# anilshanbhag/gpu-sort

Hardware: AMD Instinct MI355X
Metric: Gkeys/s sorting 2^30 uint32 keys; achieved HBM GB/s vs roofline (higher is better)
Workload: dtype u32; 1 GPU; lsb_radix_sort_2^30_u32_uniform_keys_only; keys_per_gpu=1073741824, algorithm=lsb, distribution=uniform, parallelism=single

## Files before the change

### gpu-sort_amd/_lib.py

```python
import ctypes as C
import os

import torch

_HERE = os.path.dirname(os.path.abspath(__file__))
LIB_PATH = os.environ.get("GS_LIB_PATH", os.path.join(_HERE, "lib", "libgpusort.so"))
CSRC_DIR = os.path.join(_HERE, "csrc")
INCLUDE_DIR = os.path.join(os.path.dirname(_HERE), "include")

GS_KEY_U32, GS_KEY_I32, GS_KEY_F32, GS_KEY_U64, GS_KEY_I64, GS_KEY_F64 = 0, 1, 2, 3, 4, 5
GS_KEY_U8, GS_KEY_I8, GS_KEY_U16, GS_KEY_I16 = 6, 7, 8, 9
GS_KEY_F16, GS_KEY_BF16, GS_KEY_F8 = 10, 11, 12
GS_GEN_UNIFORM, GS_GEN_ZIPF, GS_GEN_ENTROPY_AND, GS_GEN_ENUMERATED = 0, 1, 2, 3

u64, i32, vp, sz = C.c_uint64, C.c_int, C.c_void_p, C.c_size_t
pp = C.POINTER(C.c_void_p)

SIGNATURES = {
    "gs_version": (i32, []),
    "gs_error_string": (C.c_char_p, [i32]),
    "gs_lsb_temp_bytes": (sz, [u64, i32]),
    "gs_lsb_sort_u32": (i32, [vp, sz, pp, pp, C.POINTER(i32), u64, i32, i32, i32, i32, vp]),
    "gs_lsb_copy_temp_bytes": (sz, [u64, i32]),
    "gs_lsb_sort_copy_u32": (i32, [vp, sz, vp, vp, vp, vp, u64, i32, i32, i32, i32, vp]),
    "gs_lsb_wide_temp_bytes": (sz, [u64, i32, i32]),
    "gs_lsb_sort_wide": (i32, [vp, sz, pp, pp, C.POINTER(i32), u64, i32, i32, i32, i32, i32, i32, vp]),
    "gs_lsb_any_temp_bytes": (sz, [u64, i32, i32]),
    "gs_lsb_sort_any": (i32, [vp, sz, vp, vp, vp, vp, u64, i32, i32, i32, i32, i32, vp]),
    "gs_lsb_narrow_temp_bytes": (sz, [u64, i32, i32]),
    "gs_lsb_sort_narrow": (i32, [vp, sz, vp, vp, vp, vp, u64, i32, i32, i32, i32, i32, vp]),
    "gs_lsb_narrow_tile": (C.c_uint32, [i32, i32]),
    "gs_lsb_geometry": (None, [u64, i32, C.POINTER(C.c_uint32), C.POINTER(C.c_uint32), C.POINTER(C.c_uint32)]),
    "gs_lsb_workspace_layout": (i32, [vp, u64, pp, pp, pp]),
    "gs_lsb_pipe_status": (i32, [vp, u64, C.POINTER(C.c_uint32), vp]),
    "gs_lsb_plan_status": (i32, [vp, u64, C.POINTER(C.c_uint32), vp]),
    "gs_lsb_plan_cursor_status": (i32, [vp, u64, C.POINTER(C.c_uint32), vp]),
    "gs_lsb_plan_peek_status": (i32, [C.POINTER(C.c_uint32)]),
    "gs_lsb_plan_look_only": (i32, [vp, vp, vp, u64, i32, i32, vp]),
    "gs_lsb_plan_layout": (i32, [u64, C.POINTER(C.c_uint64)]),
    "gs_lsb_upsweep_u32": (i32, [vp, sz, vp, u64, i32, i32, i32, i32, vp]),
    "gs_lsb_scan_spine": (i32, [vp, sz, u64, vp]),
    "gs_lsb_downsweep_u32": (i32, [vp, sz, vp, vp, vp, vp, u64, i32, i32, i32, i32, i32, vp]),
    "gs_msb_temp_bytes": (sz, [u64, i32]),
    "gs_msb_sort_u32": (i32, [vp, sz, vp, vp, u64, vp, vp, pp, pp, i32, vp, i32]),
    "gs_msb_wide_temp_bytes": (sz, [u64, i32, i32]),
    "gs_msb_sort_wide": (i32, [vp, sz, vp, vp, u64, vp, vp, i32, i32, pp, pp, i32, vp, i32]),
    "gs_msb_large_temp_bytes": (sz, [u64, i32]),
    "gs_msb_sort_large_u32": (i32, [vp, sz, vp, vp, u64, vp, vp, i32, vp, i32]),
    "gs_msb_large_wide_temp_bytes": (sz, [u64, i32, i32]),
    "gs_msb_sort_large_wide": (i32, [vp, sz, vp, vp, u64, vp, vp, i32, i32, i32, vp, i32]),
    "gs_lsb_large_temp_bytes": (sz, [u64, i32, i32]),
    "gs_lsb_sort_large": (i32, [vp, sz, pp, pp, C.POINTER(i32), u64, i32, i32, i32, i32, i32, i32, vp]),
    "gs_lsb_narrow_large_temp_bytes": (sz, [u64, i32, i32]),
    "gs_lsb_sort_narrow_large": (i32, [vp, sz, vp, vp, vp, vp, u64, i32, i32, i32, i32, i32, vp]),
    "gs_topk_temp_bytes": (sz, [u64, u64, i32]),
    "gs_topk_u32": (i32, [vp, sz, vp, vp, vp, vp, u64, u64, i32, i32, vp]),
    "gs_topk_status": (i32, [vp, u64, u64, i32, C.POINTER(C.c_uint32), vp]),
    "gs_topk_u16_temp_bytes": (sz, [u64, u64, i32]),
    "gs_topk_u16": (i32, [vp, sz, vp, vp, vp, vp, u64, u64, i32, i32, vp]),
    "gs_topk_u16_status": (i32, [vp, u64, u64, i32, C.POINTER(C.c_uint32), vp]),
    "gs_topk_rows_temp_bytes": (sz, [u64, u64, u64, i32]),
    "gs_topk_rows_u32": (i32, [vp, sz, vp, vp, vp, vp, u64, u64, u64, u64, i32, i32, vp]),
    "gs_topk_rows_max_k": (C.c_uint32, []),
    "gs_topk_rows_plan": (i32, [u64, u64, u64, i32, C.POINTER(C.c_uint32)]),
    "gs_topk_rows_u16_temp_bytes": (sz, [u64, u64, u64, i32]),
    "gs_topk_rows_u16": (i32, [vp, sz, vp, vp, vp, vp, u64, u64, u64, u64, i32, i32, vp]),
    "gs_topk_segmented_temp_bytes": (sz, [u64, C.c_uint32, u64, i32]),
    "gs_topk_segmented_u32": (i32, [vp, sz, vp, vp, vp, vp, vp, u64, C.c_uint32, vp, vp, u64, i32, i32, vp]),
    "gs_topk_segmented_plan": (i32, [u64, C.c_uint32, u64, i32, C.POINTER(C.c_uint32)]),
    "gs_topk_segmented_status": (i32, [vp, u64, C.c_uint32, u64, i32, C.POINTER(C.c_uint32), vp]),
    "gs_msb_census": (i32, [vp, u64, i32, vp, vp]),
    "gs_msb_wide_census": (i32, [vp, u64, i32, i32, vp, vp]),
    "gs_msb_capacities": (None, [u64, i32, C.POINTER(C.c_uint32), C.POINTER(C.c_uint32), C.POINTER(C.c_uint32)]),
    "gs_msb_classify_upto": (i32, [vp, sz, vp, vp, u64, i32, i32, vp]),
    "gs_msb_read_lists": (i32, [vp, u64, i32, i32, vp, C.c_uint32, C.POINTER(C.c_uint32), C.POINTER(C.POINTER(C.c_uint32)), C.c_uint32,
                                C.POINTER(C.c_uint32), vp]),
    "gs_segmented_temp_bytes": (sz, [u64, i32, C.c_uint32]),
    "gs_segmented_sort_u32": (i32, [vp, sz, pp, pp, C.POINTER(i32), u64, C.c_uint32, vp, vp, i32, i32, i32, i32, vp]),
    "gs_segmented_wide_temp_bytes": (sz, [u64, i32, i32, C.c_uint32]),
    "gs_segmented_sort_wide": (i32, [vp, sz, pp, pp, C.POINTER(i32), u64, C.c_uint32, vp, vp, i32, i32, i32, i32, i32, i32, vp]),
    "gs_segmented_narrow_temp_bytes": (sz, [u64, i32, i32, C.c_uint32]),
    "gs_segmented_sort_narrow": (i32, [vp, sz, pp, pp, C.POINTER(i32), u64, C.c_uint32, vp, vp, i32, i32, i32, i32, i32, vp]),
    "gs_segmented_narrow_cap": (C.c_uint32, [i32, i32]),
    "gs_msb_first_pass_u32": (i32, [vp, sz, vp, vp, vp, vp, u64, i32, vp, vp]),
    "gs_msb_finish_temp_bytes": (sz, [u64, i32, i32]),
    "gs_msb_finish_u32": (i32, [vp, sz, vp, vp, vp, vp, u64, vp, i32, i32, vp, i32]),
    "gs_shard_histogram_u32": (i32, [vp, u64, i32, vp, i32, vp]),
    "gs_shard_partition_u32": (i32, [vp, sz, vp, vp, vp, vp, u64, i32, vp, i32, vp, vp, i32, vp]),
    "gs_generate_u32": (i32, [vp, u64, i32, u64, u64, i32, vp]),
    "gs_check_sorted_u32": (i32, [vp, u64, i32, vp, vp]),
    "gs_check_pairs_enumerated_u32": (i32, [vp, vp, vp, u64, vp, vp]),
    "gs_check_sorted_u64": (i32, [vp, u64, i32, vp, vp]),
    "gs_check_pairs_enumerated_wide": (i32, [vp, vp, vp, u64, i32, vp, vp]),
    "gs_check_sorted_stable": (i32, [vp, vp, u64, i32, i32, i32, i32, i32, vp, vp]),
    "gs_profile_create": (vp, []),
    "gs_profile_destroy": (None, [vp]),
    "gs_profile_begin": (None, [vp]),
    "gs_profile_end": (None, []),
    "gs_profile_read": (i32, [vp, C.POINTER(C.c_double), C.POINTER(u64)]),
    "gs_kernel_name": (C.c_char_p, [i32]),
}
GS_K_COUNT = 10


class GpuSortError(RuntimeError):
    def __init__(self, code, what):
        self.code = code
        super().__init__(f"{what}: hipError {code} ({error_string(code)})")


def _load():
    if not os.path.exists(LIB_PATH):
        raise ImportError(
            f"{LIB_PATH} is missing: the HIP extension is not built. "
            "Run `python -c 'import __graft_entry__ as g; g.build()'` (or make -C gpu-sort_amd/csrc). "
            "There is no CPU fallback."
        )
    lib = C.CDLL(LIB_PATH)
    for name, (res, args) in SIGNATURES.items():
        fn = getattr(lib, name)
        fn.restype = res
        fn.argtypes = args
    return lib


lib = _load()


def error_string(code):
    s = lib.gs_error_string(int(code))
    return s.decode() if s else "?"


def check(code, what):
    if code != 0:
        raise GpuSortError(code, what)


class KernelProfile:

    def __init__(self):
        self._p = lib.gs_profile_create()

    def __enter__(self):
        lib.gs_profile_begin(self._p)
        return self

    def __exit__(self, *exc):
        lib.gs_profile_end()
        return False

    def read(self):
        ms = (C.c_double * GS_K_COUNT)()
        cnt = (u64 * GS_K_COUNT)()
        check(lib.gs_profile_read(self._p, ms, cnt), "gs_profile_read")
        return {lib.gs_kernel_name(i).decode(): (ms[i], int(cnt[i])) for i in range(GS_K_COUNT) if cnt[i]}

    def close(self):
        if self._p and lib is not None:
            lib.gs_profile_destroy(self._p)
        self._p = None

    def __del__(self):
        try:
            self.close()
        except Exception:
            pass
```

### gpu-sort_amd/csrc/gs_lsb_downsweep.inc

```
#ifndef GS_EXP_SLEEP_MODE
#define GS_EXP_SLEEP_MODE 0
#endif
#ifndef GS_EXP_SLEEP_MIN_TILES
#define GS_EXP_SLEEP_MIN_TILES 49152u
#endif
#ifndef GS_EXP_SLEEP_PAIRS
#define GS_EXP_SLEEP_PAIRS 0
#endif
template <bool HAS_VALUES, bool OFF64 = false>
struct DownsweepSmem {
    uint32_t whist[LSB_WAVES][RADIX];
#ifdef GS_EXP_ALLWAVE_KEYS
    uint16_t wbase[LSB_WAVES][RADIX];
#else
    uint16_t wbase[HAS_VALUES ? LSB_WAVES : 1][RADIX];
#endif
    std::conditional_t<OFF64, uint64_t, uint32_t> gbase[RADIX];
    uint32_t stage[LSB_TILE * (HAS_VALUES ? 2 : 1)];
    uint32_t dead;
};

#ifdef GS_EXP_PHASES
__device__ uint32_t gs_phase_buf[131072 * 16];
#define GS_PHASE(k)                                                                          \
    do {                                                                                     \
        const unsigned long long now_ = __builtin_amdgcn_s_memtime();                        \
        if (tid == 0 && t < 131072u) gs_phase_buf[t * 16 + (k)] = (uint32_t)(now_ - tprev_); \
        tprev_ = now_;                                                                       \
    } while (0)
#define GS_PHASE_WAIT(what) asm volatile("s_waitcnt " what ::: "memory")
#else
#define GS_PHASE(k) do { } while (0)
#define GS_PHASE_WAIT(what) do { } while (0)
#endif

constexpr uint32_t PIPE_SPIN_LIMIT = 1u << 18;

template <bool HAS_VALUES, bool TAIL, int TW, bool BIG, bool PIPE, bool OFF64 = false, bool CURSOR = false>
__device__ __forceinline__ void downsweep_tile(DownsweepSmem<HAS_VALUES, OFF64> &sm, const uint32_t t,
    const uint32_t *__restrict__ keys_in, uint32_t *__restrict__ keys_out, const uint32_t *__restrict__ vals_in,
    uint32_t *__restrict__ vals_out, const uint32_t *__restrict__ spine, const uint16_t *__restrict__ prefix16,
    const uint32_t *__restrict__ totals, const PassParams &p, const uint64_t *__restrict__ sc, uint32_t tag,
    uint32_t *__restrict__ error_word, const uint32_t tid_ = threadIdx.x, const uint64_t *__restrict__ dbase = nullptr,
    uint32_t *__restrict__ cursor = nullptr, uint32_t *__restrict__ irr = nullptr, const uint32_t irr_cap = 0u)
{
    static_assert(!CURSOR || (!HAS_VALUES && !TAIL && !PIPE && !OFF64), "cursor mode: full tiles of keys-only three-launch passes");
#ifdef GS_EXP_ALLWAVE_KEYS
    constexpr bool ALLWAVE = true;
#else
    constexpr bool ALLWAVE = HAS_VALUES;
#endif

    [[maybe_unused]] const int tid = (int)tid_;
    const int lane = (int)(tid_ & 63u), w = (int)(tid_ >> 6);
    const uint32_t full_tiles = p.n / (uint32_t)LSB_TILE;
    auto tw_in = [&](uint32_t k) { return TW == 0 ? k : twiddle_in(k, TW == 2 ? p.f32_in : 0, p.xor_in); };
    auto tw_out = [&](uint32_t k) { return TW == 0 ? k : twiddle_out(k, TW == 2 ? p.f32_out : 0, p.xor_out); };
    uint32_t wbits = p.bits;
    asm volatile("" : "+v"(wbits));
    auto digit = [&](uint32_t k) { return __builtin_amdgcn_ubfe(k, p.shift, wbits); };

    uint32_t *my = sm.whist[w];
    const uint16_t *mybase = sm.wbase[w];
    const uint32_t wbase = (uint32_t)w * (WAVE * LSB_KPT) + lane;
    const uint32_t tail_valid = p.n - full_tiles * (uint32_t)LSB_TILE;
    (void)full_tiles;

#ifdef GS_EXP_PHASES
    unsigned long long tprev_ = __builtin_amdgcn_s_memtime();
    const unsigned long long t0_ = tprev_, r0_ = __builtin_amdgcn_s_memrealtime();
#endif
#ifdef GS_EXP_SLEEP_START
    __builtin_amdgcn_s_sleep(GS_EXP_SLEEP_START);
#endif
    if (!HAS_VALUES) __builtin_amdgcn_s_setprio(3);
    const uint64_t tile_base = (uint64_t)t * LSB_TILE;
    const uint32_t valid = TAIL ? tail_valid : (uint32_t)LSB_TILE;

    uint64_t scg[4] = {0, 0, 0, 0};
    const uint64_t *scrow = nullptr;
    if (PIPE && w == 0) {
        scrow = sc + (size_t)(t / LSB_CHUNK) * RADIX + 4 * lane;
#pragma unroll
        for (int q = 0; q < 4; ++q) scg[q] = ld_agent(scrow + q);
    }

    uint32_t key[LSB_KPT], val[HAS_VALUES ? LSB_KPT : 1], pos[LSB_KPT];
    {
        const uint32_t *kin = keys_in + tile_base;
        if (!TAIL) {
#pragma unroll
            for (int i = 0; i < LSB_KPT; ++i) key[i] = kin[wbase + i * WAVE];
        } else {
            const uint32_t pad = twiddle_out(0xffffffffu, TW == 2 ? p.f32_in : 0, TW ? p.xor_in : 0u);
#pragma unroll
            for (int i = 0; i < LSB_KPT; ++i) {
                const uint32_t idx = wbase + i * WAVE;
                key[i] = pad;
                if (idx < tail_valid) key[i] = kin[idx];
            }
        }
    }
    [[maybe_unused]] uint32_t cur_lo = 0, cur_hi = 0, claim[4] = {0, 0, 0, 0};
    if constexpr (CURSOR) {
        if (w == 0) {
            cur_lo = (tw_in(keys_in[tile_base]) >> (p.shift - (uint32_t)RADIX_BITS)) & (uint32_t)(RADIX - 1);
            cur_hi = (tw_in(keys_in[tile_base + (LSB_TILE - 1)]) >> (p.shift - (uint32_t)RADIX_BITS)) & (uint32_t)(RADIX - 1);
        }
    }
    GS_PHASE(0);
#ifndef GS_EXP_RANK_PRIO
#define GS_EXP_RANK_PRIO 0
#endif
    if (!HAS_VALUES) __builtin_amdgcn_s_setprio(GS_EXP_RANK_PRIO);
    if (HAS_VALUES) {
        const uint32_t *vin = vals_in + tile_base;
#pragma unroll
        for (int i = 0; i < LSB_KPT; ++i) {
            const uint32_t idx = wbase + i * WAVE;
            val[i] = 0;
            if (!TAIL || idx < valid) val[i] = vin[idx];
        }
    }
    uint32_t dstart[4] = {0, 0, 0, 0};
    if constexpr (OFF64) {
        if (TAIL && w == 0) {
            const uint4 tot = reinterpret_cast<const uint4 *>(totals)[lane];
            dstart[0] = tot.x; dstart[1] = tot.y; dstart[2] = tot.z; dstart[3] = tot.w;
        }
    } else if (!CURSOR && w == 0) {
        const uint4 tot = reinterpret_cast<const uint4 *>(totals)[lane];
        const uint32_t lane_sum = tot.x + tot.y + tot.z + tot.w;
        const uint32_t ex = wave_inclusive_scan(lane_sum) - lane_sum;
        dstart[0] = ex + (TAIL ? tot.x : 0u);
        dstart[1] = dstart[0] + (TAIL ? tot.y : tot.x);
        dstart[2] = dstart[1] + (TAIL ? tot.z : tot.y);
        dstart[3] = dstart[2] + (TAIL ? tot.w : tot.z);
    }

    uint32_t tbase[4] = {0, 0, 0, 0};
    if (!TAIL && !PIPE && !CURSOR && w == 0) {
        const uint32_t *sp = spine + (uint32_t)(4 * lane) * p.grid + t / LSB_CHUNK;
        const uint2 pf = reinterpret_cast<const uint2 *>(prefix16 + (size_t)t * RADIX)[lane];
        tbase[0] = sp[0] + (pf.x & 0xffffu);
        tbase[1] = sp[p.grid] + (pf.x >> 16);
        tbase[2] = sp[2 * p.grid] + (pf.y & 0xffffu);
        tbase[3] = sp[3 * p.grid] + (pf.y >> 16);
    }

    if (PIPE && !TAIL && w == 0) {
        uint32_t spins = 0;
        bool gave_up = false;
        for (;;) {
            const bool ok = (uint32_t)(scg[0] >> 32) == tag && (uint32_t)(scg[1] >> 32) == tag &&
                            (uint32_t)(scg[2] >> 32) == tag && (uint32_t)(scg[3] >> 32) == tag;
            if (__builtin_amdgcn_ballot_w64(!ok) == 0) break;
            if (++spins > PIPE_SPIN_LIMIT) {
                if (lane == 0) atomicOr(error_word, 1u);
                gave_up = true;
                break;
            }
            __builtin_amdgcn_s_sleep(8);
#pragma unroll
            for (int q = 0; q < 4; ++q) scg[q] = ld_agent(scrow + q);
        }
        if (lane == 0) sm.dead = gave_up ? 1u : 0u;
        const uint64_t pf = ld_agent(reinterpret_cast<const uint64_t *>(prefix16 + (size_t)t * RADIX) + lane);
        tbase[0] = (uint32_t)scg[0] + (uint32_t)(pf & 0xffffu);
        tbase[1] = (uint32_t)scg[1] + (uint32_t)((pf >> 16) & 0xffffu);
        tbase[2] = (uint32_t)scg[2] + (uint32_t)((pf >> 32) & 0xffffu);
        tbase[3] = (uint32_t)scg[3] + (uint32_t)(pf >> 48);
    }

    auto publish_gbase = [&](const uint32_t (&ex)[4], const uint32_t (&run)[4]) {
        uint32_t g[4];
#pragma unroll
        for (int q = 0; q < 4; ++q) g[q] = dstart[q] + tbase[q] - ex[q];
        if (TAIL) {
#pragma unroll
            for (int q = 0; q < 4; ++q) g[q] -= run[q];
            const uint32_t pads = (uint32_t)LSB_TILE - valid, dmax = p.mask;
            if (lane == (int)(dmax >> 2)) {
#pragma unroll
                for (int q = 0; q < 4; ++q)
                    if ((dmax & 3u) == (uint32_t)q) g[q] += pads;
            }
        }
        if constexpr (OFF64) {
#pragma unroll
            for (int q = 0; q < 4; ++q) sm.gbase[4 * lane + q] = dbase[4 * lane + q] + (uint64_t)(int64_t)(int32_t)g[q];
        } else {
            if (!BIG) {
#pragma unroll
                for (int q = 0; q < 4; ++q) g[q] <<= 2;
            }
            reinterpret_cast<uint4 *>(sm.gbase)[lane] = make_uint4(g[0], g[1], g[2], g[3]);
        }
    };

#pragma unroll
    for (int i = lane; i < RADIX; i += WAVE) my[i] = 0;
    GS_PHASE_WAIT("vmcnt(0)");
    GS_PHASE(1);
#pragma unroll
    for (int i = 0; i < LSB_KPT; ++i) key[i] = tw_in(key[i]);
    {
        uint32_t d_prev = 0, plo = 0, phi = 0;
#pragma unroll
        for (int i = 0; i <= LSB_KPT; ++i) {
            uint32_t d_cur = 0, clo = 0, chi = 0;
            if (i < LSB_KPT) {
                d_cur = digit(key[i]);
                match_digit(d_cur, clo, chi);
            }
            if (i > 0) {
                const uint32_t lower = count_lower(plo, phi);
                pos[i - 1] = my[d_prev] + lower;
                if (lower == 0)
                    __hip_atomic_fetch_add(&my[d_prev], (uint32_t)(__popc(plo) + __popc(phi)), __ATOMIC_RELAXED,
                                           __HIP_MEMORY_SCOPE_WAVEFRONT);
            }
            d_prev = d_cur; plo = clo; phi = chi;
        }
    }
#pragma unroll
    for (int i = 0; i < LSB_KPT; ++i) {
        asm volatile("" : "+v"(pos[i]), "+v"(key[i]));
    }
    if constexpr (CURSOR) {
        if (w == 0 && lane == 0) {
            const bool straddles = cur_lo != cur_hi;
            sm.dead = straddles ? 1u : 0u;
            if (straddles) {
                const uint32_t at = atomicAdd(&irr[0], 1u);
                if (at < irr_cap) irr[1u + at] = t;
            }
        }
    }
    GS_PHASE_WAIT("lgkmcnt(0)");
    GS_PHASE(2);
    __syncthreads();
    GS_PHASE(3);
    if (PIPE && !TAIL && sm.dead) return;
    if (CURSOR && sm.dead) return;

    if constexpr (ALLWAVE) {
        uint32_t run[4] = {0, 0, 0, 0}, below[4] = {0, 0, 0, 0};
#pragma unroll
        for (int j = 0; j < LSB_WAVES; ++j) {
            const uint4 x = reinterpret_cast<const uint4 *>(sm.whist[j])[lane];
            run[0] += x.x; run[1] += x.y; run[2] += x.z; run[3] += x.w;
            if (j < w) { below[0] += x.x; below[1] += x.y; below[2] += x.z; below[3] += x.w; }
        }
        const uint32_t lane_sum = run[0] + run[1] + run[2] + run[3];
        uint32_t ex[4];
        ex[0] = wave_inclusive_scan(lane_sum) - lane_sum;
        ex[1] = ex[0] + run[0];
        ex[2] = ex[1] + run[1];
        ex[3] = ex[2] + run[2];
        reinterpret_cast<uint2 *>(sm.wbase[w])[lane] =
            make_uint2((ex[0] + below[0]) | ((ex[1] + below[1]) << 16), (ex[2] + below[2]) | ((ex[3] + below[3]) << 16));
        if (w == 0) publish_gbase(ex, run);
    } else {
        if (w == 0) {
            uint32_t run[4] = {0, 0, 0, 0};
#pragma unroll
            for (int j = 0; j < LSB_WAVES; ++j) {
                const uint4 x = reinterpret_cast<const uint4 *>(sm.whist[j])[lane];
                run[0] += x.x; run[1] += x.y; run[2] += x.z; run[3] += x.w;
            }
            const uint32_t lane_sum = run[0] + run[1] + run[2] + run[3];
            uint32_t ex[4];
            ex[0] = wave_inclusive_scan(lane_sum) - lane_sum;
            ex[1] = ex[0] + run[0];
            ex[2] = ex[1] + run[1];
            ex[3] = ex[2] + run[2];
            if constexpr (CURSOR) {
                reinterpret_cast<uint4 *>(sm.gbase)[lane] = make_uint4(ex[0], ex[1], ex[2], ex[3]);
                uint32_t *row = cursor + (size_t)__builtin_amdgcn_readfirstlane(cur_lo) * RADIX;
#pragma unroll
                for (int q = 0; q < 4; ++q) {
                    const int d = q * WAVE + lane;
                    const uint32_t e0 = sm.gbase[d], e1 = sm.gbase[d == RADIX - 1 ? d : d + 1];
                    const uint32_t cnt = (d == RADIX - 1 ? (uint32_t)LSB_TILE : e1) - e0;
                    claim[q] = __hip_atomic_fetch_add(row + d, cnt, __ATOMIC_RELAXED, __HIP_MEMORY_SCOPE_AGENT);
                }
            } else {
                publish_gbase(ex, run);
            }
            asm volatile("" ::: "memory");
            uint4 e4 = make_uint4(ex[0] << 2, ex[1] << 2, ex[2] << 2, ex[3] << 2);
#pragma unroll
            for (int j = 0; j < LSB_WAVES; ++j) {
                const uint4 x = reinterpret_cast<const uint4 *>(sm.whist[j])[lane];
                reinterpret_cast<uint4 *>(sm.whist[j])[lane] = e4;
                e4.x += x.x << 2; e4.y += x.y << 2; e4.z += x.z << 2; e4.w += x.w << 2;
            }
        }
        __syncthreads();
    }
    GS_PHASE(4);

    {
        uint32_t wb[LSB_KPT];
#pragma unroll
        for (int i = 0; i < LSB_KPT; ++i) {
            const uint32_t d = digit(key[i]);
            wb[i] = ALLWAVE ? (uint32_t)mybase[d] : my[d];
        }
#pragma unroll
        for (int i = 0; i < LSB_KPT; ++i) {
            if (HAS_VALUES) {
                reinterpret_cast<uint2 *>(sm.stage)[pos[i] + wb[i]] = make_uint2(key[i], val[i]);
            } else if (ALLWAVE) {
                sm.stage[pos[i] + wb[i]] = key[i];
            } else {
                const uint32_t at = (pos[i] << 2) + wb[i];
                *reinterpret_cast<uint32_t *>(reinterpret_cast<char *>(sm.stage) + at) = key[i];
            }
        }
    }
    if constexpr (CURSOR) {
        if (w == 0) {
#pragma unroll
            for (int q = 0; q < 4; ++q) {
                const int d = q * WAVE + lane;
                const uint32_t g = claim[q] - sm.gbase[d];
                sm.gbase[d] = BIG ? g : g << 2;
            }
        }
    }
    GS_PHASE_WAIT("lgkmcnt(0)");
    GS_PHASE(5);
    __syncthreads();
    GS_PHASE(6);
#ifndef GS_EXP_SLEEP
#define GS_EXP_SLEEP 32
#define GS_EXP_SLEEP_MODE_DEFAULT 0
#else
#define GS_EXP_SLEEP_MODE_DEFAULT GS_EXP_SLEEP_MODE
#endif
    if ((!HAS_VALUES || GS_EXP_SLEEP_PAIRS) && full_tiles >= GS_EXP_SLEEP_MIN_TILES) {
        [[maybe_unused]] const int ws = __builtin_amdgcn_readfirstlane(w);
#if GS_EXP_SLEEP_MODE_DEFAULT == 3
        if (ws & 1) __builtin_amdgcn_s_sleep(GS_EXP_SLEEP); else __builtin_amdgcn_s_sleep(GS_EXP_SLEEP_B);
#elif GS_EXP_SLEEP_MODE_DEFAULT == 4
        if (ws >= 4) __builtin_amdgcn_s_sleep(GS_EXP_SLEEP);
#elif GS_EXP_SLEEP_MODE_DEFAULT == 1
        if (ws & 1) __builtin_amdgcn_s_sleep(GS_EXP_SLEEP);
#elif GS_EXP_SLEEP_MODE_DEFAULT == 0
        __builtin_amdgcn_s_sleep(GS_EXP_SLEEP);
#endif
    }
#ifndef GS_EXP_STORE_PRIO
#define GS_EXP_STORE_PRIO 3
#endif
    if (!HAS_VALUES) __builtin_amdgcn_s_setprio(GS_EXP_STORE_PRIO);
#pragma unroll
    for (int i = 0; i < LSB_KPT; ++i) {
        const uint32_t slot = (uint32_t)w * (WAVE * LSB_KPT) + i * WAVE + lane;
        uint32_t k, v = 0;
        if (HAS_VALUES) {
            const uint2 kv = reinterpret_cast<const uint2 *>(sm.stage)[slot];
            k = kv.x; v = kv.y;
        } else {
            k = sm.stage[slot];
        }
        const auto g = sm.gbase[digit(k)];
        if (!TAIL || slot < valid) {
            if constexpr (OFF64) {
                const uint64_t dst = g + slot;
                keys_out[dst] = tw_out(k);
                if (HAS_VALUES) vals_out[dst] = v;
            } else if (BIG) {
                const uint32_t dst = g + slot;
                keys_out[dst] = tw_out(k);
                if (HAS_VALUES) vals_out[dst] = v;
            } else {
                const uint32_t off = g + slot * 4u;
                *reinterpret_cast<uint32_t *>(reinterpret_cast<char *>(keys_out) + off) = tw_out(k);
                if (HAS_VALUES) *reinterpret_cast<uint32_t *>(reinterpret_cast<char *>(vals_out) + off) = v;
            }
        }
    }
    GS_PHASE(7);
#ifdef GS_EXP_DRAIN
    asm volatile("s_waitcnt vmcnt(0)" ::: "memory");
#endif
    GS_PHASE_WAIT("vmcnt(0)");
    GS_PHASE(8);
#ifdef GS_EXP_PHASES
    if (tid == 0 && t < 131072u) {
        gs_phase_buf[t * 16 + 9] = (uint32_t)(__builtin_amdgcn_s_memtime() - t0_);
        gs_phase_buf[t * 16 + 10] = (uint32_t)(__builtin_amdgcn_s_memrealtime() - r0_);
        gs_phase_buf[t * 16 + 11] = (uint32_t)r0_;
        gs_phase_buf[t * 16 + 12] = blockIdx.x;
        gs_phase_buf[t * 16 + 13] = __builtin_amdgcn_s_getreg((31 << 11) | 4);
        gs_phase_buf[t * 16 + 14] = __builtin_amdgcn_s_getreg((31 << 11) | 20);
    }
#endif
}
```

### gpu-sort_amd/csrc/gs_lsb_plan.hip

```cpp
#include "gs_device.hpp"
#include "gs_lsb.hpp"
#include "gs_msb_tasks.hpp"
#ifndef GS_PLAN_N_MIN
#define GS_PLAN_N_MIN (1ull << 28)
#endif
#include <cstddef>
#include <cstdlib>
#include <cstring>
#include <type_traits>

namespace gs {

#include "gs_lsb_upsweep.inc"

#include "gs_lsb_downsweep.inc"

constexpr uint32_t PLAN_GROUPS = 65536;
constexpr uint32_t PLAN_WORDS = PLAN_GROUPS / 2;
constexpr uint32_t PLAN_PLANNED = 1u, PLAN_CLASSIC = 2u;
constexpr uint32_t PLAN_SKIP = 0xffffffffu;
constexpr int PLAN_LOOK_THREADS = 1024, PLAN_LOOK_WAVES = PLAN_LOOK_THREADS / WAVE, PLAN_LOOK_BATCH = 32;
constexpr uint32_t PLAN_LOOK_HALVES = PLAN_LOOK_WAVES / LSB_CHUNK;
static_assert(PLAN_LOOK_WAVES % LSB_CHUNK == 0, "a look workgroup takes whole chunks");
constexpr uint32_t PLAN_LOOK_MAX_GRID = MI355X_CUS;
constexpr uint32_t PLAN_BLOCKS = 128, PLAN_BLOCK_WORDS = PLAN_WORDS / PLAN_BLOCKS, PLAN_BLOCK_GROUPS = PLAN_GROUPS / PLAN_BLOCKS;
constexpr int PLAN_SORT_BITS = 16;
constexpr int PLAN_SKEW_LANES = 8;
constexpr uint32_t PLAN_IRR_CAP = RADIX - 1;
constexpr size_t PLAN_CURSOR_BYTES = (size_t)PLAN_GROUPS * sizeof(uint32_t);

struct PlanBlock {
    uint32_t route, max_group, nonempty, tasks[MSB_NCLASS], total;
    uint32_t shift[4];
    uint32_t ups_skip[4];
    MsbLevel level[2];
    union {
        uint32_t wg_bad[PLAN_LOOK_MAX_GRID];
        uint32_t irr[1 + PLAN_IRR_CAP];
    };
    uint32_t blk_total[PLAN_BLOCKS], blk_max[PLAN_BLOCKS], blk_nonempty[PLAN_BLOCKS];
    uint32_t blk_class[PLAN_BLOCKS][MSB_NCLASS];
    uint32_t blk_class_base[PLAN_BLOCKS][MSB_NCLASS];
    uint32_t offsets[PLAN_GROUPS + 1];
    uint32_t cursor_mode;
};
static_assert(1 + PLAN_IRR_CAP <= PLAN_LOOK_MAX_GRID, "the list of straddling tiles fits the look's flags");
static_assert(sizeof(MsbLevel) == 64 && offsetof(PlanBlock, level) == 64, "plan block layout");

__device__ __forceinline__ int plan_class_of(uint32_t size)
{
    return size <= msb_class_cap(0) ? 0 : size <= msb_class_cap(1) ? 1 : size <= msb_class_cap(2) ? 2 : 3;
}

__device__ __forceinline__ void look_add(uint32_t *tab, uint32_t *my, uint32_t g)
{
    const unsigned long long act = __builtin_amdgcn_ballot_w64(true);
    const uint32_t g0 = __builtin_amdgcn_readfirstlane(g);
    if (__builtin_amdgcn_ballot_w64(g == g0) == act) {
        if (count_lower_mask(act) == 0) {
            atomicAdd(&tab[g0 >> 1], (uint32_t)__popcll(act) << ((g0 & 1u) * 16u));
            atomicAdd(&my[g0 & 0xffu], (uint32_t)__popcll(act));
        }
    } else {
        atomicAdd(&tab[g >> 1], 1u << ((g & 1u) * 16u));
        atomicAdd(&my[g & 0xffu], 1u);
    }
}

__device__ __forceinline__ void look_add_skew(uint32_t *tab, uint32_t *my, uint32_t g, int lane)
{
    unsigned long long rest = ~0ull;
#pragma unroll
    for (int r = 0; r < 2; ++r) {
        if (rest == 0ull) break;
        const int lead = __builtin_amdgcn_readfirstlane(__builtin_ctzll(rest));
        const uint32_t g0 = (uint32_t)__builtin_amdgcn_readlane((int)g, lead);
        const unsigned long long m = __builtin_amdgcn_ballot_w64(g == g0) & rest;
        if (lane == lead) {
            atomicAdd(&tab[g0 >> 1], (uint32_t)__popcll(m) << ((g0 & 1u) * 16u));
            atomicAdd(&my[g0 & 0xffu], (uint32_t)__popcll(m));
        }
        rest &= ~m;
    }
    if ((rest >> lane) & 1ull) {
        atomicAdd(&tab[g >> 1], 1u << ((g & 1u) * 16u));
        atomicAdd(&my[g & 0xffu], 1u);
    }
}

__device__ __forceinline__ uint32_t look_slot_of_block(uint32_t b, uint32_t grid)
{
    if (grid % MI355X_XCDS) return b;
    return (b % MI355X_XCDS) * (grid / MI355X_XCDS) + b / MI355X_XCDS;
}

struct LookSmem {
    uint32_t tab[PLAN_WORDS];
    uint32_t hist[PLAN_LOOK_WAVES][RADIX + 1];
    uint32_t red[2];
};
static_assert(sizeof(LookSmem) <= 160 * 1024, "the look's LDS");

__global__ __launch_bounds__(PLAN_LOOK_THREADS) void lsb_plan_look_kernel(const uint32_t *__restrict__ keys, uint32_t *__restrict__ partial,
                                                                          PlanBlock *__restrict__ plan, uint32_t *__restrict__ spine,
                                                                          uint16_t *__restrict__ prefix16, uint32_t n, uint32_t chunks,
                                                                          int f32_in, uint32_t xor_in)
{
    __shared__ LookSmem sm;
    uint32_t *tab = sm.tab;
    const int tid = threadIdx.x, w = wave_id(), lane = lane_id();
    for (uint32_t i = tid; i < PLAN_WORDS; i += PLAN_LOOK_THREADS) tab[i] = 0;
    for (uint32_t i = tid; i < sizeof(sm.hist) / sizeof(uint32_t); i += PLAN_LOOK_THREADS) (&sm.hist[0][0])[i] = 0;
    if (tid < 2) sm.red[tid] = 0;
    __syncthreads();
    uint32_t *my = sm.hist[w];
    const uint32_t num_tiles = n / (uint32_t)LSB_TILE + (n % (uint32_t)LSB_TILE ? 1u : 0u);
    const uint32_t units = (chunks + PLAN_LOOK_HALVES - 1u) / PLAN_LOOK_HALVES;
    auto group_of = [&](uint32_t raw) { return twiddle_in(raw, f32_in, xor_in) >> 16; };
    uint32_t counted = 0;
    constexpr int GB = PLAN_LOOK_BATCH;
#pragma unroll 1
    for (uint32_t unit = look_slot_of_block(blockIdx.x, gridDim.x); unit < units; unit += gridDim.x) {
        const uint32_t tile = unit * (uint32_t)PLAN_LOOK_WAVES + (uint32_t)w;
        if (tile < num_tiles) {
        const uint32_t lo = tile * (uint32_t)LSB_TILE;
        const uint32_t len = (n - lo < (uint32_t)LSB_TILE) ? n - lo : (uint32_t)LSB_TILE;
        const uint32_t *src = keys + lo;
        counted += len;
        if (len == (uint32_t)LSB_TILE) {
#pragma unroll 1
            for (uint32_t j = 0; j < (uint32_t)LSB_TILE; j += GB * WAVE) {
                const uint32_t *at = src + j + lane;
                uint32_t v[GB];
#pragma unroll
                for (int u = 0; u < GB; ++u) v[u] = __builtin_nontemporal_load(at + u * WAVE);
                const uint32_t ga = group_of(v[0]), gb = group_of(v[GB / 2]);
                const unsigned long long ma = __builtin_amdgcn_ballot_w64(ga == __builtin_amdgcn_readfirstlane(ga)),
                                         mb = __builtin_amdgcn_ballot_w64(gb == __builtin_amdgcn_readfirstlane(gb));
                if (ma == ~0ull || mb == ~0ull) {
#pragma unroll
                    for (int u = 0; u < GB; ++u) look_add(tab, my, group_of(v[u]));
                } else if (__popcll(ma) >= PLAN_SKEW_LANES || __popcll(mb) >= PLAN_SKEW_LANES) {
#pragma unroll
                    for (int u = 0; u < GB; ++u) look_add_skew(tab, my, group_of(v[u]), lane);
                } else {
#pragma unroll
                    for (int u = 0; u < GB; ++u) {
                        const uint32_t g = group_of(v[u]);
                        atomicAdd(&tab[g >> 1], 1u << ((g & 1u) * 16u));
                        atomicAdd(&my[g & 0xffu], 1u);
                    }
                }
            }
        } else {
            const uint32_t last = len - 1u;
#pragma unroll 1
            for (uint32_t j = 0; j < len; j += GB * WAVE) {
                uint32_t v[GB];
#pragma unroll
                for (int u = 0; u < GB; ++u) {
                    const uint32_t idx = j + u * WAVE + lane;
                    v[u] = src[idx < last ? idx : last];
                }
#pragma unroll
                for (int u = 0; u < GB; ++u)
                    if (j + u * WAVE + lane < len) look_add(tab, my, group_of(v[u]));
            }
        }
        }
        __syncthreads();
        if (tid < (int)PLAN_LOOK_HALVES * RADIX) {
            const uint32_t half = (uint32_t)tid / RADIX, d = (uint32_t)tid % RADIX, chunk = unit * PLAN_LOOK_HALVES + half;
            uint32_t run = 0;
#pragma unroll
            for (int j = 0; j < LSB_CHUNK; ++j) {
                const uint32_t t = chunk * LSB_CHUNK + (uint32_t)j;
                if (t < num_tiles) prefix16[(size_t)t * RADIX + d] = (uint16_t)run;
                uint32_t *c = &sm.hist[half * LSB_CHUNK + j][d];
                run += *c;
                *c = 0;
            }
            if (chunk < chunks) spine[d * chunks + chunk] = run;
        }
        __syncthreads();
    }
    uint32_t sum = 0;
    uint32_t *out = partial + (size_t)blockIdx.x * PLAN_WORDS;
    for (uint32_t i = tid; i < PLAN_WORDS; i += PLAN_LOOK_THREADS) {
        const uint32_t c = tab[i];
        sum += (c & 0xffffu) + (c >> 16);
        out[i] = c;
    }
    sum = wave_reduce_sum(sum);
    if (lane == 0) { atomicAdd(&sm.red[0], sum); atomicAdd(&sm.red[1], counted); }
    __syncthreads();
    if (tid == 0) plan->wg_bad[blockIdx.x] = sm.red[0] != sm.red[1] ? 1u : 0u;
}

__global__ __launch_bounds__(RADIX) void lsb_plan_reduce_kernel(const uint32_t *__restrict__ partial, PlanBlock *__restrict__ plan, uint32_t parts)
{
    __shared__ uint32_t scratch[8];
    __shared__ uint32_t red[2 + MSB_NCLASS];
    const uint32_t tid = threadIdx.x, wi = blockIdx.x * PLAN_BLOCK_WORDS + tid;
    if (tid < 2 + MSB_NCLASS) red[tid] = 0;
    uint32_t c0 = 0, c1 = 0;
#pragma unroll 8
    for (uint32_t g = 0; g < parts; ++g) {
        const uint32_t v = partial[(size_t)g * PLAN_WORDS + wi];
        c0 += v & 0xffffu;
        c1 += v >> 16;
    }
    uint32_t total = 0;
    const uint32_t ex = block_exclusive_scan_256(c0 + c1, scratch, &total);
    plan->offsets[2 * wi] = ex;
    plan->offsets[2 * wi + 1] = ex + c0;
    atomicMax(&red[0], c0 > c1 ? c0 : c1);
    if (c0) { atomicAdd(&red[1], 1u); atomicAdd(&red[2 + plan_class_of(c0)], 1u); }
    if (c1) { atomicAdd(&red[1], 1u); atomicAdd(&red[2 + plan_class_of(c1)], 1u); }
    __syncthreads();
    if (tid == 0) {
        plan->blk_total[blockIdx.x] = total;
        plan->blk_max[blockIdx.x] = red[0];
        plan->blk_nonempty[blockIdx.x] = red[1];
    }
    if (tid < MSB_NCLASS) plan->blk_class[blockIdx.x][tid] = red[2 + tid];
}

__global__ __launch_bounds__(RADIX) void lsb_plan_decide_kernel(PlanBlock *__restrict__ plan, uint32_t n, uint32_t parts, uint32_t cursor_on)
{
    __shared__ uint32_t s_base, s_total, s_max, s_nz, s_cls[MSB_NCLASS], s_clsbase[MSB_NCLASS];
    const uint32_t tid = threadIdx.x, b = blockIdx.x;
    if (tid == 0) {
        uint32_t base = 0, total = 0, mx = 0, nz = 0;
        for (uint32_t i = 0; i < PLAN_BLOCKS; ++i) {
            if (i == b) base = total;
            total += plan->blk_total[i];
            const uint32_t m = plan->blk_max[i];
            mx = m > mx ? m : mx;
            nz += plan->blk_nonempty[i];
        }
        s_base = base; s_total = total; s_max = mx; s_nz = nz;
    } else if (tid <= MSB_NCLASS) {
        const uint32_t c = tid - 1u;
        uint32_t base = 0, total = 0;
        for (uint32_t i = 0; i < PLAN_BLOCKS; ++i) {
            if (i == b) base = total;
            total += plan->blk_class[i][c];
        }
        s_cls[c] = total; s_clsbase[c] = base;
    }
    const int any_bad = __syncthreads_or(tid < parts ? (int)plan->wg_bad[tid] : 0);
    const uint32_t g = b * PLAN_BLOCK_GROUPS + 2u * tid;
    plan->offsets[g] += s_base;
    plan->offsets[g + 1] += s_base;
    if (tid < MSB_NCLASS) plan->blk_class_base[b][tid] = s_clsbase[tid];
    if (b == 0 && tid == 0) {
        const bool planned = !any_bad && s_total == n && s_max <= msb_class_cap(MSB_NCLASS - 1);
        plan->route = planned ? PLAN_PLANNED : PLAN_CLASSIC;
        plan->max_group = s_max;
        plan->nonempty = s_nz;
        plan->total = s_total;
        MsbLevel l0{}, l1{};
        for (int c = 0; c < MSB_NCLASS; ++c) {
            plan->tasks[c] = planned ? s_cls[c] : 0u;
            l0.task_count[c] = planned ? s_cls[c] : 0u;
        }
        l0.keys = n;
        l1.packed = planned ? (1ull << 32) : 0ull;
        plan->level[0] = l0;
        plan->level[1] = l1;
        for (int q = 0; q < 4; ++q) {
            plan->shift[q] = planned ? (q < 2 ? 16u + 8u * (uint32_t)q : PLAN_SKIP) : 8u * (uint32_t)q;
            plan->ups_skip[q] = planned && q != 1 ? 1u : 0u;
        }
        plan->offsets[PLAN_GROUPS] = n;
        plan->cursor_mode = planned && cursor_on ? 1u : 0u;
    }
}

constexpr int PLAN_PEEK_WORDS = 9;
static_assert(offsetof(PlanBlock, total) == (PLAN_PEEK_WORDS - 2) * sizeof(uint32_t), "the head is eight words");
__global__ void lsb_plan_peek_kernel(const PlanBlock *__restrict__ plan, uint32_t *mailbox)
{
    const uint32_t *head = &plan->route;
    for (int i = 0; i < PLAN_PEEK_WORDS - 1; ++i) mailbox[i] = head[i];
    mailbox[PLAN_PEEK_WORDS - 1] = plan->cursor_mode;
    __threadfence_system();
}

struct PlanLists { MsbTask *tasks[MSB_NCLASS]; uint32_t cap[MSB_NCLASS]; };
__global__ __launch_bounds__(PLAN_BLOCK_GROUPS) void lsb_plan_tasks_kernel(const PlanBlock *__restrict__ plan, PlanLists lists)
{
    __shared__ uint32_t wcnt[PLAN_BLOCK_GROUPS / WAVE][MSB_NCLASS];
    if (plan->route != PLAN_PLANNED) return;
    const uint32_t tid = threadIdx.x, g = blockIdx.x * PLAN_BLOCK_GROUPS + tid;
    const int w = wave_id(), lane = lane_id();
    const uint32_t off = plan->offsets[g], size = plan->offsets[g + 1] - off;
    const int cls = size ? plan_class_of(size) : -1;
    uint32_t lower = 0;
#pragma unroll
    for (int c = 0; c < MSB_NCLASS; ++c) {
        const unsigned long long m = __builtin_amdgcn_ballot_w64(cls == c);
        if (cls == c) lower = count_lower_mask(m);
        if (lane == 0) wcnt[w][c] = (uint32_t)__popcll(m);
    }
    __syncthreads();
    if (cls >= 0) {
        uint32_t idx = plan->blk_class_base[blockIdx.x][cls] + lower;
        for (int j = 0; j < w; ++j) idx += wcnt[j][cls];
        if (idx < lists.cap[cls]) lists.tasks[cls][idx] = MsbTask{off, size, (uint32_t)PLAN_SORT_BITS, 0u};
    }
}

template <bool PLAIN>
__global__ __launch_bounds__(LSB_THREADS, GS_EXP_UPS_WPE) void lsb_plan_upsweep_kernel(const uint32_t *__restrict__ keys,
                                                                       uint32_t *__restrict__ spine, uint16_t *__restrict__ prefix16,
                                                                       const uint32_t *__restrict__ slot_shift,
                                                                       const uint32_t *__restrict__ slot_ups_skip, PassParams p)
{
    __shared__ UpsweepSmem<false, false> sm;
    const uint32_t sh = *slot_shift;
    if (sh == PLAN_SKIP || *slot_ups_skip) return;
    p.shift = sh;
    upsweep_chunk<false, false, PLAIN>(sm, keys, chunk_of_block(blockIdx.x, p.grid), spine, prefix16, nullptr, nullptr, p, PipeParams{});
}

template <bool TAIL, int TW, bool BIG>
__global__ __launch_bounds__(LSB_THREADS, 6) void lsb_plan_downsweep_kernel(const uint32_t *__restrict__ keys_in, uint32_t *__restrict__ keys_out,
                                                                            const uint32_t *__restrict__ totals, const uint32_t *__restrict__ spine,
                                                                            const uint16_t *__restrict__ prefix16,
                                                                            const uint32_t *__restrict__ slot_shift, PassParams p)
{
    __shared__ __attribute__((aligned(16))) DownsweepSmem<false> sm;
    const uint32_t sh = *slot_shift;
    if (sh == PLAN_SKIP) return;
    p.shift = sh;
    const uint32_t full_tiles = p.n / (uint32_t)LSB_TILE;
    if (!TAIL && blockIdx.x >= full_tiles) return;
    const uint32_t t = TAIL ? full_tiles : tile_of_item_wide(blockIdx.x, full_tiles);
    downsweep_tile<false, TAIL, TW, BIG, false>(sm, t, keys_in, keys_out, nullptr, nullptr, spine, prefix16, totals, p, nullptr, 0u, nullptr);
}

template <bool PLAIN>
__global__ __launch_bounds__(LSB_THREADS, GS_EXP_UPS_WPE) void lsb_plan_upsweep2_kernel(const uint32_t *__restrict__ keys,
                                                                        uint32_t *__restrict__ spine, uint16_t *__restrict__ prefix16,
                                                                        PlanBlock *__restrict__ plan, uint32_t *__restrict__ cursor,
                                                                        PassParams p)
{
    __shared__ UpsweepSmem<false, false> sm;
    if (plan->cursor_mode) {
        if (blockIdx.x == 0 && threadIdx.x == 0) plan->irr[0] = 0;
        for (uint32_t i = blockIdx.x * (uint32_t)LSB_THREADS + threadIdx.x; i < PLAN_GROUPS; i += gridDim.x * (uint32_t)LSB_THREADS)
            cursor[i] = plan->offsets[((i & (uint32_t)(RADIX - 1)) << RADIX_BITS) | (i >> RADIX_BITS)];
        return;
    }
    const uint32_t sh = plan->shift[1];
    if (sh == PLAN_SKIP || plan->ups_skip[1]) return;
    p.shift = sh;
    upsweep_chunk<false, false, PLAIN>(sm, keys, chunk_of_block(blockIdx.x, p.grid), spine, prefix16, nullptr, nullptr, p, PipeParams{});
}

template <bool TAIL, bool BIG>
__global__ __launch_bounds__(LSB_THREADS, 6) void lsb_plan_scatter2_kernel(const uint32_t *__restrict__ keys_in, uint32_t *__restrict__ keys_out,
                                                                           const uint32_t *__restrict__ totals, const uint32_t *__restrict__ spine,
                                                                           const uint16_t *__restrict__ prefix16, PlanBlock *__restrict__ plan,
                                                                           uint32_t *__restrict__ cursor, PassParams p)
{
    __shared__ __attribute__((aligned(16))) DownsweepSmem<false> sm;
    const uint32_t sh = plan->shift[1];
    if (sh == PLAN_SKIP) return;
    p.shift = sh;
    const uint32_t full_tiles = p.n / (uint32_t)LSB_TILE;
    const uint32_t mode = plan->cursor_mode;
    if constexpr (TAIL) {
        if (mode) return;
        downsweep_tile<false, true, 2, true, false>(sm, full_tiles, keys_in, keys_out, nullptr, nullptr, spine, prefix16, totals, p, nullptr, 0u,
                                                    nullptr);
    } else {
        if (blockIdx.x >= full_tiles) return;
        const uint32_t t = tile_of_item_wide(blockIdx.x, full_tiles);
        if (mode)
            downsweep_tile<false, false, 0, BIG, false, false, true>(sm, t, keys_in, keys_out, nullptr, nullptr, spine, prefix16, totals, p,
                                                                     nullptr, 0u, nullptr, threadIdx.x, nullptr, cursor, plan->irr, PLAN_IRR_CAP);
        else
            downsweep_tile<false, false, 0, BIG, false>(sm, t, keys_in, keys_out, nullptr, nullptr, spine, prefix16, totals, p, nullptr, 0u,
                                                        nullptr);
    }
}

__global__ __launch_bounds__(LSB_THREADS) void lsb_plan_irregular_kernel(const uint32_t *__restrict__ keys_in, uint32_t *__restrict__ keys_out,
                                                                         const PlanBlock *__restrict__ plan, uint32_t *__restrict__ cursor,
                                                                         uint32_t n)
{
    if (!plan->cursor_mode) return;
    const uint32_t full_tiles = n / (uint32_t)LSB_TILE;
    uint32_t lo, len;
    if (blockIdx.x == PLAN_IRR_CAP) {
        lo = full_tiles * (uint32_t)LSB_TILE;
        len = n - lo;
    } else {
        const uint32_t listed = plan->irr[0] < PLAN_IRR_CAP ? plan->irr[0] : PLAN_IRR_CAP;
        if (blockIdx.x >= listed) return;
        const uint32_t t = plan->irr[1u + blockIdx.x];
        if (t >= full_tiles) return;
        lo = t * (uint32_t)LSB_TILE;
        len = (uint32_t)LSB_TILE;
    }
    const int lane = lane_id();
    for (uint32_t i = threadIdx.x; i - (uint32_t)lane < len; i += (uint32_t)LSB_THREADS) {
        const bool have = i < len;
        const uint32_t k = have ? keys_in[lo + i] : 0u;
        const uint32_t g = k >> 16, c = ((g & (uint32_t)(RADIX - 1)) << RADIX_BITS) | (g >> RADIX_BITS);
        unsigned long long rest = __builtin_amdgcn_ballot_w64(have);
        uint32_t at = 0;
#pragma unroll
        for (int r = 0; r < 2; ++r) {
            if (rest == 0ull) break;
            const int lead = __builtin_amdgcn_readfirstlane(__builtin_ctzll(rest));
            const uint32_t c0 = (uint32_t)__builtin_amdgcn_readlane((int)c, lead);
            const unsigned long long m = __builtin_amdgcn_ballot_w64(have && c == c0) & rest;
            uint32_t first = 0;
            if (lane == lead) first = __hip_atomic_fetch_add(cursor + c0, (uint32_t)__popcll(m), __ATOMIC_RELAXED, __HIP_MEMORY_SCOPE_AGENT);
            first = (uint32_t)__builtin_amdgcn_readlane((int)first, lead);
            if ((m >> lane) & 1ull) at = first + (uint32_t)__popcll(m & ((1ull << lane) - 1ull));
            rest &= ~m;
        }
        if ((rest >> lane) & 1ull) at = __hip_atomic_fetch_add(cursor + c, 1u, __ATOMIC_RELAXED, __HIP_MEMORY_SCOPE_AGENT);
        if (have && at < n) keys_out[at] = k;
    }
}

static inline size_t align256(size_t x) { return (x + 255) & ~(size_t)255; }

static inline bool plan_enabled()
{
    static const bool v = [] { const char *e = getenv("GS_LSB_KEYS_PLAN"); return !(e && strcmp(e, "classic") == 0); }();
    return v;
}
static inline bool plan_cursor_enabled()
{
    static const bool v = [] { const char *e = getenv("GS_LSB_PLAN_SCATTER2"); return !(e && strcmp(e, "stable") == 0); }();
    return v;
}
constexpr uint64_t PLAN_N_MAX = (uint64_t)PLAN_GROUPS * 16620u;
constexpr uint64_t PLAN_N_FLOOR = 65536;
constexpr uint64_t PLAN_N_MIN = GS_PLAN_N_MIN;
static inline uint64_t plan_min_items()
{
    static const uint64_t v = [] {
        const char *e = getenv("GS_LSB_PLAN_MIN_ITEMS");
        if (!e) return PLAN_N_MIN;
        const uint64_t x = strtoull(e, nullptr, 10);
        return x < PLAN_N_FLOOR ? PLAN_N_FLOOR : x;
    }();
    return v;
}
static inline bool plan_has_block(uint64_t n) { return !lsb_pipe_enabled() && n >= plan_min_items(); }
static inline bool plan_size_ok(uint64_t n) { return plan_has_block(n) && n <= PLAN_N_MAX; }
static inline uint32_t plan_list_cap(uint64_t n, int c)
{
    const uint64_t m = c == 0 ? n : n / ((uint64_t)msb_class_cap(c - 1) + 1u) + 1u;
    return (uint32_t)(m < PLAN_GROUPS ? m : PLAN_GROUPS);
}
static inline size_t plan_lists_bytes(uint64_t n)
{
    size_t b = 0;
    for (int c = 0; c < MSB_NCLASS; ++c) b += (size_t)plan_list_cap(n, c) * sizeof(MsbTask);
    return b;
}
static inline size_t plan_block_offset(uint64_t n)
{
    const size_t a = lsb_temp_bytes(n), b = plan_lists_bytes(n);
    return align256(a > b ? a : b);
}
static inline size_t plan_temp_bytes(uint64_t n) { return plan_block_offset(n) + align256(sizeof(PlanBlock)); }
static inline uint32_t *plan_cursors(char *base, uint64_t n) { return (uint32_t *)(base + plan_block_offset(n) - PLAN_CURSOR_BYTES); }

template <int TW, bool BIG>
static void launch_plan_downsweep(const uint32_t *kin, uint32_t *kout, const LsbWorkspace &ws, const uint32_t *slot_shift,
                                  const PassParams &p, hipStream_t s)
{
    hipLaunchKernelGGL((lsb_plan_downsweep_kernel<false, TW, BIG>), dim3(p.ds_grid), dim3(LSB_THREADS), 0, s, kin, kout, ws.totals,
                       ws.spine, ws.prefix16, slot_shift, p);
}

static int lsb_plan_slot2(const uint32_t *kin, uint32_t *kout, const LsbWorkspace &ws, PlanBlock *plan, uint32_t *cursor,
                          const PassParams &p, hipStream_t s);
static int lsb_plan_slot(const uint32_t *kin, uint32_t *kout, const LsbWorkspace &ws, const uint32_t *slot_shift,
                         const uint32_t *slot_ups_skip, const PassParams &p, bool real, bool ups_real, hipStream_t s)
{
    {
        KernelTimer kt(ups_real ? GS_K_LSB_UPSWEEP : GS_K_OTHER, s);
        if (!p.f32_in && !p.xor_in)
            hipLaunchKernelGGL(lsb_plan_upsweep_kernel<true>, dim3(p.grid), dim3(LSB_THREADS), 0, s, kin, ws.spine, ws.prefix16, slot_shift,
                               slot_ups_skip, p);
        else
            hipLaunchKernelGGL(lsb_plan_upsweep_kernel<false>, dim3(p.grid), dim3(LSB_THREADS), 0, s, kin, ws.spine, ws.prefix16, slot_shift,
                               slot_ups_skip, p);
    }
    {
        if (const int e = lsb_scan_as(ws.spine, ws.totals, p.grid, s, real ? GS_K_LSB_SCAN : GS_K_OTHER)) return e;
    }
    {
        KernelTimer kt(real ? GS_K_LSB_DOWNSWEEP : GS_K_OTHER, s);
        if (p.n >= (uint32_t)LSB_TILE) {
            const int tw = (p.f32_in || p.f32_out) ? 2 : ((p.xor_in | p.xor_out) ? 1 : 0);
            const bool big = p.n > (1u << 30);
#define GS_PDS(TW_, BIG_) launch_plan_downsweep<TW_, BIG_>(kin, kout, ws, slot_shift, p, s)
            if (big) { if (tw == 2) GS_PDS(2, true); else if (tw == 1) GS_PDS(1, true); else GS_PDS(0, true); }
            else { if (tw == 2) GS_PDS(2, false); else if (tw == 1) GS_PDS(1, false); else GS_PDS(0, false); }
#undef GS_PDS
        }
        if (p.n % (uint32_t)LSB_TILE)
            hipLaunchKernelGGL((lsb_plan_downsweep_kernel<true, 2, true>), dim3(1), dim3(LSB_THREADS), 0, s, kin, kout, ws.totals,
                               (const uint32_t *)nullptr, (const uint16_t *)nullptr, slot_shift, p);
    }
    return (int)hipGetLastError();
}

static int lsb_plan_slot2(const uint32_t *kin, uint32_t *kout, const LsbWorkspace &ws, PlanBlock *plan, uint32_t *cursor,
                          const PassParams &p, hipStream_t s)
{
    if (p.f32_in || p.f32_out || p.xor_in || p.xor_out) return hipErrorInvalidValue;
    if ((char *)cursor < (char *)ws.prefix16) return hipErrorInvalidValue;
    {
        KernelTimer kt(GS_K_OTHER, s);
        hipLaunchKernelGGL(lsb_plan_upsweep2_kernel<true>, dim3(p.grid), dim3(LSB_THREADS), 0, s, kin, ws.spine, ws.prefix16, plan, cursor, p);
    }
    if (const int e = lsb_scan_as(ws.spine, ws.totals, p.grid, s, GS_K_LSB_SCAN)) return e;
    {
        KernelTimer kt(GS_K_LSB_DOWNSWEEP, s);
        if (p.n >= (uint32_t)LSB_TILE) {
            if (p.n > (1u << 30))
                hipLaunchKernelGGL((lsb_plan_scatter2_kernel<false, true>), dim3(p.ds_grid), dim3(LSB_THREADS), 0, s, kin, kout, ws.totals,
                                   ws.spine, ws.prefix16, plan, cursor, p);
            else
                hipLaunchKernelGGL((lsb_plan_scatter2_kernel<false, false>), dim3(p.ds_grid), dim3(LSB_THREADS), 0, s, kin, kout, ws.totals,
                                   ws.spine, ws.prefix16, plan, cursor, p);
        }
        if (p.n % (uint32_t)LSB_TILE)
            hipLaunchKernelGGL((lsb_plan_scatter2_kernel<true, true>), dim3(1), dim3(LSB_THREADS), 0, s, kin, kout, ws.totals,
                               (const uint32_t *)nullptr, (const uint16_t *)nullptr, plan, cursor, p);
    }
    {
        KernelTimer kt(GS_K_OTHER, s);
        hipLaunchKernelGGL(lsb_plan_irregular_kernel, dim3(PLAN_IRR_CAP + (p.n % (uint32_t)LSB_TILE ? 1u : 0u)), dim3(LSB_THREADS), 0, s, kin,
                           kout, plan, cursor, p.n);
    }
    return (int)hipGetLastError();
}

static int lsb_plan_look(const uint32_t *keys, uint32_t *alt, const LsbWorkspace &ws, PlanBlock *plan, uint64_t n, const PassParams &tw,
                         hipStream_t s)
{
    const uint32_t parts = (uint32_t)(n / PLAN_WORDS < PLAN_LOOK_MAX_GRID ? n / PLAN_WORDS : PLAN_LOOK_MAX_GRID);
    const uint32_t chunks = lsb_make_params(n, 16, RADIX_BITS).grid;
    KernelTimer kt(GS_K_OTHER, s);
    hipLaunchKernelGGL(lsb_plan_look_kernel, dim3(parts), dim3(PLAN_LOOK_THREADS), 0, s, keys, alt, plan, ws.spine, ws.prefix16, (uint32_t)n,
                       chunks, tw.f32_in, tw.xor_in);
    hipLaunchKernelGGL(lsb_plan_reduce_kernel, dim3(PLAN_BLOCKS), dim3(RADIX), 0, s, alt, plan, parts);
    hipLaunchKernelGGL(lsb_plan_decide_kernel, dim3(PLAN_BLOCKS), dim3(RADIX), 0, s, plan, (uint32_t)n, parts, plan_cursor_enabled() ? 1u : 0u);
    return (int)hipGetLastError();
}

static int lsb_plan_slot2_cursor(const uint32_t *kin, uint32_t *kout, const LsbWorkspace &ws, PlanBlock *plan, uint32_t *cursor,
                                 const PassParams &p, hipStream_t s)
{
    if (p.f32_in || p.f32_out || p.xor_in || p.xor_out) return hipErrorInvalidValue;
    if ((char *)cursor < (char *)ws.prefix16) return hipErrorInvalidValue;
    {
        KernelTimer kt(GS_K_OTHER, s);
        hipLaunchKernelGGL(lsb_plan_upsweep2_kernel<true>, dim3(p.grid), dim3(LSB_THREADS), 0, s, kin, ws.spine, ws.prefix16, plan, cursor, p);
    }
    if (p.n >= (uint32_t)LSB_TILE) {
        KernelTimer kt(GS_K_LSB_DOWNSWEEP, s);
        if (p.n > (1u << 30))
            hipLaunchKernelGGL((lsb_plan_scatter2_kernel<false, true>), dim3(p.ds_grid), dim3(LSB_THREADS), 0, s, kin, kout, ws.totals,
                               ws.spine, ws.prefix16, plan, cursor, p);
        else
            hipLaunchKernelGGL((lsb_plan_scatter2_kernel<false, false>), dim3(p.ds_grid), dim3(LSB_THREADS), 0, s, kin, kout, ws.totals,
                               ws.spine, ws.prefix16, plan, cursor, p);
    }
    {
        KernelTimer kt(GS_K_OTHER, s);
        hipLaunchKernelGGL(lsb_plan_irregular_kernel, dim3(PLAN_IRR_CAP + (p.n % (uint32_t)LSB_TILE ? 1u : 0u)), dim3(LSB_THREADS), 0, s, kin,
                           kout, plan, cursor, p.n);
    }
    return (int)hipGetLastError();
}

struct PlanPeek {
    uint32_t *host = nullptr, *dev = nullptr;
    hipEvent_t ev = nullptr;
    int device = -1;
    bool armed = false;
};
static bool plan_peek_enabled()
{
    static const bool on = [] { const char *e = getenv("GS_LSB_PLAN_PEEK"); return !(e && e[0] == '0'); }();
    return on;
}
constexpr int PLAN_PEEK_DEVICES = 16;
struct PlanPeekTable {
    PlanPeek slot[PLAN_PEEK_DEVICES];
    ~PlanPeekTable()
    {
        for (PlanPeek &pk : slot) {
            if (pk.ev) (void)hipEventDestroy(pk.ev);
            if (pk.host) (void)hipHostFree(pk.host);
        }
    }
};
static PlanPeek *plan_peek_get(hipStream_t s)
{
    if (!plan_peek_enabled()) return nullptr;
    hipStreamCaptureStatus cs = hipStreamCaptureStatusNone;
    if (hipStreamIsCapturing(s, &cs) != hipSuccess || cs != hipStreamCaptureStatusNone) { (void)hipGetLastError(); return nullptr; }
    thread_local PlanPeekTable table;
    int dev = -1;
    if (hipGetDevice(&dev) != hipSuccess || dev < 0 || dev >= PLAN_PEEK_DEVICES) { (void)hipGetLastError(); return nullptr; }
    PlanPeek &pk = table.slot[dev];
    if (pk.device != dev) {
        void *h = nullptr, *d = nullptr;
        if (hipHostMalloc(&h, 64, hipHostMallocMapped | hipHostMallocPortable) != hipSuccess ||
            hipHostGetDevicePointer(&d, h, 0) != hipSuccess ||
            hipEventCreateWithFlags(&pk.ev, hipEventDisableTiming) != hipSuccess) {
            (void)hipGetLastError();
            if (h) (void)hipHostFree(h);
            pk.ev = nullptr;
            return nullptr;
        }
        pk.host = (uint32_t *)h; pk.dev = (uint32_t *)d; pk.device = dev;
    }
    if (pk.armed) { (void)hipEventSynchronize(pk.ev); (void)hipGetLastError(); }
    pk.armed = false;
    return &pk;
}
static void plan_peek_arm(PlanPeek *pk, const PlanBlock *plan, hipStream_t s)
{
    if (!pk) return;
    for (int i = 0; i < PLAN_PEEK_WORDS; ++i) ((volatile uint32_t *)pk->host)[i] = 0;
    KernelTimer kt(GS_K_OTHER, s);
    hipLaunchKernelGGL(lsb_plan_peek_kernel, dim3(1), dim3(1), 0, s, plan, pk->dev);
    pk->armed = hipGetLastError() == hipSuccess && hipEventRecord(pk->ev, s) == hipSuccess;
    if (!pk->armed) (void)hipGetLastError();
}
struct PlanSeen { bool ok = false; uint32_t route = 0, tasks[MSB_NCLASS] = {0, 0, 0, 0}, cursor_mode = 0; };
static PlanSeen plan_peek_wait(PlanPeek *pk, uint64_t n)
{
    PlanSeen seen;
    if (!pk || !pk->armed) return seen;
    pk->armed = false;
    if (hipEventSynchronize(pk->ev) != hipSuccess) { (void)hipGetLastError(); return seen; }
    uint32_t w[PLAN_PEEK_WORDS];
    for (int i = 0; i < PLAN_PEEK_WORDS; ++i) w[i] = ((const volatile uint32_t *)pk->host)[i];
    const uint32_t route = w[0], nonempty = w[2], total = w[7], mode = w[8];
    if (route != PLAN_PLANNED && route != PLAN_CLASSIC) return seen;
    if (route == PLAN_PLANNED ? (uint64_t)total != n : (uint64_t)total > n) return seen;
    if (mode > 1u || (mode && route != PLAN_PLANNED)) return seen;
    uint64_t sum = 0;
    for (int c = 0; c < MSB_NCLASS; ++c) {
        if (w[3 + c] > plan_list_cap(n, c)) return seen;
        sum += w[3 + c];
    }
    if (route == PLAN_PLANNED ? sum != nonempty : sum != 0) return seen;
    seen.ok = true;
    seen.route = route;
    seen.cursor_mode = mode;
    for (int c = 0; c < MSB_NCLASS; ++c) seen.tasks[c] = w[3 + c];
    return seen;
}
static thread_local uint32_t plan_peek_last[4] = {0, 0, 0, 0};

int lsb_plan_sort(char *base, uint32_t *d_keys[2], int *selector, uint64_t n, int descending, int key_type, hipStream_t s)
{
    const LsbWorkspace ws = lsb_carve(base, n);
    char *lists_end = base + plan_block_offset(n);
    PlanBlock *plan = (PlanBlock *)lists_end;
    PlanLists lists;
    for (int c = MSB_NCLASS - 1; c >= 0; --c) {
        lists.cap[c] = plan_list_cap(n, c);
        lists_end -= (size_t)lists.cap[c] * sizeof(MsbTask);
        lists.tasks[c] = (MsbTask *)lists_end;
    }
    int sel = *selector, e;
    PassParams tw{};
    lsb_twiddle_masks(key_type, descending, true, true, tw);
    if ((e = lsb_plan_look(d_keys[sel], d_keys[sel ^ 1], ws, plan, n, tw, s))) return e;
    PlanPeek *peek = plan_peek_get(s);
    plan_peek_arm(peek, plan, s);
    PlanSeen seen;
    plan_peek_last[0] = plan_peek_last[1] = 0; plan_peek_last[2] = 4; plan_peek_last[3] = (1u << MSB_NCLASS) - 1u;
    for (int slot = 0; slot < 4; ++slot) {
        PassParams p = lsb_make_params(n, 0, RADIX_BITS);
        lsb_twiddle_masks(key_type, descending, slot == 0, slot == 3, p);
        const uint32_t *kin = d_keys[sel];
        uint32_t *kout = d_keys[sel ^ 1];
        e = hipSuccess;
        if (seen.ok && seen.route == PLAN_CLASSIC)
            e = lsb_plan_slot(kin, kout, ws, &plan->shift[slot], &plan->ups_skip[slot], p, true, true, s);
        else if (seen.ok && slot >= 2)
            ;
        else if (seen.ok && slot == 1 && seen.cursor_mode)
            e = lsb_plan_slot2_cursor(kin, kout, ws, plan, plan_cursors(base, n), p, s);
        else if (slot == 1 && plan_cursor_enabled())
            e = lsb_plan_slot2(kin, kout, ws, plan, plan_cursors(base, n), p, s);
        else
            e = lsb_plan_slot(kin, kout, ws, &plan->shift[slot], &plan->ups_skip[slot], p, slot < 2, slot == 1, s);
        if (e) return e;
        sel ^= 1;
        if (slot == 0) {
            seen = plan_peek_wait(peek, n);
            if (seen.ok) {
                plan_peek_last[0] = 1; plan_peek_last[1] = seen.route; plan_peek_last[2] = seen.route == PLAN_PLANNED ? 2 : 4;
                plan_peek_last[3] = 0;
                for (int c = 0; c < MSB_NCLASS; ++c) plan_peek_last[3] |= seen.tasks[c] ? 1u << c : 0u;
            }
        }
    }
    if (seen.ok && seen.route == PLAN_CLASSIC) {
        *selector = sel;
        return hipSuccess;
    }
    {
        KernelTimer kt(GS_K_OTHER, s);
        hipLaunchKernelGGL(lsb_plan_tasks_kernel, dim3(PLAN_BLOCKS), dim3(PLAN_BLOCK_GROUPS), 0, s, plan, lists);
    }
    if ((e = (int)hipGetLastError())) return e;
    if ((e = msb_local_sorts_in_place(plan->level, lists.tasks, PLAN_GROUPS, PLAN_GROUPS, d_keys[sel], PLAN_SORT_BITS, n, tw.f32_out,
                                      tw.xor_out, s, seen.ok ? seen.tasks : nullptr)))
        return e;
    *selector = sel;
    return hipSuccess;
}


bool lsb_plan_has_block(uint64_t n) { return plan_has_block(n); }
size_t lsb_plan_temp_bytes(uint64_t n) { return plan_temp_bytes(n); }
bool lsb_plan_applies(uint64_t n) { return plan_enabled() && plan_size_ok(n); }

}

using namespace gs;

extern "C" {

int gs_lsb_plan_status(void *d_temp, uint64_t num_items, uint32_t out[8], void *stream)
{
    GS_CLEAR_STALE_ERROR();
    if (!d_temp || !out || num_items >= (1ull << 32)) return hipErrorInvalidValue;
    memset(out, 0, 8 * sizeof(uint32_t));
    if (!plan_enabled() || !plan_size_ok(num_items)) return hipSuccess;
    const PlanBlock *plan = (const PlanBlock *)(gs_ws_base(d_temp) + plan_block_offset(num_items));
    hipError_t e = hipMemcpyAsync(out, plan, 8 * sizeof(uint32_t), hipMemcpyDeviceToHost, (hipStream_t)stream);
    if (e == hipSuccess) e = hipStreamSynchronize((hipStream_t)stream);
    return (int)e;
}

int gs_lsb_plan_cursor_status(void *d_temp, uint64_t num_items, uint32_t out[4], void *stream)
{
    GS_CLEAR_STALE_ERROR();
    if (!d_temp || !out || num_items >= (1ull << 32)) return hipErrorInvalidValue;
    memset(out, 0, 4 * sizeof(uint32_t));
    if (!plan_enabled() || !plan_size_ok(num_items)) return hipSuccess;
    const PlanBlock *plan = (const PlanBlock *)(gs_ws_base(d_temp) + plan_block_offset(num_items));
    uint32_t w[2] = {0, 0};
    hipError_t e = hipMemcpyAsync(&w[0], &plan->cursor_mode, sizeof(uint32_t), hipMemcpyDeviceToHost, (hipStream_t)stream);
    if (e == hipSuccess) e = hipMemcpyAsync(&w[1], &plan->irr[0], sizeof(uint32_t), hipMemcpyDeviceToHost, (hipStream_t)stream);
    if (e == hipSuccess) e = hipStreamSynchronize((hipStream_t)stream);
    if (e != hipSuccess) return (int)e;
    if (w[0] == 1u) {
        out[0] = 1;
        out[2] = w[1];
        out[1] = w[1] + (num_items % (uint64_t)LSB_TILE ? 1u : 0u);
    }
    return hipSuccess;
}

int gs_lsb_plan_peek_status(uint32_t out[4])
{
    if (!out) return hipErrorInvalidValue;
    memcpy(out, plan_peek_last, sizeof(plan_peek_last));
    return hipSuccess;
}

int gs_lsb_plan_look_only(void *d_temp, const void *d_keys, void *d_alt, uint64_t num_items, int key_type, int descending, void *stream)
{
    GS_CLEAR_STALE_ERROR();
    if (!d_temp || !d_keys || !d_alt || num_items >= (1ull << 32)) return hipErrorInvalidValue;
    if (!plan_enabled() || !plan_size_ok(num_items)) return hipErrorInvalidValue;
    char *base = gs_ws_base(d_temp);
    PassParams tw{};
    lsb_twiddle_masks(key_type, descending, true, true, tw);
    return lsb_plan_look((const uint32_t *)d_keys, (uint32_t *)d_alt, lsb_carve(base, num_items), (PlanBlock *)(base + plan_block_offset(num_items)),
                         num_items, tw, (hipStream_t)stream);
}

int gs_lsb_plan_layout(uint64_t num_items, uint64_t out[4])
{
    if (!out || num_items >= (1ull << 32) || !plan_enabled() || !plan_size_ok(num_items)) return hipErrorInvalidValue;
    char *base = (char *)(uintptr_t)GS_WS_ALIGN;
    const LsbWorkspace ws = lsb_carve(base, num_items);
    out[0] = (uint64_t)((char *)ws.spine - base);
    out[1] = (uint64_t)((char *)ws.prefix16 - base);
    out[2] = plan_block_offset(num_items);
    out[3] = lsb_make_params(num_items, 16, RADIX_BITS).grid;
    return hipSuccess;
}

}
```

### gpu-sort_amd/csrc/gs_msb.hip

```cpp
#include "gs_device.hpp"
#include <new>
#include "gs_lsb.hpp"
#include "gs_msb_tasks.hpp"
#include <type_traits>
#include <vector>
#include <cstdlib>

namespace gs {

constexpr int MSB_THREADS = 512;
constexpr int MSB_WAVES = MSB_THREADS / WAVE;
constexpr int MSB_KPT = 16;
constexpr int MSB_TILE = MSB_THREADS * MSB_KPT;
constexpr uint32_t MSB_MERGE = 3000;
constexpr uint32_t MSB_MAX_GRID = 16384;
__host__ __device__ constexpr uint32_t msb_tiles_of(uint32_t x) { return x / (uint32_t)MSB_TILE + (x % (uint32_t)MSB_TILE ? 1u : 0u); }
#ifndef GS_PAIR_CLASSES
#define GS_PAIR_CLASSES 4
#endif
__host__ __device__ constexpr int msb_num_classes(bool has_values) { return has_values ? GS_PAIR_CLASSES : 4; }

struct MsbBucket { uint32_t offset, size, tile_start, tiles; };
struct MsbPiece { uint32_t lo, size, tile_start, bucket; };
struct MsbTile { uint32_t lo, valid, bucket, pad; };
// ... 619 lines not shown
                e4.x += x.x << ESH; e4.y += x.y << ESH; e4.z += x.z << ESH; e4.w += x.w << ESH;
            }
        }
        __syncthreads();
    }
    {
        uint32_t wb[MSB_KPT];
#pragma unroll
        for (int i = 0; i < MSB_KPT; ++i) {
            const uint32_t d = digit(key[i], wbase + i * WAVE);
            wb[i] = ALLWAVE ? (uint32_t)mybase[d] : my[d];
        }
#pragma unroll
        for (int i = 0; i < MSB_KPT; ++i) {
            const uint32_t at = ALLWAVE ? ((pos[i] + wb[i]) << ESH) : ((pos[i] << ESH) + wb[i]);
            if (HAS_VALUES) *reinterpret_cast<uint2 *>(reinterpret_cast<char *>(sm.stage) + at) = make_uint2(key[i], val[i]);
            else *reinterpret_cast<uint32_t *>(reinterpret_cast<char *>(sm.stage) + at) = key[i];
        }
    }
    __syncthreads();
#ifndef GS_MSB_SCATTER_SLEEP
#define GS_MSB_SCATTER_SLEEP 0
#endif
    if (!HAS_VALUES && GS_MSB_SCATTER_SLEEP && (w & 1)) __builtin_amdgcn_s_sleep(GS_MSB_SCATTER_SLEEP);
    if (!HAS_VALUES) __builtin_amdgcn_s_setprio(3);
#pragma unroll
    for (int i = 0; i < MSB_KPT; ++i) {
        const uint32_t slot = (uint32_t)w * (WAVE * MSB_KPT) + i * WAVE + lane;
        uint32_t k, v = 0;
        if (HAS_VALUES) {
            const uint2 kv = reinterpret_cast<const uint2 *>(sm.stage)[slot];
            k = kv.x; v = kv.y;
        } else {
            k = sm.stage[slot];
        }
        if (FULL || slot < valid) {
            const uint32_t gb = sm.gbase[msb_digit<REMAP>(ds, sm.tab, k)];
            const uint32_t ko = TWOUT ? twiddle_out(k, f32_out, xor_out) : k;
            if (small) {
                const uint32_t off = gb + slot * 4u;
                *reinterpret_cast<uint32_t *>(reinterpret_cast<char *>(dst_k) + off) = ko;
                if (HAS_VALUES) *reinterpret_cast<uint32_t *>(reinterpret_cast<char *>(dst_v) + off) = v;
            } else {
                const uint32_t dst = gb + slot;
                dst_k[dst] = ko;
                if (HAS_VALUES) dst_v[dst] = v;
            }
        }
    }
}

template <bool FULL>
__device__ __forceinline__ void msb_pivot_tile(uint32_t *__restrict__ scratch ,
                                               MsbPivot *__restrict__ P, const MsbBucket &B, const uint32_t *__restrict__ src_k,
                                               uint32_t *__restrict__ other, uint32_t *__restrict__ result, uint32_t lo,
                                               uint32_t valid, int f32_out, uint32_t xor_out, bool write_all)
{
    const int lane = lane_id(), w = wave_id();
    const uint32_t wbase = (uint32_t)w * (WAVE * MSB_KPT) + lane;
    uint32_t key[MSB_KPT];
    const uint32_t *pk = src_k + lo;
#pragma unroll
    for (int i = 0; i < MSB_KPT; ++i) {
        const uint32_t idx = wbase + i * WAVE;
        key[i] = pk[FULL ? idx : (idx < valid ? idx : valid - 1u)];
    }
    const uint32_t cand = P->cand, mid_lo = B.offset + P->less, mid_hi = mid_lo + P->eq;
    const uint32_t cand_out = twiddle_out(cand, f32_out, xor_out);
    uint32_t wl = 0, wg = 0;
#pragma unroll
    for (int i = 0; i < MSB_KPT; ++i) {
        const bool in = FULL || wbase + i * WAVE < valid;
        wl += (uint32_t)__popcll(__builtin_amdgcn_ballot_w64(in && key[i] < cand));
        wg += (uint32_t)__popcll(__builtin_amdgcn_ballot_w64(in && key[i] > cand));
    }
    if (lane == 0) { scratch[w] = wl; scratch[MSB_WAVES + w] = wg; }
    __syncthreads();
    if (threadIdx.x == 0) {
        uint32_t tl = 0, tg = 0;
#pragma unroll
        for (int j = 0; j < MSB_WAVES; ++j) { const uint32_t a = scratch[j], b2 = scratch[MSB_WAVES + j]; scratch[j] = tl; scratch[MSB_WAVES + j] = tg; tl += a; tg += b2; }
        scratch[2 * MSB_WAVES] = tl ? atomicAdd(&P->cur_less, tl) : 0u;
        scratch[2 * MSB_WAVES + 1] = tg ? atomicAdd(&P->cur_greater, tg) : 0u;
    }
    __syncthreads();
    uint32_t nl = B.offset + scratch[2 * MSB_WAVES] + scratch[w];
    uint32_t ng = B.offset + B.size - 1u - scratch[2 * MSB_WAVES + 1] - scratch[MSB_WAVES + w];
#pragma unroll
    for (int i = 0; i < MSB_KPT; ++i) {
        const uint32_t idx = wbase + i * WAVE;
        const bool in = FULL || idx < valid;
        const uint32_t k = key[i], at = lo + idx;
        const unsigned long long ml = __builtin_amdgcn_ballot_w64(in && k < cand), mg = __builtin_amdgcn_ballot_w64(in && k > cand);
        if (in) {
            if (k < cand) other[nl + count_lower_mask(ml)] = k;
            else if (k > cand) other[ng - count_lower_mask(mg)] = k;
            if (at >= mid_lo && at < mid_hi && (write_all || k != cand)) result[at] = cand_out;
        }
        nl += (uint32_t)__popcll(ml);
        ng -= (uint32_t)__popcll(mg);
    }
}

template <bool FULL>
__device__ __forceinline__ void msb_pivot_tile_pairs(uint32_t *__restrict__ scratch ,
                                                     MsbPivot *__restrict__ P, const MsbBucket &B, const uint32_t *__restrict__ src_k,
                                                     const uint32_t *__restrict__ src_v, uint32_t *__restrict__ other_k,
                                                     uint32_t *__restrict__ other_v, uint32_t *__restrict__ mid_k,
                                                     uint32_t *__restrict__ mid_v, uint32_t lo, uint32_t valid, int f32_out, uint32_t xor_out)
{
    const int lane = lane_id(), w = wave_id();
    const uint32_t wbase = (uint32_t)w * (WAVE * MSB_KPT) + lane;
    uint32_t key[MSB_KPT], val[MSB_KPT];
    const uint32_t *pk = src_k + lo, *pv = src_v + lo;
#pragma unroll
    for (int i = 0; i < MSB_KPT; ++i) {
        const uint32_t idx = wbase + i * WAVE, at = FULL ? idx : (idx < valid ? idx : valid - 1u);
        key[i] = pk[at]; val[i] = pv[at];
    }
    const uint32_t cand = P->cand, mid_lo = B.offset + P->less;
    const uint32_t cand_out = twiddle_out(cand, f32_out, xor_out);
    uint32_t wl = 0, wg = 0, we = 0;
#pragma unroll
    for (int i = 0; i < MSB_KPT; ++i) {
        const bool in = FULL || wbase + i * WAVE < valid;
        wl += (uint32_t)__popcll(__builtin_amdgcn_ballot_w64(in && key[i] < cand));
        wg += (uint32_t)__popcll(__builtin_amdgcn_ballot_w64(in && key[i] > cand));
        we += (uint32_t)__popcll(__builtin_amdgcn_ballot_w64(in && key[i] == cand));
    }
    if (lane == 0) { scratch[w] = wl; scratch[MSB_WAVES + w] = wg; scratch[2 * MSB_WAVES + w] = we; }
    __syncthreads();
    if (threadIdx.x == 0) {
        uint32_t tl = 0, tg = 0, te = 0;
#pragma unroll
        for (int j = 0; j < MSB_WAVES; ++j) {
            const uint32_t a = scratch[j], b2 = scratch[MSB_WAVES + j], c = scratch[2 * MSB_WAVES + j];
            scratch[j] = tl; scratch[MSB_WAVES + j] = tg; scratch[2 * MSB_WAVES + j] = te;
            tl += a; tg += b2; te += c;
        }
        scratch[3 * MSB_WAVES] = tl ? atomicAdd(&P->cur_less, tl) : 0u;
        scratch[3 * MSB_WAVES + 1] = tg ? atomicAdd(&P->cur_greater, tg) : 0u;
        scratch[3 * MSB_WAVES + 2] = te ? atomicAdd(&P->pad1, te) : 0u;
    }
    __syncthreads();
    uint32_t nl = B.offset + scratch[3 * MSB_WAVES] + scratch[w];
    uint32_t ng = B.offset + B.size - 1u - scratch[3 * MSB_WAVES + 1] - scratch[MSB_WAVES + w];
    uint32_t ne = mid_lo + scratch[3 * MSB_WAVES + 2] + scratch[2 * MSB_WAVES + w];
#pragma unroll
    for (int i = 0; i < MSB_KPT; ++i) {
        const bool in = FULL || wbase + i * WAVE < valid;
        const uint32_t k = key[i];
        const unsigned long long ml = __builtin_amdgcn_ballot_w64(in && k < cand), mg = __builtin_amdgcn_ballot_w64(in && k > cand),
                                 me = __builtin_amdgcn_ballot_w64(in && k == cand);
        if (in) {
            if (k < cand) { const uint32_t at = nl + count_lower_mask(ml); other_k[at] = k; other_v[at] = val[i]; }
            else if (k > cand) { const uint32_t at = ng - count_lower_mask(mg); other_k[at] = k; other_v[at] = val[i]; }
            else { const uint32_t at = ne + count_lower_mask(me); if (mid_k) mid_k[at] = cand_out; mid_v[at] = val[i]; }
        }
        nl += (uint32_t)__popcll(ml);
        ng -= (uint32_t)__popcll(mg);
        ne += (uint32_t)__popcll(me);
    }
}

__global__ __launch_bounds__(MSB_THREADS) void msb_pivot_copyback_kernel(MsbWs ws, int L, const uint32_t *__restrict__ from_v,
                                                                         uint32_t *__restrict__ result_k, uint32_t *__restrict__ result_v,
                                                                         int f32_out, uint32_t xor_out)
{
    const unsigned long long packed = ws.level[L].packed;
    if (blockIdx.x >= (uint32_t)packed) return;
    const MsbTile T = ws.tiles[blockIdx.x];
    const MsbPivot P = ws.pivots[T.bucket];
    if (!P.flag) return;
    const MsbBucket B = ws.buckets[L & 1][T.bucket];
    const uint32_t mid_lo = B.offset + P.less, mid_hi = mid_lo + P.eq, cand_out = twiddle_out(P.cand, f32_out, xor_out);
    for (uint32_t i = threadIdx.x; i < T.valid; i += MSB_THREADS) {
        const uint32_t at = T.lo + i;
        if (at >= mid_lo && at < mid_hi) { result_k[at] = cand_out; result_v[at] = from_v[at]; }
    }
}

template <bool HAS_VALUES, bool REMAP, bool TWOUT, bool FULL, bool BIG, bool PIVOT = false>
__global__ __launch_bounds__(MSB_THREADS, HAS_VALUES ? 4 : 6) void msb_scatter_kernel(
    MsbWs ws, int L, const uint32_t *__restrict__ src_k, uint32_t *__restrict__ dst_k, const uint32_t *__restrict__ src_v,
    uint32_t *__restrict__ dst_v, DigitSel ds, int f32_out, uint32_t xor_out, int ragged_anywhere,
    uint32_t *__restrict__ result_k = nullptr, int pivot_f32_out = 0, uint32_t pivot_xor_out = 0u, uint32_t *__restrict__ result_v = nullptr)
{
    __shared__ __attribute__((aligned(16))) ScatterSmem<HAS_VALUES, REMAP> sm;
    const unsigned long long packed = ws.level[L].packed;
    auto one_tile = [&](uint32_t g) {
        const MsbTile T = ws.tiles[g];
        if (FULL ? T.valid != (uint32_t)MSB_TILE : T.valid == (uint32_t)MSB_TILE) return;
        if (PIVOT && ws.pivots[T.bucket].flag) {
            const MsbBucket B = ws.buckets[L & 1][T.bucket];
            const bool in_place = result_k == src_k;
            if constexpr (HAS_VALUES) {
                msb_pivot_tile_pairs<FULL>(sm.gbase, ws.pivots + T.bucket, B, src_k, src_v, dst_k, dst_v, in_place ? (uint32_t *)nullptr : result_k,
                                           in_place ? dst_v : result_v, T.lo, T.valid, pivot_f32_out, pivot_xor_out);
            } else {
                msb_pivot_tile<FULL>(sm.gbase, ws.pivots + T.bucket, B, src_k, dst_k, result_k, T.lo, T.valid, pivot_f32_out, pivot_xor_out,
                                     !in_place || pivot_f32_out != 0 || pivot_xor_out != 0u);
            }
            return;
        }
        if (REMAP) load_remap(ds, sm.tab);
        msb_scatter_tile<HAS_VALUES, REMAP, TWOUT, FULL, BIG>(sm, ds, ws.cursors + (size_t)T.bucket * RADIX, ws.spine + g / MSB_WAVES,
                                                              ws.stride, ws.prefix16 + (size_t)g * RADIX, src_k, dst_k, src_v, dst_v,
                                                              T.lo, T.valid, f32_out, xor_out);
    };
    if (FULL) {
        if (blockIdx.x >= (uint32_t)packed) return;
#ifdef GS_MSB_WIDE_GROUP
        one_tile(tile_of_item_wide(blockIdx.x, (uint32_t)packed));
#else
        one_tile(tile_of_item(blockIdx.x, (uint32_t)packed));
#endif
    } else if (ragged_anywhere == 1) {
        if (blockIdx.x >= (uint32_t)packed) return;
        one_tile(blockIdx.x);
    } else {
        const bool two = ragged_anywhere == 2;
        const uint32_t b = two ? blockIdx.x >> 1 : blockIdx.x;
        if (b >= (uint32_t)(packed >> 32)) return;
        const MsbBucket B = ws.buckets[L & 1][b];
        const bool short_first = B.tiles >= 2u && ws_first_tile(ws, B.offset, B.size) != (1u << ws.tile_shift);
        if (two) {
            if (blockIdx.x & 1u) { if (short_first) one_tile(B.tile_start); }
            else one_tile(B.tile_start + B.tiles - 1u);
        } else {
            one_tile(B.tile_start + B.tiles - 1u);
            if (short_first) {
                __syncthreads();
                one_tile(B.tile_start);
            }
        }
    }
}

template <bool HAS_VALUES, bool REMAP, bool TWOUT>
static void launch_scatter(const MsbWs &ws, int L, uint32_t tiles_ub, uint32_t buckets_ub, bool big, const uint32_t *sk, uint32_t *dk,
                           const uint32_t *sv, uint32_t *dv, const DigitSel &ds, int f32_out, uint32_t xor_out, hipStream_t s,
                           bool ragged_anywhere = false, uint32_t *pivot_result = nullptr, int pivot_f32_out = 0,
                           uint32_t pivot_xor_out = 0u, uint32_t *pivot_result_v = nullptr)
{
    const dim3 blk(MSB_THREADS);
    const bool two_per_bucket = !ragged_anywhere && buckets_ub <= 1024u;
    const dim3 rg(ragged_anywhere ? tiles_ub : two_per_bucket ? 2u * buckets_ub : buckets_ub);
    const int ra = ragged_anywhere ? 1 : two_per_bucket ? 2 : 0;
    if constexpr (!REMAP) {
        if (pivot_result) {
            if (big) {
                hipLaunchKernelGGL((msb_scatter_kernel<HAS_VALUES, false, TWOUT, true, true, true>), dim3(tiles_ub), blk, 0, s, ws, L, sk, dk, sv,
                                   dv, ds, f32_out, xor_out, 0, pivot_result, pivot_f32_out, pivot_xor_out, pivot_result_v);
                hipLaunchKernelGGL((msb_scatter_kernel<HAS_VALUES, false, TWOUT, false, true, true>), rg, blk, 0, s, ws, L, sk, dk, sv, dv, ds,
                                   f32_out, xor_out, ra, pivot_result, pivot_f32_out, pivot_xor_out, pivot_result_v);
            } else {
                hipLaunchKernelGGL((msb_scatter_kernel<HAS_VALUES, false, TWOUT, true, false, true>), dim3(tiles_ub), blk, 0, s, ws, L, sk, dk, sv,
                                   dv, ds, f32_out, xor_out, 0, pivot_result, pivot_f32_out, pivot_xor_out, pivot_result_v);
                hipLaunchKernelGGL((msb_scatter_kernel<HAS_VALUES, false, TWOUT, false, false, true>), rg, blk, 0, s, ws, L, sk, dk, sv, dv, ds,
                                   f32_out, xor_out, ra, pivot_result, pivot_f32_out, pivot_xor_out, pivot_result_v);
            }
            if constexpr (HAS_VALUES) {
                if (pivot_result == sk)
                    hipLaunchKernelGGL(msb_pivot_copyback_kernel, dim3(tiles_ub), blk, 0, s, ws, L, (const uint32_t *)dv, pivot_result,
                                       pivot_result_v, pivot_f32_out, pivot_xor_out);
            }
            return;
        }
    }
    if (big) {
        hipLaunchKernelGGL((msb_scatter_kernel<HAS_VALUES, REMAP, TWOUT, true, true>), dim3(tiles_ub), blk, 0, s, ws, L, sk, dk, sv, dv,
                           ds, f32_out, xor_out, 0);
        hipLaunchKernelGGL((msb_scatter_kernel<HAS_VALUES, REMAP, TWOUT, false, true>), rg, blk, 0, s, ws, L, sk, dk, sv, dv, ds,
                           f32_out, xor_out, ra);
    } else {
        hipLaunchKernelGGL((msb_scatter_kernel<HAS_VALUES, REMAP, TWOUT, true, false>), dim3(tiles_ub), blk, 0, s, ws, L, sk, dk, sv, dv,
                           ds, f32_out, xor_out, 0);
        hipLaunchKernelGGL((msb_scatter_kernel<HAS_VALUES, REMAP, TWOUT, false, false>), rg, blk, 0, s, ws, L, sk, dk, sv, dv, ds,
                           f32_out, xor_out, ra);
    }
}

__host__ __device__ constexpr int local_b1(int cap) { return cap >= 16384 ? 14 : cap >= 8192 ? 13 : cap >= 4096 ? 12 : 11; }
template <int THREADS, int KPT, bool HAS_VALUES>
struct LocalSmem {
    static constexpr int WAVES = THREADS / WAVE;
    union {
        uint32_t stage[KPT * THREADS * (HAS_VALUES ? 2 : 1)];
        uint32_t hist[1 << (local_b1(KPT * THREADS * (HAS_VALUES ? 2 : 1)) > local_b1(KPT * THREADS) ? local_b1(KPT * THREADS * (HAS_VALUES ? 2 : 1)) : local_b1(KPT * THREADS))];
        uint32_t whist[WAVES][RADIX];
    };
    uint32_t wtot[16];
};

enum { LS_ALL = 0, LS_ONEPASS = 1, LS_FLAGGED = 2, LS_DEDUPE = 3, LS_DEDUPE_ALL = 4 };
constexpr uint32_t LS_FLAG = 0x80000000u;
constexpr uint32_t LS_DONE = 0x40000000u;
constexpr uint32_t DD_BITW = 4096;
constexpr uint32_t DD_MAX = 2048;
constexpr uint32_t DD_CNT = 4096;
__host__ __device__ constexpr bool ls_is_dedupe(int mode) { return mode == LS_DEDUPE || mode == LS_DEDUPE_ALL; }
constexpr uint32_t LS_DD = 0x20000000u;

__global__ __launch_bounds__(256) void msb_task_sample_kernel(MsbWs ws, int L, const uint32_t *__restrict__ src_k, int has_values)
{
    if (!(L < 3 && (ws.level[L + 1].packed >> 32) != 0ull)) return;
    const uint32_t lane = lane_id(), wv = (blockIdx.x * blockDim.x + threadIdx.x) >> 6, nwv = (gridDim.x * blockDim.x) >> 6;
    bool flagged = false;
    for (int cls = 0; cls < MSB_NCLASS; ++cls) {
        uint32_t ntasks = ws.level[L].task_count[cls];
        if (ntasks > ws.max_tasks) ntasks = ws.max_tasks;
        const int b1 = local_b1((int)ws.caps[cls]), onepass_bits = local_b1((int)ws.caps[cls] * (has_values ? 2 : 1)) + 2;
        for (uint32_t t = wv; t < ntasks; t += nwv) {
            const MsbTask c = ws.tasks[cls][t];
            if (c.sort_bits <= (uint32_t)b1 || c.sort_bits > 16u || c.size < 64u) continue;
            const uint32_t smp = src_k[c.offset + (uint32_t)(((unsigned long long)(c.size - 8u) * (2u * (lane >> 3) + 1u)) >> 4) + (lane & 7u)];
            unsigned long long same = ~0ull;
            for (uint32_t b = 0; b < c.sort_bits; ++b) {
                const bool bit = (smp >> b) & 1u;
                const unsigned long long m = __builtin_amdgcn_ballot_w64(bit);
                same &= bit ? m : ~m;
            }
            const int mult = __popcll(same);
            uint32_t add = 0;
            if (c.sort_bits <= (uint32_t)onepass_bits && __builtin_amdgcn_ballot_w64(mult >= 3) != 0ull) { add |= LS_FLAG; flagged = true; }
            if (__popcll(__builtin_amdgcn_ballot_w64(mult >= 2)) >= 4) add |= LS_DD;
            if (add && lane == 0) ws.tasks[cls][t].pad = c.pad | add;
        }
    }
    if (flagged && lane == 0) ws.level[L].flagged = 1u;
}
#ifdef GS_EXP_LS_PHASES
constexpr uint32_t LSP_TASKS = 65536;
__device__ uint32_t gs_ls_phase_buf[3 * MSB_NCLASS * LSP_TASKS * 16];
#define LSP_PLAN (MODE == LS_ONEPASS ? 0 : ls_is_dedupe(MODE) ? 2 : 1)
#define LSP(k)                                                                                                         \
    do {                                                                                                               \
        const unsigned long long now_ = __builtin_amdgcn_s_memtime();                                                  \
        if (tid == 0 && ti < LSP_TASKS) gs_ls_phase_buf[((LSP_PLAN * MSB_NCLASS + cls) * LSP_TASKS + ti) * 16 + (k)] += (uint32_t)(now_ - tprev_); \
        tprev_ = now_;                                                                                                 \
    } while (0)
#define LSP_WAIT(what) asm volatile("s_waitcnt " what ::: "memory")
#else
#define LSP(k) do { } while (0)
#define LSP_WAIT(what) do { } while (0)
#endif
template <int THREADS, int KPT, bool HAS_VALUES, bool STABLE = false, int MODE = LS_ALL, bool PLAIN = false>
#ifndef GS_LS_WPE_512x18
#define GS_LS_WPE_512x18 4
#endif
__global__ __launch_bounds__(THREADS, (THREADS == 1024 && !(HAS_VALUES && KPT > 9)) ? 8 : (THREADS == 512 && KPT == 18 && !HAS_VALUES) ? GS_LS_WPE_512x18 : 4) void msb_local_sort_kernel(
    MsbWs ws, int L, int cls, const uint32_t *__restrict__ src_k, uint32_t *__restrict__ dst_k, const uint32_t *__restrict__ src_v,
    uint32_t *__restrict__ dst_v, int f32_in, uint32_t xor_in, int f32_out, uint32_t xor_out)
{
    constexpr int WAVES = THREADS / WAVE;
    constexpr int LOCAL_B1 = local_b1(KPT * THREADS);
    constexpr int ONEPASS_BITS = local_b1(KPT * THREADS * (HAS_VALUES ? 2 : 1)) + 2;
    static_assert(KPT * THREADS >= (1 << LOCAL_B1) && KPT * THREADS >= WAVES * RADIX, "counters must fit the staging buffer");
    __shared__ __attribute__((aligned(16))) LocalSmem<THREADS, KPT, HAS_VALUES> sm;
    uint32_t ntasks = ws.level[L].task_count[cls];
    if (ntasks > ws.max_tasks) ntasks = ws.max_tasks;
    if ((MODE == LS_FLAGGED || MODE == LS_DEDUPE) && ws.level[L].flagged == 0u) return;
    const int tid = threadIdx.x, lane = lane_id(), w = wave_id();
    uint32_t *my = sm.whist[w];
    const uint32_t wbase0 = (uint32_t)w * (WAVE * KPT) + lane;
    auto fresh = [](uint32_t x) { asm volatile("" : "+v"(x)); return x; };
    static_assert(!(STABLE && MODE != LS_ALL), "the stable sort has one plan");
    auto advance = [&](uint32_t from, MsbTask &out) {
        uint32_t t = from;
        for (; t < ntasks; t += gridDim.x) {
            const MsbTask c = ws.tasks[cls][t];
            const bool mine = MODE == LS_ALL ? (STABLE || (c.pad & LS_DONE) == 0u)
                        : MODE == LS_ONEPASS ? (c.sort_bits > (uint32_t)LOCAL_B1 && c.sort_bits <= (uint32_t)ONEPASS_BITS && (c.pad & LS_FLAG) == 0u)
                        : MODE == LS_FLAGGED ? (c.pad & (LS_FLAG | LS_DONE)) == LS_FLAG
                        : ((c.pad & LS_DD) != 0u && (MODE == LS_DEDUPE_ALL || (c.pad & LS_FLAG) != 0u) && c.sort_bits > (uint32_t)LOCAL_B1 && c.sort_bits <= 16u);
            if (mine) {
                out.offset = __builtin_amdgcn_readfirstlane(c.offset);
                out.size = __builtin_amdgcn_readfirstlane(c.size);
                out.sort_bits = __builtin_amdgcn_readfirstlane(c.sort_bits);
                out.pad = __builtin_amdgcn_readfirstlane(c.pad);
                break;
            }
            if (MODE == LS_ONEPASS && tid == 0 && (c.pad & LS_FLAG) == 0u) { ws.tasks[cls][t].pad = c.pad | LS_FLAG; ws.level[L].flagged = 1u; }
        }
        return t;
    };
    MsbTask T{};
    uint32_t ti = advance(blockIdx.x, T);
    if (ti >= ntasks) return;
    uint32_t key[KPT], val[HAS_VALUES ? KPT : 1], pos[KPT];
    auto request = [&](const MsbTask &t) {
        const uint32_t *pk = src_k + t.offset, *pv = HAS_VALUES ? src_v + t.offset : nullptr;
        const uint32_t last = t.size - 1u;
        const uint32_t wbase = fresh(wbase0);
#pragma unroll
        for (int i = 0; i < KPT; ++i) {
            const uint32_t idx = wbase + i * WAVE;
            const uint32_t off = (idx < last ? idx : last) * 4u;
            key[i] = *reinterpret_cast<const uint32_t *>(reinterpret_cast<const char *>(pk) + off);
            if (HAS_VALUES) val[i] = *reinterpret_cast<const uint32_t *>(reinterpret_cast<const char *>(pv) + off);
        }
    };
    request(T);
    [[maybe_unused]] bool zeroed = false;
    for (;;) {
#ifdef GS_EXP_LS_PHASES
        unsigned long long tprev_ = __builtin_amdgcn_s_memtime();
        const unsigned long long t0_ = tprev_, r0_ = __builtin_amdgcn_s_memrealtime();
#endif
        MsbTask Tn = T;
        const uint32_t tn = advance(ti + gridDim.x, Tn);
        const bool has_next = tn < ntasks;
        LSP(0);
        LSP_WAIT("vmcnt(0)");
        LSP(1);
        {
            const uint32_t wbase = fresh(wbase0);
#pragma unroll
            for (int i = 0; i < KPT; ++i) {
                const uint32_t idx = wbase + i * WAVE;
                const uint32_t k = PLAIN ? key[i] : twiddle_in(key[i], f32_in, xor_in);
                key[i] = (idx < T.size) ? k : 0xffffffffu;
            }
        }
        const uint32_t B = T.sort_bits;
        bool done = false;
        if constexpr (MODE == LS_ONEPASS) {
            const uint32_t nwords = (1u << B) >> 2, maskB = (1u << B) - 1u, wmask = maskB & ~3u;
            if (!zeroed) {
                for (uint32_t j = tid; j < nwords; j += THREADS) sm.hist[j] = 0;
                __syncthreads();
            }
            zeroed = false;
            LSP(2);
            uint32_t overflow = 0;
            {
                const uint32_t wbase = fresh(wbase0);
                const uint32_t ba = key[0] & maskB, bb = key[KPT / 2] & maskB;
                const bool hot = __builtin_amdgcn_ballot_w64(ba == __builtin_amdgcn_readfirstlane(ba)) == __builtin_amdgcn_ballot_w64(true) ||
                                 __builtin_amdgcn_ballot_w64(bb == __builtin_amdgcn_readfirstlane(bb)) == __builtin_amdgcn_ballot_w64(true);
                if (hot) {
#pragma unroll
                for (int i = 0; i < KPT; ++i) {
                    pos[i] = 0;
                    if (wbase + i * WAVE < T.size) {
                        const uint32_t bin = key[i] & maskB, sh = (bin & 3u) * 8u;
                        const unsigned long long act = __builtin_amdgcn_ballot_w64(true);
                        const uint32_t b0 = __builtin_amdgcn_readfirstlane(bin);
                        uint32_t r;
                        if (__builtin_amdgcn_ballot_w64(bin == b0) == act) {
                            const uint32_t lower = count_lower_mask(act), cnt = (uint32_t)__popcll(act);
                            uint32_t old = 0;
                            if (lower == 0) old = atomicAdd(&sm.hist[b0 >> 2], cnt << sh);
                            old = (__builtin_amdgcn_readfirstlane(old) >> sh) & 255u;
                            r = old + lower;
                            overflow |= (old + cnt > 255u) ? 1u : 0u;
                        } else {
                            r = (atomicAdd(&sm.hist[bin >> 2], 1u << sh) >> sh) & 255u;
                            overflow |= (r >= 255u) ? 1u : 0u;
                        }
                        pos[i] = r;
                    }
                }
                } else {
                    uint32_t rmax = 0;
#pragma unroll
                    for (int i = 0; i < KPT; ++i) {
                        const uint32_t sh = (key[i] & 3u) << 3;
                        const uint32_t inc = (wbase + i * WAVE < T.size) ? (1u << sh) : 0u;
                        const uint32_t old = atomicAdd(reinterpret_cast<uint32_t *>(reinterpret_cast<char *>(sm.hist) + (key[i] & wmask)), inc);
                        pos[i] = __builtin_amdgcn_ubfe(old, sh, 8u);
                        rmax = pos[i] > rmax ? pos[i] : rmax;
                    }
                    overflow = (rmax >= 255u) ? 1u : 0u;
                }
            }
            LSP_WAIT("lgkmcnt(0)");
            LSP(3);
            const int ovf_ = __syncthreads_or((int)overflow);
            LSP(4);
            if (!ovf_) {
                constexpr uint32_t WPT = ((1u << ONEPASS_BITS) >> 2) / THREADS;
                static_assert(WPT >= 4 && WPT % 4 == 0, "words per thread");
                static_assert(KPT * THREADS <= 65536, "a word's base must fit 16 bits");
                uint32_t rk[(KPT + 3) / 4];
#pragma unroll
                for (int j = 0; j < (KPT + 3) / 4; ++j) {
                    rk[j] = pos[4 * j];
                    if (4 * j + 1 < KPT) rk[j] |= pos[4 * j + 1] << 8;
                    if (4 * j + 2 < KPT) rk[j] |= pos[4 * j + 2] << 16;
                    if (4 * j + 3 < KPT) rk[j] |= pos[4 * j + 3] << 24;
                }
#pragma unroll
                for (int j = 0; j < (KPT + 3) / 4; ++j) asm volatile("" : "+v"(rk[j]));
#pragma unroll
                for (int i = 0; i < KPT; ++i) asm volatile("" : "+v"(key[i]));
                const bool act = (uint32_t)tid * WPT < nwords;
                uint32_t ssum = 0;
                if (act) {
#pragma unroll
                    for (uint32_t q = 0; q < WPT; q += 4) {
                        const uint4 c4 = reinterpret_cast<const uint4 *>(sm.hist)[((uint32_t)tid * WPT + q) >> 2];
                        ssum = __builtin_amdgcn_sad_u8(c4.x, 0u, ssum); ssum = __builtin_amdgcn_sad_u8(c4.y, 0u, ssum);
                        ssum = __builtin_amdgcn_sad_u8(c4.z, 0u, ssum); ssum = __builtin_amdgcn_sad_u8(c4.w, 0u, ssum);
                    }
                }
                const uint32_t inc = wave_inclusive_scan(ssum);
                if (lane == 63) sm.wtot[w] = inc;
                LSP(5);
                __syncthreads();
                LSP(6);
                const uint32_t wsv = (lane < WAVES) ? sm.wtot[lane] : 0u;
                const uint32_t wincl = wave_inclusive_scan(wsv);
                uint32_t run = (uint32_t)__shfl((int)(wincl - wsv), w, WAVE) + inc - ssum;
                uint32_t wide = 0;
                auto pack = [&](uint32_t c) {
                    wide |= c & 0xf0f0f0f0u;
                    const uint32_t nib = (c & 0xfu) | ((c >> 4) & 0xf0u) | ((c >> 8) & 0xf00u) | ((c >> 12) & 0xf000u);
                    const uint32_t e = run | (nib << 16);
                    run = __builtin_amdgcn_sad_u8(c, 0u, run);
                    return e;
                };
                if (act) {
#pragma unroll
                    for (uint32_t q = 0; q < WPT; q += 4) {
                        uint4 *p4 = reinterpret_cast<uint4 *>(sm.hist) + (((uint32_t)tid * WPT + q) >> 2);
                        const uint4 c4 = *p4;
                        uint4 e4;
                        e4.x = pack(c4.x); e4.y = pack(c4.y); e4.z = pack(c4.z); e4.w = pack(c4.w);
                        *p4 = e4;
                    }
                }
                LSP_WAIT("lgkmcnt(0)");
                LSP(7);
                const int wide_ = __syncthreads_or((int)(wide != 0u));
                LSP(8);
                if (!wide_) {
#pragma unroll
                for (int i = 0; i < KPT; ++i) {
                    const uint32_t wd = *reinterpret_cast<const uint32_t *>(reinterpret_cast<const char *>(sm.hist) + (key[i] & wmask));
                    const uint32_t low = __builtin_amdgcn_ubfe(wd >> 16, 0u, (key[i] & 3u) << 2);
                    pos[i] = ((rk[i >> 2] >> (8 * (i & 3))) & 255u) + (wd & 0xffffu) + (low & 0xfu) + ((low >> 4) & 0xfu) + (low >> 8);
                }
#pragma unroll
                for (int i = 0; i < KPT; ++i) asm volatile("" : "+v"(pos[i]));
                LSP(9);
                __syncthreads();
                LSP(10);
                {
                    const uint32_t wbase = fresh(wbase0);
#pragma unroll
                    for (int i = 0; i < KPT; ++i) {
                        const uint32_t idx = wbase + i * WAVE;
                        const uint32_t at = idx < T.size ? pos[i] : idx;
                        if (HAS_VALUES) reinterpret_cast<uint2 *>(sm.stage)[at] = make_uint2(key[i], val[i]);
                        else sm.stage[at] = key[i];
                    }
                }
                LSP_WAIT("lgkmcnt(0)");
                LSP(11);
                __syncthreads();
                LSP(12);
                done = true;
                }
            }
        }
        if constexpr (ls_is_dedupe(MODE)) {
            static_assert((uint32_t)(KPT * THREADS * (HAS_VALUES ? 2 : 1)) >= DD_BITW + DD_CNT, "the map and the counters are overlaid on the staging buffer");
            static_assert(DD_BITW % THREADS == 0 && DD_CNT % (4 * THREADS) == 0 && KPT * THREADS <= 65536 && DD_MAX * 2 <= DD_CNT, "dedupe geometry");
            const uint32_t maskB = (1u << B) - 1u;
            uint32_t *const bitw = sm.stage, *const cnt = sm.stage + DD_BITW;
            if (!zeroed) {
                for (uint32_t j = tid; j < DD_BITW + DD_CNT; j += THREADS) sm.stage[j] = 0;
                __syncthreads();
            }
            zeroed = false;
            LSP(2);
            {
                const uint32_t wbase = fresh(wbase0);
#pragma unroll
                for (int i = 0; i < KPT; ++i) {
                    if (wbase + i * WAVE < T.size) {
                        const uint32_t v = key[i] & maskB, bit = 1u << (v & 15u);
                        if (!(bitw[v >> 4] & bit)) atomicOr(&bitw[v >> 4], bit);
                    }
                }
            }
            LSP_WAIT("lgkmcnt(0)");
            LSP(3);
            __syncthreads();
            LSP(4);
            constexpr uint32_t WPT = DD_BITW / THREADS;
            static_assert(WPT % 4 == 0, "map words per thread");
            uint32_t ssum = 0;
#pragma unroll
            for (uint32_t q = 0; q < WPT; q += 4) {
                const uint4 c4 = reinterpret_cast<const uint4 *>(bitw)[((uint32_t)tid * WPT + q) >> 2];
                ssum += (uint32_t)(__popc(c4.x) + __popc(c4.y) + __popc(c4.z) + __popc(c4.w));
            }
            uint32_t inc = wave_inclusive_scan(ssum);
            if (lane == 63) sm.wtot[w] = inc;
            __syncthreads();
            uint32_t wsv = (lane < WAVES) ? sm.wtot[lane] : 0u;
            uint32_t wincl = wave_inclusive_scan(wsv);
            uint32_t run = (uint32_t)__shfl((int)(wincl - wsv), w, WAVE) + inc - ssum;
            const uint32_t distinct = (uint32_t)__shfl((int)wincl, WAVES - 1, WAVE);
            LSP(5);
            if (distinct <= DD_MAX) {
#pragma unroll
                for (uint32_t q = 0; q < WPT; q += 4) {
                    uint4 *p4 = reinterpret_cast<uint4 *>(bitw) + (((uint32_t)tid * WPT + q) >> 2);
                    uint4 c4 = *p4;
                    const uint32_t px = run, py = px + (uint32_t)__popc(c4.x), pz = py + (uint32_t)__popc(c4.y), pw = pz + (uint32_t)__popc(c4.z);
                    run = pw + (uint32_t)__popc(c4.w);
                    c4.x |= px << 16; c4.y |= py << 16; c4.z |= pz << 16; c4.w |= pw << 16;
                    *p4 = c4;
                }
                __syncthreads();
                LSP(6);
                const uint32_t rs = distinct <= 256u ? 4u : distinct <= 512u ? 3u : distinct <= 1024u ? 2u : 1u;
                const uint32_t rep = (uint32_t)lane & ((1u << rs) - 1u);
                {
                    const uint32_t wbase = fresh(wbase0);
#pragma unroll
                    for (int i = 0; i < KPT; ++i) {
                        pos[i] = 0;
                        if (wbase + i * WAVE < T.size) {
                            const uint32_t v = key[i] & maskB, wd = bitw[v >> 4];
                            const uint32_t id = (((wd >> 16) + (uint32_t)__popc(wd & ((1u << (v & 15u)) - 1u))) << rs) | rep;
#ifdef GS_EXP_DD_NOCONTEND
                            pos[i] = atomicAdd(&cnt[(id + (uint32_t)lane * 31u) & (DD_CNT - 1u)], 1u) | (id << 16);
#else
                            pos[i] = atomicAdd(&cnt[id], 1u) | (id << 16);
#endif
                        }
                    }
                }
#pragma unroll
                for (int i = 0; i < KPT; ++i) asm volatile("" : "+v"(pos[i]), "+v"(key[i]));
                LSP_WAIT("lgkmcnt(0)");
                LSP(7);
                __syncthreads();
                LSP(8);
                constexpr uint32_t CPT = DD_CNT / THREADS;
                uint32_t csum = 0;
#pragma unroll
                for (uint32_t q = 0; q < CPT; q += 4) {
                    const uint4 c4 = reinterpret_cast<const uint4 *>(cnt)[((uint32_t)tid * CPT + q) >> 2];
                    csum += c4.x + c4.y + c4.z + c4.w;
                }
                inc = wave_inclusive_scan(csum);
                if (lane == 63) sm.wtot[w] = inc;
                __syncthreads();
                wsv = (lane < WAVES) ? sm.wtot[lane] : 0u;
                wincl = wave_inclusive_scan(wsv);
                run = (uint32_t)__shfl((int)(wincl - wsv), w, WAVE) + inc - csum;
#pragma unroll
                for (uint32_t q = 0; q < CPT; q += 4) {
                    uint4 *p4 = reinterpret_cast<uint4 *>(cnt) + (((uint32_t)tid * CPT + q) >> 2);
                    const uint4 c4 = *p4;
                    uint4 e4;
                    e4.x = run; e4.y = e4.x + c4.x; e4.z = e4.y + c4.y; e4.w = e4.z + c4.z;
                    run = e4.w + c4.w;
                    *p4 = e4;
                }
                __syncthreads();
                LSP(9);
#pragma unroll
                for (int i = 0; i < KPT; ++i) pos[i] = cnt[pos[i] >> 16] + (pos[i] & 0xffffu);
#pragma unroll
                for (int i = 0; i < KPT; ++i) asm volatile("" : "+v"(pos[i]));
                LSP(10);
                __syncthreads();
                {
                    const uint32_t wbase = fresh(wbase0);
#pragma unroll
                    for (int i = 0; i < KPT; ++i) {
                        const uint32_t idx = wbase + i * WAVE;
                        const uint32_t at = idx < T.size ? pos[i] : idx;
                        if (HAS_VALUES) reinterpret_cast<uint2 *>(sm.stage)[at] = make_uint2(key[i], val[i]);
                        else sm.stage[at] = key[i];
                    }
                }
                LSP_WAIT("lgkmcnt(0)");
                LSP(11);
                __syncthreads();
                LSP(12);
                done = true;
            } else {
                __syncthreads();
            }
        }
        if constexpr (MODE == LS_ONEPASS) {
            if (!done && tid == 0) { ws.tasks[cls][ti].pad = T.pad | LS_FLAG; ws.level[L].flagged = 1u; }
        } else if constexpr (ls_is_dedupe(MODE)) {
            if (done && tid == 0) ws.tasks[cls][ti].pad = T.pad | LS_DONE;
        } else {
        done = true;
        const uint32_t b1 = STABLE ? 0u : (B < (uint32_t)LOCAL_B1 ? B : (uint32_t)LOCAL_B1);
        bool in_regs = STABLE;
        if (!STABLE) {
            const uint32_t nbins = 1u << b1, mask1 = nbins - 1u;
            for (uint32_t j = tid; j < nbins; j += THREADS) sm.hist[j] = 0;
            __syncthreads();
            LSP(2);
            {
                const uint32_t wbase = fresh(wbase0);
#pragma unroll
                for (int i = 0; i < KPT; ++i) {
                    pos[i] = 0;
                    if (wbase + i * WAVE < T.size) {
                        const uint32_t d = key[i] & mask1;
                        const unsigned long long act = __builtin_amdgcn_ballot_w64(true);
                        const uint32_t d0 = __builtin_amdgcn_readfirstlane(d);
                        if (__builtin_amdgcn_ballot_w64(d == d0) == act) {
                            const uint32_t lower = count_lower_mask(act);
                            uint32_t base = 0;
                            if (lower == 0) base = atomicAdd(&sm.hist[d0], (uint32_t)__popcll(act));
                            pos[i] = __builtin_amdgcn_readfirstlane(base) + lower;
                        } else {
                            pos[i] = atomicAdd(&sm.hist[d], 1u);
                        }
                    }
                }
            }
#pragma unroll
            for (int i = 0; i < KPT; ++i) asm volatile("" : "+v"(pos[i]), "+v"(key[i]));
            LSP_WAIT("lgkmcnt(0)");
            LSP(3);
            __syncthreads();
            LSP(4);
            constexpr uint32_t IPT = (1u << LOCAL_B1) / THREADS;
            const bool act = (uint32_t)tid * IPT < nbins;
            uint32_t ssum = 0;
            if (act) {
#pragma unroll
                for (uint32_t q = 0; q < IPT; q += 4) {
                    const uint4 c4 = reinterpret_cast<const uint4 *>(sm.hist)[((uint32_t)tid * IPT + q) >> 2];
                    ssum += c4.x + c4.y + c4.z + c4.w;
                }
            }
            const uint32_t inc = wave_inclusive_scan(ssum);
            if (lane == 63) sm.wtot[w] = inc;
            __syncthreads();
            const uint32_t wsv = (lane < WAVES) ? sm.wtot[lane] : 0u;
            const uint32_t wincl = wave_inclusive_scan(wsv);
            uint32_t run = (uint32_t)__shfl((int)(wincl - wsv), w, WAVE) + inc - ssum;
            if (act) {
#pragma unroll
                for (uint32_t q = 0; q < IPT; q += 4) {
                    uint4 *p4 = reinterpret_cast<uint4 *>(sm.hist) + (((uint32_t)tid * IPT + q) >> 2);
                    const uint4 c4 = *p4;
                    uint4 e4;
                    e4.x = run; e4.y = e4.x + c4.x; e4.z = e4.y + c4.y; e4.w = e4.z + c4.z;
                    run = e4.w + c4.w;
                    *p4 = e4;
                }
            }
            LSP_WAIT("lgkmcnt(0)");
            LSP(5);
            __syncthreads();
            LSP(6);
#pragma unroll
            for (int i = 0; i < KPT; ++i) pos[i] += sm.hist[key[i] & mask1];
#pragma unroll
            for (int i = 0; i < KPT; ++i) asm volatile("" : "+v"(pos[i]));
            LSP(7);
            __syncthreads();
            LSP(8);
            {
                const uint32_t wbase = fresh(wbase0);
#pragma unroll
                for (int i = 0; i < KPT; ++i) {
                    if (wbase + i * WAVE < T.size) {
                        if (HAS_VALUES) reinterpret_cast<uint2 *>(sm.stage)[pos[i]] = make_uint2(key[i], val[i]);
                        else sm.stage[pos[i]] = key[i];
                    }
                }
            }
            LSP_WAIT("lgkmcnt(0)");
            LSP(9);
            __syncthreads();
            LSP(10);
        }
        uint32_t rem = B - b1, np = (rem + 7u) / 8u, shift = b1 + (STABLE ? T.pad : 0u);
        while (rem) {
            const uint32_t b = (rem + np - 1u) / np, nd = 1u << b;
            const uint32_t wbase = fresh(wbase0);
            if (!in_regs) {
#pragma unroll
            for (int i = 0; i < KPT; ++i) {
                const uint32_t idx = wbase + i * WAVE;
                if (HAS_VALUES) {
                    const uint2 kv = reinterpret_cast<const uint2 *>(sm.stage)[idx];
                    key[i] = kv.x; val[i] = kv.y;
                } else {
                    key[i] = sm.stage[idx];
                }
                if (idx >= T.size) key[i] = 0xffffffffu;
            }
            __syncthreads();
            }
            in_regs = false;
#pragma unroll
            for (int i = lane; i < RADIX; i += WAVE) my[i] = 0;
            auto rank_pass = [&](auto width) {
                uint32_t d_prev = 0, plo = 0, phi = 0;
#pragma unroll
                for (int i = 0; i <= KPT; ++i) {
                    uint32_t d_cur = 0, clo = 0, chi = 0;
                    if (i < KPT) {
                        d_cur = __builtin_amdgcn_ubfe(key[i], shift, b);
                        constexpr int MB = decltype(width)::value;
                        if (MB == 2) match_digit2(d_cur, clo, chi);
                        else if (MB == 4) match_digit4(d_cur, clo, chi);
                        else if (MB == 5) match_digit5(d_cur, clo, chi);
                        else match_digit(d_cur, clo, chi);
                    }
                    if (i > 0) {
                        const uint32_t lower = count_lower(plo, phi);
                        pos[i - 1] = my[d_prev] + lower;
                        if (lower == 0)
                            __hip_atomic_fetch_add(&my[d_prev], (uint32_t)(__popc(plo) + __popc(phi)), __ATOMIC_RELAXED,
                                                   __HIP_MEMORY_SCOPE_WAVEFRONT);
                    }
                    d_prev = d_cur; plo = clo; phi = chi;
                }
            };
            if (b <= 2u) rank_pass(std::integral_constant<int, 2>{});
            else if (b <= 4u) rank_pass(std::integral_constant<int, 4>{});
            else if (b <= 5u) rank_pass(std::integral_constant<int, 5>{});
            else rank_pass(std::integral_constant<int, 8>{});
#pragma unroll
            for (int i = 0; i < KPT; ++i) asm volatile("" : "+v"(pos[i]), "+v"(key[i]));
            __syncthreads();
            uint32_t tot = 0, inc = 0;
            if ((uint32_t)tid < nd) {
#pragma unroll
                for (int j = 0; j < WAVES; ++j) {
                    const uint32_t c = sm.whist[j][tid];
                    sm.whist[j][tid] = tot;
                    tot += c;
                }
            }
            if (tid < RADIX) {
                inc = wave_inclusive_scan(tot);
                if (lane == 63) sm.wtot[w] = inc;
            }
            __syncthreads();
            if ((uint32_t)tid < nd) {
                uint32_t ex = inc - tot;
                if (w > 0) ex += sm.wtot[0];
                if (w > 1) ex += sm.wtot[1];
                if (w > 2) ex += sm.wtot[2];
#pragma unroll
                for (int j = 0; j < WAVES; ++j) sm.whist[j][tid] += ex;
            }
            __syncthreads();
#pragma unroll
            for (int i = 0; i < KPT; ++i) pos[i] += my[__builtin_amdgcn_ubfe(key[i], shift, b)];
#pragma unroll
            for (int i = 0; i < KPT; ++i) asm volatile("" : "+v"(pos[i]));
            __syncthreads();
#pragma unroll
            for (int i = 0; i < KPT; ++i) {
                if (HAS_VALUES) reinterpret_cast<uint2 *>(sm.stage)[pos[i]] = make_uint2(key[i], val[i]);
                else sm.stage[pos[i]] = key[i];
            }
            __syncthreads();
            shift += b; rem -= b; --np;
        }
        LSP(11);
        }
        if (has_next) request(Tn);
        LSP(13);
        constexpr uint32_t CAP = (uint32_t)(KPT * THREADS);
        const uint32_t ssh = (T.size + (T.offset & 63u) <= CAP) ? (T.offset & 63u) : 0u;
        if (done) {
        uint32_t *qk = dst_k + T.offset, *qv = HAS_VALUES ? dst_v + T.offset : nullptr;
        if (HAS_VALUES) {
            for (uint32_t jj = tid; jj < T.size + ssh; jj += THREADS) {
                const uint32_t j = jj - ssh;
                if (j >= T.size) continue;
                const uint2 kv = reinterpret_cast<const uint2 *>(sm.stage)[j];
                __builtin_nontemporal_store(PLAIN ? kv.x : twiddle_out(kv.x, f32_out, xor_out), &qk[j]);
                __builtin_nontemporal_store(kv.y, &qv[j]);
            }
        } else {
            const uint32_t t0 = fresh((uint32_t)tid);
            const uint32_t jb = t0 - ssh, s0 = jb < CAP ? jb : jb + CAP;
            pos[0] = sm.stage[s0];
#pragma unroll
            for (int i = 1; i < KPT; ++i) pos[i] = sm.stage[jb + i * THREADS];
            if constexpr ((MODE == LS_ONEPASS || ls_is_dedupe(MODE)) && !HAS_VALUES) {
#pragma unroll
                for (int i = 1; i < KPT; ++i) sm.stage[jb + i * THREADS] = 0;
                sm.stage[s0] = 0;
                zeroed = true;
            }
#pragma unroll
            for (int i = 0; i < KPT; ++i) {
                const uint32_t j = jb + i * THREADS;
                if (j < T.size) __builtin_nontemporal_store(PLAIN ? pos[i] : twiddle_out(pos[i], f32_out, xor_out), reinterpret_cast<uint32_t *>(reinterpret_cast<char *>(qk) + j * 4u));
            }
        }
        }
        LSP(14);
        __syncthreads();
#ifdef GS_EXP_LS_PHASES
        if (tid == 0 && ti < LSP_TASKS) {
            gs_ls_phase_buf[((LSP_PLAN * MSB_NCLASS + cls) * LSP_TASKS + ti) * 16 + 15] += (uint32_t)(__builtin_amdgcn_s_memtime() - t0_);
            (void)r0_;
        }
#endif
        if (!has_next) break;
        T = Tn; ti = tn;
    }
}


template <bool VEC>
__global__ __launch_bounds__(MSB_THREADS) void shard_hist_kernel(const uint32_t *__restrict__ keys, uint64_t n, int bits,
                                                                 unsigned long long *__restrict__ hist, int f32_in,
                                                                 uint32_t xor_in)
{
    __shared__ uint32_t lh[1 << SHARD_MAX_BITS];
    const uint32_t nb = 1u << bits;
    for (uint32_t i = threadIdx.x; i < nb; i += MSB_THREADS) lh[i] = 0;
    __syncthreads();
    const int rshift = 32 - bits;
    auto count = [&](uint32_t k) { atomicAdd(&lh[twiddle_in(k, f32_in, xor_in) >> rshift], 1u); };
    const uint64_t stride = (uint64_t)gridDim.x * MSB_THREADS;
    uint64_t done = 0;
    if (VEC) {
        const uint4 *k4 = reinterpret_cast<const uint4 *>(keys);
        const uint64_t nvec = n >> 2;
        uint64_t v = (uint64_t)blockIdx.x * MSB_THREADS + threadIdx.x;
        for (; v + 3 * stride < nvec; v += 4 * stride) {
            const uint4 a = k4[v], b = k4[v + stride], c = k4[v + 2 * stride], d = k4[v + 3 * stride];
            count(a.x); count(a.y); count(a.z); count(a.w);
            count(b.x); count(b.y); count(b.z); count(b.w);
            count(c.x); count(c.y); count(c.z); count(c.w);
            count(d.x); count(d.y); count(d.z); count(d.w);
        }
        for (; v < nvec; v += stride) { const uint4 a = k4[v]; count(a.x); count(a.y); count(a.z); count(a.w); }
        done = nvec << 2;
    }
    for (uint64_t i = done + (uint64_t)blockIdx.x * MSB_THREADS + threadIdx.x; i < n; i += stride) count(keys[i]);
    __syncthreads();
    for (uint32_t i = threadIdx.x; i < nb; i += MSB_THREADS)
        if (lh[i]) atomicAdd(&hist[i], (unsigned long long)lh[i]);
}

__global__ void shard_counts_kernel(const uint32_t *__restrict__ row, uint32_t n, int num_ranks, unsigned long long *__restrict__ counts)
{
    const int r = threadIdx.x;
    if (r < num_ranks) counts[r] = (unsigned long long)((r + 1 < RADIX ? row[r + 1] : n) - row[r]);
}


static inline bool onepass_possible(int min_bits, int b1, int onepass_bits)
{
    return (min_bits > b1 && min_bits <= onepass_bits) || (min_bits + 8 > b1 && min_bits + 8 <= onepass_bits);
}
template <bool HAS_VALUES, bool STABLE = false>
static void launch_local_sorts(const MsbWs &ws, int L, uint32_t bound, const uint32_t *sk, uint32_t *dk, const uint32_t *sv,
                               uint32_t *dv, int f32_in, uint32_t xor_in, int f32_out, uint32_t xor_out, hipStream_t s,
                               int min_bits = 0, uint64_t num_items = 0, const uint32_t *known_tasks = nullptr, bool maybe_skew = true)
{
    KernelTimer kt(GS_K_MSB_LOCAL_SORT, s);
    auto grid_of = [&](int c) {
        uint64_t b = bound;
        if (known_tasks && known_tasks[c] < b) b = known_tasks[c];
        if (num_items && c > 0) {
            const uint64_t lim = num_items / msb_class_cap(c - 1) + RADIX;
            if (lim < b) b = lim;
        }
#ifndef MSB_LS_MAX_GRID
#define MSB_LS_MAX_GRID MSB_MAX_GRID
#endif
        return (uint32_t)(b < MSB_LS_MAX_GRID ? (b ? b : 1) : MSB_LS_MAX_GRID);
    };
#define GS_LS1P(C, HV, M, P) hipLaunchKernelGGL((msb_local_sort_kernel<msb_class_threads(C), msb_class_kpt(C), HV, STABLE, M, P>), dim3(grid_of(C)), \
                                               dim3(msb_class_threads(C)), 0, s, ws, L, C, sk, dk, sv, dv, f32_in, xor_in, f32_out, xor_out)
#define GS_LS1(C, HV, M) GS_LS1P(C, HV, M, false)
#define GS_LSDD(C, HV, M) hipLaunchKernelGGL((msb_local_sort_kernel<msb_class_threads(C), msb_class_kpt(C), HV, STABLE, M, false>),                \
                                             dim3(grid_of(C)), dim3(msb_class_threads(C)), 0, s, ws, L, C, sk, dk, sv, dv,                             \
                                             f32_in, xor_in, f32_out, xor_out)
    const bool plain = !f32_in && !xor_in && !f32_out && !xor_out;
    static const bool dedupe_on = [] { const char *e = getenv("GS_MSB_DEDUPE"); return !(e && e[0] == '0'); }();
#define GS_LS(C, HV)                                                                                                  \
    do {                                                                                                              \
        constexpr bool DD = !STABLE && msb_class_cap(C) * (HV ? 2u : 1u) >= DD_BITW + DD_CNT;                           \
        const bool dd = DD && dedupe_on && maybe_skew && L < 3 && onepass_possible(min_bits, local_b1((int)msb_class_cap(C)), 16);          \
        if constexpr (STABLE) { GS_LS1(C, HV, LS_ALL); }                                                              \
        else if (!onepass_possible(min_bits, local_b1((int)msb_class_cap(C)), local_b1((int)msb_class_cap(C) * (HV ? 2 : 1)) + 2)) \
            { if constexpr (DD) { if (dd) GS_LSDD(C, HV, LS_DEDUPE_ALL); } GS_LS1(C, HV, LS_ALL); }                    \
        else { if (plain) GS_LS1P(C, HV, LS_ONEPASS, true); else GS_LS1(C, HV, LS_ONEPASS);                           \
               if constexpr (DD) { if (dd) GS_LSDD(C, HV, LS_DEDUPE); } GS_LS1(C, HV, LS_FLAGGED); }                   \
    } while (0)
    auto wanted = [&](int c) { return !known_tasks || known_tasks[c] != 0u; };
    if constexpr (!STABLE) {
        uint64_t waves = bound;
        if (known_tasks) waves = (uint64_t)known_tasks[0] + known_tasks[1] + known_tasks[2] + known_tasks[3];
        if (L < 3 && waves && maybe_skew) {
            const uint32_t blocks = (uint32_t)(waves / 4 + 1 < 2048 ? waves / 4 + 1 : 2048);
            hipLaunchKernelGGL(msb_task_sample_kernel, dim3(blocks), dim3(256), 0, s, ws, L, sk, HAS_VALUES ? 1 : 0);
        }
    }
    if (wanted(0)) GS_LS(0, HAS_VALUES);
    if (wanted(1)) GS_LS(1, HAS_VALUES);
    if (wanted(2)) GS_LS(2, HAS_VALUES);
    if ((!HAS_VALUES || GS_PAIR_CLASSES > 3) && wanted(3)) GS_LS(3, HAS_VALUES);
#undef GS_LS
#undef GS_LS1
#undef GS_LS1P
#undef GS_LSDD
}

int msb_local_sorts_in_place(MsbLevel *level, MsbTask *const tasks[MSB_NCLASS], uint32_t max_tasks, uint32_t bound, uint32_t *keys,
                             int sort_bits, uint64_t num_items, int f32_out, uint32_t xor_out, hipStream_t s, const uint32_t *known_tasks)
{
    MsbWs ws{};
    ws.level = level;
    for (int c = 0; c < MSB_NCLASS; ++c) { ws.tasks[c] = tasks[c]; ws.caps[c] = msb_class_cap(c); }
    ws.max_tasks = max_tasks;
    ws.tile_shift = 13u;
    ws.key_bits = 32u;
    launch_local_sorts<false>(ws, 0, bound, keys, keys, nullptr, nullptr, 0, 0u, f32_out, xor_out, s, sort_bits, num_items, known_tasks);
    return (int)hipGetLastError();
}

static inline bool msb_pivot_enabled()
{
    static const bool on = [] { const char *e = getenv("GS_MSB_PIVOT"); return !(e && e[0] == '0'); }();
    return on;
}

__global__ void msb_peek_kernel(MsbWs ws, int L, unsigned long long *mailbox)
{
    mailbox[0] = ws.level[L].packed;
    mailbox[1] = ((unsigned long long)ws.level[L - 1].task_count[1] << 32) | ws.level[L - 1].task_count[0];
    mailbox[2] = ((unsigned long long)ws.level[L - 1].task_count[3] << 32) | ws.level[L - 1].task_count[2];
    __threadfence_system();
}
struct MsbPeek {
    unsigned long long *host = nullptr, *dev = nullptr;
    hipEvent_t ev = nullptr;
    int device = -1;
    bool armed = false;
};
static bool msb_peek_enabled()
{
    static const bool on = [] { const char *e = getenv("GS_MSB_PEEK"); return !(e && e[0] == '0'); }();
    return on;
}
constexpr int MSB_PEEK_DEVICES = 16;
struct MsbPeekTable {
    MsbPeek slot[MSB_PEEK_DEVICES];
    ~MsbPeekTable()
    {
        for (MsbPeek &pk : slot) {
            if (pk.ev) (void)hipEventDestroy(pk.ev);
            if (pk.host) (void)hipHostFree(pk.host);
        }
    }
};
static MsbPeek *msb_peek_get(hipStream_t s)
{
    if (!msb_peek_enabled()) return nullptr;
    hipStreamCaptureStatus cs = hipStreamCaptureStatusNone;
    if (hipStreamIsCapturing(s, &cs) != hipSuccess || cs != hipStreamCaptureStatusNone) { (void)hipGetLastError(); return nullptr; }
    thread_local MsbPeekTable table;
    int dev = -1;
    if (hipGetDevice(&dev) != hipSuccess || dev < 0 || dev >= MSB_PEEK_DEVICES) { (void)hipGetLastError(); return nullptr; }
    MsbPeek &pk = table.slot[dev];
    if (pk.device != dev) {
        void *h = nullptr, *d = nullptr;
        if (hipHostMalloc(&h, 64, hipHostMallocMapped | hipHostMallocPortable) != hipSuccess ||
            hipHostGetDevicePointer(&d, h, 0) != hipSuccess ||
            hipEventCreateWithFlags(&pk.ev, hipEventDisableTiming) != hipSuccess) {
            (void)hipGetLastError();
            if (h) (void)hipHostFree(h);
            pk.ev = nullptr;
            return nullptr;
        }
        pk.host = (unsigned long long *)h; pk.dev = (unsigned long long *)d; pk.device = dev;
    }
    if (pk.armed) { (void)hipEventSynchronize(pk.ev); (void)hipGetLastError(); }
    pk.armed = false;
    return &pk;
}

static void msb_peek_arm(MsbPeek *pk, const MsbWs &ws, int L, hipStream_t s)
{
    if (!pk) return;
    hipLaunchKernelGGL(msb_peek_kernel, dim3(1), dim3(1), 0, s, ws, L, pk->dev);
    pk->armed = hipEventRecord(pk->ev, s) == hipSuccess;
    if (!pk->armed) (void)hipGetLastError();
}
struct MsbLook { bool ok = false; uint32_t buckets = 0, tiles = 0, tasks[MSB_NCLASS] = {0, 0, 0, 0}; };
static MsbLook msb_peek_wait(MsbPeek *pk)
{
    MsbLook lk;
    if (!pk || !pk->armed) return lk;
    pk->armed = false;
    if (hipEventSynchronize(pk->ev) != hipSuccess) { (void)hipGetLastError(); return lk; }
    const volatile unsigned long long *m = pk->host;
    const unsigned long long a = m[0], b = m[1], c = m[2];
    lk.ok = true;
    lk.buckets = (uint32_t)(a >> 32); lk.tiles = (uint32_t)a;
    lk.tasks[0] = (uint32_t)b; lk.tasks[1] = (uint32_t)(b >> 32); lk.tasks[2] = (uint32_t)c; lk.tasks[3] = (uint32_t)(c >> 32);
    return lk;
}

static void msb_run_levels(const MsbWs &ws, uint64_t num_items, bool pairs, uint32_t npieces, uint32_t *const buf_k[2],
                           uint32_t *const buf_v[2], const PassParams &tw, hipStream_t s, int stop_level = 99,
                           bool allow_pivot = true)
{
    const int nclass = msb_num_classes(pairs);
    const uint32_t tiles_all = (uint32_t)((num_items + MSB_TILE - 1) / MSB_TILE);
    const uint32_t max_tasks_lvl = ws.max_tasks;
    uint32_t *d_keys = buf_k[0], *d_vals = buf_v[0];
    MsbPeek *peek = (stop_level == 99 && (npieces == 0 || getenv("GS_MSB_PEEK_FINISH"))) ? msb_peek_get(s) : nullptr;
    uint32_t known_b = 0, known_tiles = 0;
    bool known = false;
    for (int L = 1; L <= 3; ++L) {
        const int shift = 24 - 8 * L;
        const DigitSel dsel{shift, nullptr, 0, 0, 0u, 8, 0};
        uint32_t *sk = buf_k[L & 1], *dk = buf_k[(L + 1) & 1];
        uint32_t *sv = buf_v[L & 1], *dv = buf_v[(L + 1) & 1];
        const bool in_pieces = npieces != 0 && L == 1;
        const bool pivot = allow_pivot && msb_pivot_enabled() && !in_pieces && L <= 2;
        uint32_t max_b = (L == 1) ? (uint32_t)RADIX : ws.max_buckets;
        uint32_t max_tiles = tiles_all + (in_pieces ? 2u * npieces : max_b + tiles_all / MSB_ALIGN_MIN_TILES + 1u);
        if (known && L >= 2) {
            if (known_b < max_b) max_b = known_b;
            if (known_tiles < max_tiles) max_tiles = known_tiles;
            known = false;
        }
        const bool last = (L == 3);
        { KernelTimer kt(GS_K_MSB_HISTOGRAM, s);
          if (in_pieces) {
              hipLaunchKernelGGL(msb_expand_pieces_kernel, dim3(npieces < 4096u ? npieces : 4096u), dim3(256), 0, s, ws, npieces);
          } else {
              const uint32_t eg = max_b < 4096u ? max_b : 4096u;
              hipLaunchKernelGGL(msb_expand_kernel, dim3(eg), dim3(256), 0, s, ws, L, pivot ? (const uint32_t *)sk : (const uint32_t *)nullptr);
          }
          const uint32_t hg_ub = max_tiles / MSB_WAVES + 1;
          const uint32_t hg = hg_ub < MSB_MAX_GRID ? hg_ub : MSB_MAX_GRID;
          if (pivot) hipLaunchKernelGGL((msb_upsweep_kernel<false, true>), dim3(hg), dim3(MSB_THREADS), 0, s, ws, L, (const uint32_t *)sk, dsel);
          else hipLaunchKernelGGL((msb_upsweep_kernel<false, false>), dim3(hg), dim3(MSB_THREADS), 0, s, ws, L, (const uint32_t *)sk, dsel);
          hipLaunchKernelGGL(msb_scan_kernel, dim3(RADIX), dim3(1024), 0, s, ws, L); }
        { KernelTimer kt(GS_K_MSB_CLASSIFY, s);
          const uint32_t cg = max_b < 4096u ? max_b : 4096u;
          if (last) hipLaunchKernelGGL((msb_classify_kernel<true, false>), dim3(cg), dim3(256), 0, s, ws, L, (const uint32_t *)nullptr, nclass);
          else if (pivot) hipLaunchKernelGGL((msb_classify_kernel<false, true>), dim3(cg), dim3(256), 0, s, ws, L, (const uint32_t *)nullptr, nclass);
          else hipLaunchKernelGGL((msb_classify_kernel<false, false>), dim3(cg), dim3(256), 0, s, ws, L, (const uint32_t *)nullptr, nclass); }
        if (L == stop_level) return;
        if (!last) msb_peek_arm(peek, ws, L + 1, s);
        { KernelTimer kt(GS_K_MSB_PARTITION, s);
          const bool big = num_items > (1ull << 30);
          const uint32_t *svc = pairs ? (const uint32_t *)sv : (const uint32_t *)nullptr;
          uint32_t *dvc = pairs ? dv : (uint32_t *)nullptr;
#define GS_SC(HV, TW) launch_scatter<HV, false, TW>(ws, L, max_tiles, max_b, big, (const uint32_t *)sk, dk, svc, dvc, dsel, tw.f32_out, tw.xor_out, s, in_pieces, \
                                                  pivot ? d_keys : (uint32_t *)nullptr, tw.f32_out, tw.xor_out, pivot && pairs ? d_vals : (uint32_t *)nullptr)
          if (pairs) { if (last) GS_SC(true, true); else GS_SC(true, false); }
          else { if (last) GS_SC(false, true); else GS_SC(false, false); }
#undef GS_SC
        }
        if (!last) {
            const MsbLook lk = msb_peek_wait(peek);
            const uint32_t tb = (uint64_t)max_b * RADIX < (uint64_t)max_tasks_lvl ? max_b * (uint32_t)RADIX : max_tasks_lvl;
            const uint32_t *kt_ = lk.ok ? lk.tasks : nullptr;
            const bool skew = !(lk.ok && lk.buckets == 0);
            if (pairs) launch_local_sorts<true>(ws, L, tb, dk, d_keys, dv, d_vals, 0, 0u, tw.f32_out, tw.xor_out, s, 24 - 8 * L, num_items, kt_, skew);
            else launch_local_sorts<false>(ws, L, tb, dk, d_keys, nullptr, nullptr, 0, 0u, tw.f32_out, tw.xor_out, s, 24 - 8 * L, num_items, kt_, skew);
            if (lk.ok) {
                if (lk.buckets == 0) return;
                known = true; known_b = lk.buckets; known_tiles = lk.tiles;
            }
        }
    }
}

__global__ void msb_small_task_kernel(MsbLevel *level, MsbTask *task, uint32_t n, int cls, uint32_t bits, uint32_t shift0)
{
    if (threadIdx.x == 0) {
        MsbLevel z{};
        z.task_count[cls] = 1;
        level[0] = z;
        task[0] = MsbTask{0u, n, bits, shift0};
    }
}

uint32_t small_sort_capacity(bool pairs) { return msb_class_cap(msb_num_classes(pairs) - 1); }

int small_stable_sort(void *scratch, size_t scratch_bytes, const uint32_t *kin, uint32_t *kout, const uint32_t *vin, uint32_t *vout,
                      uint32_t n, int begin_bit, int end_bit, int f32_in, uint32_t xor_in, int f32_out, uint32_t xor_out,
                      hipStream_t s)
{
    const bool pairs = vin != nullptr;
    if (n == 0 || n > small_sort_capacity(pairs) || scratch_bytes < 256 + sizeof(MsbTask)) return hipErrorInvalidValue;
    int cls = 0;
    while (msb_class_cap(cls) < n) ++cls;
    MsbWs ws{};
    ws.level = (MsbLevel *)scratch;
    for (int c = 0; c < MSB_NCLASS; ++c) ws.tasks[c] = (MsbTask *)((char *)scratch + 256);
    ws.max_tasks = 1;
    KernelTimer kt(GS_K_MSB_LOCAL_SORT, s);
    hipLaunchKernelGGL(msb_small_task_kernel, dim3(1), dim3(64), 0, s, ws.level, ws.tasks[cls], n, cls,
                       (uint32_t)(end_bit - begin_bit), (uint32_t)begin_bit);
#define GS_SM(C, HV) hipLaunchKernelGGL((msb_local_sort_kernel<msb_class_threads(C), msb_class_kpt(C), HV, true, LS_ALL>), dim3(1), \
                                        dim3(msb_class_threads(C)), 0, s, ws, 0, C, kin, kout, vin, vout, f32_in, xor_in, f32_out, xor_out)
    if (pairs) { if (cls == 0) GS_SM(0, true); else if (cls == 1) GS_SM(1, true); else if (cls == 2 || GS_PAIR_CLASSES < 4) GS_SM(2, true); else GS_SM(3, true); }
    else { if (cls == 0) GS_SM(0, false); else if (cls == 1) GS_SM(1, false); else if (cls == 2) GS_SM(2, false); else GS_SM(3, false); }
#undef GS_SM
    return (int)hipGetLastError();
}


constexpr uint32_t SEG_TINY = 256;
__global__ __launch_bounds__(256) void seg_classify_kernel(MsbWs ws, const int *__restrict__ seg_begin,
                                                           const int *__restrict__ seg_end, uint32_t nseg, int nclass,
                                                           uint32_t sort_bits, uint32_t shift0, uint32_t num_items,
                                                           uint32_t tiny_cap = 0)
{
    constexpr int NW = 4, SPT = 4, NLIST = NW + MSB_NCLASS;
    __shared__ uint32_t s_cnt[NLIST], s_base[NLIST];
    const uint32_t cap_max = ws.caps[nclass - 1];
    const int tid = threadIdx.x;
    for (uint32_t base = blockIdx.x * (256u * SPT); base < nseg; base += gridDim.x * (256u * SPT)) {
        if (tid < NLIST) s_cnt[tid] = 0;
        __syncthreads();
        uint32_t b[SPT], size[SPT], off[NLIST], cnt[NLIST];
        int list[SPT];
#pragma unroll
        for (int q = 0; q < NLIST; ++q) cnt[q] = 0;
#pragma unroll
        for (int j = 0; j < SPT; ++j) {
            const uint32_t sg = base + (uint32_t)tid * SPT + j;
            b[j] = 0; size[j] = 0; list[j] = -1;
            if (sg < nseg) {
                int lo = seg_begin[sg], hi = seg_end[sg];
                if (lo < 0) lo = 0;
                if (hi > (int)num_items) hi = (int)num_items;
                if (hi > lo) { b[j] = (uint32_t)lo; size[j] = (uint32_t)(hi - lo); }
            }
            const uint32_t sz = size[j];
            if (sz != 0 && tiny_cap != 0 && sz <= 4u * tiny_cap) list[j] = sz <= (uint32_t)WAVE ? 3 : sz <= tiny_cap ? 0 : sz <= 2u * tiny_cap ? 1 : 2;
            else if (sz != 0 && sz <= cap_max) { int c = 0; while (ws.caps[c] < sz) ++c; list[j] = NW + c; }
            else if (sz > cap_max) {
                const uint32_t tiles = ws_tiles_of_at(ws, b[j], sz);
                const unsigned long long old = atomicAdd(&ws.level[1].packed, (1ull << 32) | tiles);
                if ((uint32_t)(old >> 32) < ws.max_buckets) ws.buckets[1][(uint32_t)(old >> 32)] = MsbBucket{b[j], sz, (uint32_t)old, tiles};
                else MSB_OVERFLOW(ws);
            }
#pragma unroll
            for (int q = 0; q < NLIST; ++q) cnt[q] += list[j] == q ? 1u : 0u;
        }
#pragma unroll
        for (int q = 0; q < NLIST; ++q) off[q] = cnt[q] ? atomicAdd(&s_cnt[q], cnt[q]) : 0u;
        __syncthreads();
        if (tid < NLIST && s_cnt[tid] != 0u)
            s_base[tid] = atomicAdd(tid < NW ? &ws.level[2].task_count[tid] : &ws.level[1].task_count[tid - NW], s_cnt[tid]);
        __syncthreads();
#pragma unroll
        for (int j = 0; j < SPT; ++j) {
#pragma unroll
            for (int q = 0; q < NLIST; ++q) {
                if (list[j] != q) continue;
                const uint32_t at = s_base[q] + off[q]++;
                if (at < ws.max_tasks) {
                    if (q < NW) ws.tasks[q][ws.max_tasks - 1u - at] = MsbTask{b[j], size[j], sort_bits, shift0};
                    else ws.tasks[q - NW][at] = MsbTask{b[j], size[j], sort_bits, shift0};
                } else {
                    MSB_OVERFLOW(ws);
                }
            }
        }
        __syncthreads();
    }
}


template <bool HAS_VALUES, int WKPT >
__global__ __launch_bounds__(256) void seg_wave_sort_kernel(MsbWs ws, const uint32_t *__restrict__ src_k, uint32_t *__restrict__ dst_k,
                                                            const uint32_t *__restrict__ src_v, uint32_t *__restrict__ dst_v, int f32_in,
                                                            uint32_t xor_in, int f32_out, uint32_t xor_out)
{
    typedef uint32_t K;
    constexpr int FW = 0;
#include "gs_seg_wave_body.inc"
}

template <bool HAS_VALUES>
__global__ __launch_bounds__(256) void seg_wave4_sort_kernel(MsbWs ws, const uint32_t *__restrict__ src_k, uint32_t *__restrict__ dst_k,
                                                             const uint32_t *__restrict__ src_v, uint32_t *__restrict__ dst_v, int f32_in,
                                                             uint32_t xor_in, int f32_out, uint32_t xor_out)
{
    typedef uint32_t K;
    constexpr int FW = 0;
#include "gs_seg_wave4_body.inc"
}

template <bool HAS_VALUES, int WKPT, typename K, int FW>
__global__ __launch_bounds__(256) void seg_wave_sort_narrow_kernel(MsbWs ws, const K *__restrict__ src_k, K *__restrict__ dst_k,
                                                                   const uint32_t *__restrict__ src_v, uint32_t *__restrict__ dst_v, int f32_in,
                                                                   uint32_t xor_in, int f32_out, uint32_t xor_out)
{
#include "gs_seg_wave_body.inc"
}
template <bool HAS_VALUES, typename K, int FW>
__global__ __launch_bounds__(256) void seg_wave4_sort_narrow_kernel(MsbWs ws, const K *__restrict__ src_k, K *__restrict__ dst_k,
                                                                    const uint32_t *__restrict__ src_v, uint32_t *__restrict__ dst_v, int f32_in,
                                                                    uint32_t xor_in, int f32_out, uint32_t xor_out)
{
#include "gs_seg_wave4_body.inc"
}

constexpr int MW_THREADS = 512, MW_WAVES = MW_THREADS / WAVE, MW_KPT = 8, MW_TILE = MW_THREADS * MW_KPT;
constexpr uint32_t MW_CAP = 8192;
struct MwNoVal {};

template <typename K> __device__ __forceinline__ K mw_tw_in(K k, int f, uint64_t x)
{
    if constexpr (sizeof(K) == 8) { if (f) k ^= (uint64_t)((int64_t)k >> 63) | 0x8000000000000000ull; return k ^ x; }
    else return twiddle_in((uint32_t)k, f, (uint32_t)x);
}
template <typename K> __device__ __forceinline__ K mw_tw_out(K k, int f, uint64_t x)
{
    if constexpr (sizeof(K) == 8) { k ^= x; if (f) k ^= ~(uint64_t)((int64_t)k >> 63) | 0x8000000000000000ull; return k; }
// ... 1205 lines not shown
```

### gpu-sort_amd/csrc/gs_msb_tasks.hpp

```cpp
#pragma once

#include "gs_host.hpp"

namespace gs {

constexpr int MSB_NCLASS = 4;
#ifndef GS_LS3_THREADS
#define GS_LS3_THREADS 1024
#define GS_LS3_KPT 17
#endif
#ifndef GS_LS2_THREADS
#define GS_LS2_THREADS 512
#define GS_LS2_KPT 18
#endif
#ifndef GS_LS1_THREADS
#define GS_LS1_THREADS 512
#define GS_LS1_KPT 9
#endif
#ifndef GS_LS0_THREADS
#define GS_LS0_THREADS 512
#define GS_LS0_KPT 4
#endif
__host__ __device__ constexpr int msb_class_threads(int c) { return c == 0 ? GS_LS0_THREADS : c == 1 ? GS_LS1_THREADS : c == 2 ? GS_LS2_THREADS : GS_LS3_THREADS; }
__host__ __device__ constexpr int msb_class_kpt(int c) { return c == 0 ? GS_LS0_KPT : c == 1 ? GS_LS1_KPT : c == 2 ? GS_LS2_KPT : GS_LS3_KPT; }
__host__ __device__ constexpr uint32_t msb_class_cap(int c) { return (uint32_t)(msb_class_kpt(c) * msb_class_threads(c)); }
struct MsbTask { uint32_t offset, size, sort_bits, pad; };
struct MsbLevel {
    unsigned long long packed;
    uint32_t task_count[MSB_NCLASS];
    uint32_t flagged;
    uint32_t overflow;
    unsigned long long unused1;
    unsigned long long keys;
    unsigned long long unused2;
    uint32_t census_blocks, pad;
};

int msb_local_sorts_in_place(MsbLevel *level, MsbTask *const tasks[MSB_NCLASS], uint32_t max_tasks, uint32_t bound, uint32_t *keys,
                             int sort_bits, uint64_t num_items, int f32_out, uint32_t xor_out, hipStream_t s,
                             const uint32_t *known_tasks = nullptr);

}
```

### include/gpusort.h

```cpp
#ifndef GPUSORT_H_
#define GPUSORT_H_

#include <stddef.h>
#include <stdint.h>

#ifdef __cplusplus
extern "C" {
#endif

#define GS_VERSION 100

enum gs_key_type {
    GS_KEY_U32 = 0,
    GS_KEY_I32 = 1,
    GS_KEY_F32 = 2,
    GS_KEY_U64 = 3,
    GS_KEY_I64 = 4,
    GS_KEY_F64 = 5,
    GS_KEY_U8 = 6,
    GS_KEY_I8 = 7,
    GS_KEY_U16 = 8,
    GS_KEY_I16 = 9,
    GS_KEY_F16 = 10,
    GS_KEY_BF16 = 11,
    GS_KEY_F8 = 12
};

int         gs_version(void);
const char *gs_error_string(int err);


size_t gs_lsb_temp_bytes(uint64_t num_items, int has_values);

int gs_lsb_sort_u32(void *d_temp, size_t temp_bytes,
                    uint32_t *d_keys[2], uint32_t *d_vals[2], int *selector,
                    uint64_t num_items, int begin_bit, int end_bit,
                    int descending, int key_type, void *stream);

size_t gs_lsb_copy_temp_bytes(uint64_t num_items, int has_values);
int gs_lsb_sort_copy_u32(void *d_temp, size_t temp_bytes,
                         const uint32_t *d_keys_in, uint32_t *d_keys_out,
                         const uint32_t *d_vals_in, uint32_t *d_vals_out,
                         uint64_t num_items, int begin_bit, int end_bit,
                         int descending, int key_type, void *stream);

size_t gs_lsb_wide_temp_bytes(uint64_t num_items, int key_bytes, int val_bytes);
int gs_lsb_sort_wide(void *d_temp, size_t temp_bytes, void *d_keys[2], void *d_vals[2],
                     int *selector, uint64_t num_items, int key_bytes, int val_bytes,
                     int begin_bit, int end_bit, int descending, int key_type, void *stream);

void gs_lsb_geometry(uint64_t num_items, int has_values, uint32_t *grid, uint32_t *tile,
                     uint32_t *tiles_per_chunk);
int  gs_lsb_workspace_layout(void *d_temp, uint64_t num_items, uint32_t **d_spine,
                             uint32_t **d_totals, uint16_t **d_prefix16);
int  gs_lsb_pipe_status(void *d_temp, uint64_t num_items, uint32_t *h_status, void *stream);
int  gs_lsb_plan_status(void *d_temp, uint64_t num_items, uint32_t out[8], void *stream);
int  gs_lsb_plan_cursor_status(void *d_temp, uint64_t num_items, uint32_t out[4], void *stream);
int  gs_lsb_plan_peek_status(uint32_t out[4]);
int  gs_lsb_plan_look_only(void *d_temp, const void *d_keys, void *d_alt, uint64_t num_items,
                           int key_type, int descending, void *stream);
int  gs_lsb_plan_layout(uint64_t num_items, uint64_t out[4]);
int  gs_lsb_upsweep_u32(void *d_temp, size_t temp_bytes, const uint32_t *d_keys_in,
                        uint64_t num_items, int shift, int bits, int descending,
                        int key_type_in, void *stream);
int  gs_lsb_scan_spine(void *d_temp, size_t temp_bytes, uint64_t num_items, void *stream);
int  gs_lsb_downsweep_u32(void *d_temp, size_t temp_bytes,
                          const uint32_t *d_keys_in, uint32_t *d_keys_out,
                          const uint32_t *d_vals_in, uint32_t *d_vals_out,
                          uint64_t num_items, int shift, int bits, int descending,
                          int key_type_in, int key_type_out, void *stream);

size_t gs_lsb_any_temp_bytes(uint64_t num_items, int key_type, int val_bytes);
int gs_lsb_sort_any(void *d_temp, size_t temp_bytes, const void *d_keys_in, void *d_keys_out,
                    const void *d_vals_in, void *d_vals_out, uint64_t num_items, int key_type, int val_bytes,
                    int begin_bit, int end_bit, int descending, void *stream);

size_t gs_lsb_narrow_temp_bytes(uint64_t num_items, int key_type, int val_bytes);
int gs_lsb_sort_narrow(void *d_temp, size_t temp_bytes, const void *d_keys_in, void *d_keys_out,
                       const void *d_vals_in, void *d_vals_out, uint64_t num_items, int key_type, int val_bytes,
                       int begin_bit, int end_bit, int descending, void *stream);
uint32_t gs_lsb_narrow_tile(int key_type, int val_bytes);


size_t gs_msb_temp_bytes(uint64_t num_items, int has_values);

int gs_msb_sort_u32(void *d_temp, size_t temp_bytes,
                    uint32_t *d_keys, uint32_t *d_vals, uint64_t num_items,
                    uint32_t *d_keys_alt, uint32_t *d_vals_alt,
                    uint32_t **d_sorted_keys, uint32_t **d_sorted_vals,
                    int key_type, void *stream, int synchronize);

size_t gs_msb_wide_temp_bytes(uint64_t num_items, int key_bytes, int val_bytes);
int gs_msb_sort_wide(void *d_temp, size_t temp_bytes, void *d_keys, void *d_vals, uint64_t num_items,
                     void *d_keys_alt, void *d_vals_alt, int key_bytes, int val_bytes,
                     void **d_sorted_keys, void **d_sorted_vals, int key_type, void *stream, int synchronize);

size_t gs_msb_large_temp_bytes(uint64_t num_items, int has_values);
int    gs_msb_sort_large_u32(void *d_temp, size_t temp_bytes,
                             uint32_t *d_keys, uint32_t *d_vals, uint64_t num_items,
                             uint32_t *d_keys_alt, uint32_t *d_vals_alt,
                             int key_type, void *stream, int synchronize);

size_t gs_msb_large_wide_temp_bytes(uint64_t num_items, int key_bytes, int val_bytes);
int    gs_msb_sort_large_wide(void *d_temp, size_t temp_bytes, void *d_keys, void *d_vals, uint64_t num_items,
                              void *d_keys_alt, void *d_vals_alt, int key_bytes, int val_bytes, int key_type,
                              void *stream, int synchronize);

size_t gs_lsb_large_temp_bytes(uint64_t num_items, int key_bytes, int val_bytes);
int    gs_lsb_sort_large(void *d_temp, size_t temp_bytes, void *d_keys[2], void *d_vals[2], int *selector,
                         uint64_t num_items, int key_bytes, int val_bytes, int begin_bit, int end_bit,
                         int descending, int key_type, void *stream);

size_t gs_lsb_narrow_large_temp_bytes(uint64_t num_items, int key_type, int val_bytes);
int    gs_lsb_sort_narrow_large(void *d_temp, size_t temp_bytes, const void *d_keys_in, void *d_keys_out,
                                const void *d_vals_in, void *d_vals_out, uint64_t num_items, int key_type,
                                int val_bytes, int begin_bit, int end_bit, int descending, void *stream);

size_t gs_topk_temp_bytes(uint64_t num_items, uint64_t k, int has_values);
int    gs_topk_u32(void *d_temp, size_t temp_bytes,
                   const uint32_t *d_keys_in, const uint32_t *d_vals_in,
                   uint32_t *d_keys_out, uint32_t *d_vals_out,
                   uint64_t num_items, uint64_t k, int descending, int key_type, void *stream);
int    gs_topk_status(void *d_temp, uint64_t num_items, uint64_t k, int has_values, uint32_t out[8], void *stream);

size_t gs_topk_u16_temp_bytes(uint64_t num_items, uint64_t k, int has_values);
int    gs_topk_u16(void *d_temp, size_t temp_bytes,
                   const uint16_t *d_keys_in, const uint32_t *d_vals_in,
                   uint16_t *d_keys_out, uint32_t *d_vals_out,
                   uint64_t num_items, uint64_t k, int descending, int key_type, void *stream);
int    gs_topk_u16_status(void *d_temp, uint64_t num_items, uint64_t k, int has_values, uint32_t out[8], void *stream);

size_t   gs_topk_rows_temp_bytes(uint64_t num_rows, uint64_t num_cols, uint64_t k, int has_values);
int      gs_topk_rows_u32(void *d_temp, size_t temp_bytes,
                          const uint32_t *d_keys_in, const uint32_t *d_vals_in,
                          uint32_t *d_keys_out, uint32_t *d_vals_out,
                          uint64_t num_rows, uint64_t num_cols, uint64_t row_stride, uint64_t k,
                          int descending, int key_type, void *stream);
uint32_t gs_topk_rows_max_k(void);
int      gs_topk_rows_plan(uint64_t num_rows, uint64_t num_cols, uint64_t k, int has_values, uint32_t out[8]);

size_t   gs_topk_rows_u16_temp_bytes(uint64_t num_rows, uint64_t num_cols, uint64_t k, int has_values);
int      gs_topk_rows_u16(void *d_temp, size_t temp_bytes,
                          const uint16_t *d_keys_in, const uint32_t *d_vals_in,
                          uint16_t *d_keys_out, uint32_t *d_vals_out,
                          uint64_t num_rows, uint64_t num_cols, uint64_t row_stride, uint64_t k,
                          int descending, int key_type, void *stream);

size_t gs_topk_segmented_temp_bytes(uint64_t num_items, uint32_t num_segments, uint64_t k, int has_values);
int    gs_topk_segmented_u32(void *d_temp, size_t temp_bytes,
                             const uint32_t *d_keys_in, const uint32_t *d_vals_in,
                             uint32_t *d_keys_out, uint32_t *d_vals_out, uint32_t *d_counts_out,
                             uint64_t num_items, uint32_t num_segments,
                             const int32_t *d_begin_offsets, const int32_t *d_end_offsets,
                             uint64_t k, int descending, int key_type, void *stream);
int    gs_topk_segmented_plan(uint64_t num_items, uint32_t num_segments, uint64_t k, int has_values, uint32_t out[8]);
int    gs_topk_segmented_status(void *d_temp, uint64_t num_items, uint32_t num_segments, uint64_t k, int has_values,
                                uint32_t out[8], void *stream);

typedef struct gs_msb_level_census {
    uint64_t buckets;
    uint64_t tiles;
    uint64_t keys;
    uint64_t pivot_buckets;
    uint64_t pivot_keys;
    uint64_t task_keys;
    uint32_t tasks[4];
    uint32_t flagged;
    uint32_t overflow;
} gs_msb_level_census;
int gs_msb_census(void *d_temp, uint64_t num_items, int has_values, gs_msb_level_census out[4], void *stream);
int gs_msb_wide_census(void *d_temp, uint64_t num_items, int key_bytes, int val_bytes, gs_msb_level_census out[8], void *stream);
void gs_msb_capacities(uint64_t num_items, int has_values, uint32_t *max_buckets, uint32_t *max_tasks, uint32_t *max_tiles);

int gs_msb_classify_upto(void *d_temp, size_t temp_bytes, uint32_t *d_keys, uint32_t *d_keys_alt, uint64_t num_items,
                         int stop_level, int flags, void *stream);
int gs_msb_read_lists(void *d_temp, uint64_t num_items, int has_values, int level,
                      uint32_t *h_buckets, uint32_t max_buckets, uint32_t *n_buckets,
                      uint32_t *h_tasks[4], uint32_t max_tasks, uint32_t n_tasks[4], void *stream);


size_t gs_segmented_temp_bytes(uint64_t num_items, int has_values, uint32_t num_segments);
int gs_segmented_sort_u32(void *d_temp, size_t temp_bytes, uint32_t *d_keys[2], uint32_t *d_vals[2],
                          int *selector, uint64_t num_items, uint32_t num_segments,
                          const int32_t *d_begin_offsets, const int32_t *d_end_offsets, int begin_bit,
                          int end_bit, int descending, int key_type, void *stream);

size_t gs_segmented_wide_temp_bytes(uint64_t num_items, int key_bytes, int val_bytes, uint32_t num_segments);
int gs_segmented_sort_wide(void *d_temp, size_t temp_bytes, void *d_keys[2], void *d_vals[2], int *selector,
                           uint64_t num_items, uint32_t num_segments, const int32_t *d_begin_offsets,
                           const int32_t *d_end_offsets, int key_bytes, int val_bytes, int begin_bit, int end_bit,
                           int descending, int key_type, void *stream);

size_t gs_segmented_narrow_temp_bytes(uint64_t num_items, int key_type, int val_bytes, uint32_t num_segments);
int gs_segmented_sort_narrow(void *d_temp, size_t temp_bytes, void *d_keys[2], void *d_vals[2], int *selector,
                             uint64_t num_items, uint32_t num_segments, const int32_t *d_begin_offsets,
                             const int32_t *d_end_offsets, int key_type, int val_bytes, int begin_bit, int end_bit,
                             int descending, void *stream);
uint32_t gs_segmented_narrow_cap(int key_type, int val_bytes);

int gs_msb_first_pass_u32(void *d_temp, size_t temp_bytes, const uint32_t *d_keys_in,
                          uint32_t *d_keys_out, const uint32_t *d_vals_in, uint32_t *d_vals_out,
                          uint64_t num_items, int key_type, uint64_t *d_bucket_counts, void *stream);
size_t gs_msb_finish_temp_bytes(uint64_t num_items, int has_values, int num_src);
int gs_msb_finish_u32(void *d_temp, size_t temp_bytes, uint32_t *d_keys, uint32_t *d_vals,
                      uint32_t *d_keys_out, uint32_t *d_vals_out, uint64_t num_items,
                      const uint64_t *h_piece_counts, int num_src, int key_type, void *stream,
                      int synchronize);

int gs_shard_histogram_u32(const uint32_t *d_keys, uint64_t num_items, int bits,
                           uint64_t *d_hist, int key_type, void *stream);
int gs_shard_partition_u32(void *d_temp, size_t temp_bytes,
                           const uint32_t *d_keys_in, uint32_t *d_keys_out,
                           const uint32_t *d_vals_in, uint32_t *d_vals_out,
                           uint64_t num_items, int bits, const uint8_t *d_dest_of_bin,
                           int num_ranks, const uint64_t *d_bin_hist, uint64_t *d_counts,
                           int key_type, void *stream);

enum gs_gen_kind { GS_GEN_UNIFORM = 0, GS_GEN_ZIPF = 1, GS_GEN_ENTROPY_AND = 2, GS_GEN_ENUMERATED = 3 };
int gs_generate_u32(uint32_t *d_out, uint64_t num_items, int kind, uint64_t seed,
                    uint64_t start_index, int level, void *stream);

int gs_check_sorted_u32(const uint32_t *d_keys, uint64_t num_items, int descending,
                        uint64_t *d_result, void *stream);
int gs_check_pairs_enumerated_u32(const uint32_t *d_keys_in, const uint32_t *d_keys_sorted,
                                  const uint32_t *d_vals, uint64_t num_items,
                                  uint64_t *d_result, void *stream);
int gs_check_sorted_u64(const uint64_t *d_keys, uint64_t num_items, int key_type, uint64_t *d_result, void *stream);
int gs_check_pairs_enumerated_wide(const void *d_keys_in, const void *d_keys_sorted, const uint64_t *d_vals,
                                   uint64_t num_items, int key_bytes, uint64_t *d_result, void *stream);
int gs_check_sorted_stable(const void *d_keys_sorted, const uint64_t *d_rowids, uint64_t num_items, int key_bytes,
                           int key_type, int begin_bit, int end_bit, int descending, uint64_t *d_result, void *stream);

enum gs_kernel_id {
    GS_K_LSB_UPSWEEP = 0, GS_K_LSB_SCAN = 1, GS_K_LSB_DOWNSWEEP = 2,
    GS_K_MSB_HISTOGRAM = 3, GS_K_MSB_CLASSIFY = 4, GS_K_MSB_PARTITION = 5, GS_K_MSB_LOCAL_SORT = 6,
    GS_K_SHARD = 7, GS_K_OTHER = 8,
    GS_K_LSB_PASS = 9,
    GS_K_COUNT = 10
};
typedef struct gs_profile gs_profile;
gs_profile *gs_profile_create(void);
void        gs_profile_destroy(gs_profile *p);
void        gs_profile_begin(gs_profile *p);
void        gs_profile_end(void);
int         gs_profile_read(gs_profile *p, double total_ms[GS_K_COUNT], uint64_t launches[GS_K_COUNT]);
const char *gs_kernel_name(int kernel_id);

#ifdef __cplusplus
}
#endif
#endif
```

Before: 161.1 Gkeys/s.

## Store only low 16 bits of keys in planned cursor scatter pass

```diff
diff --git a/gpu-sort_amd/_lib.py b/gpu-sort_amd/_lib.py
--- a/gpu-sort_amd/_lib.py
+++ b/gpu-sort_amd/_lib.py
@@ -35,6 +35,7 @@
     "gs_lsb_pipe_status": (i32, [vp, u64, C.POINTER(C.c_uint32), vp]),
     "gs_lsb_plan_status": (i32, [vp, u64, C.POINTER(C.c_uint32), vp]),
     "gs_lsb_plan_cursor_status": (i32, [vp, u64, C.POINTER(C.c_uint32), vp]),
+    "gs_lsb_plan_narrow_status": (i32, [vp, u64, C.POINTER(C.c_uint32), vp]),
     "gs_lsb_plan_peek_status": (i32, [C.POINTER(C.c_uint32)]),
     "gs_lsb_plan_look_only": (i32, [vp, vp, vp, u64, i32, i32, vp]),
     "gs_lsb_plan_layout": (i32, [u64, C.POINTER(C.c_uint64)]),
diff --git a/gpu-sort_amd/csrc/gs_lsb_downsweep.inc b/gpu-sort_amd/csrc/gs_lsb_downsweep.inc
--- a/gpu-sort_amd/csrc/gs_lsb_downsweep.inc
+++ b/gpu-sort_amd/csrc/gs_lsb_downsweep.inc
@@ -36,7 +36,7 @@
 
 constexpr uint32_t PIPE_SPIN_LIMIT = 1u << 18;
 
-template <bool HAS_VALUES, bool TAIL, int TW, bool BIG, bool PIPE, bool OFF64 = false, bool CURSOR = false>
+template <bool HAS_VALUES, bool TAIL, int TW, bool BIG, bool PIPE, bool OFF64 = false, bool CURSOR = false, bool NARROW = false>
 __device__ __forceinline__ void downsweep_tile(DownsweepSmem<HAS_VALUES, OFF64> &sm, const uint32_t t,
     const uint32_t *__restrict__ keys_in, uint32_t *__restrict__ keys_out, const uint32_t *__restrict__ vals_in,
     uint32_t *__restrict__ vals_out, const uint32_t *__restrict__ spine, const uint16_t *__restrict__ prefix16,
@@ -45,6 +45,7 @@
     uint32_t *__restrict__ cursor = nullptr, uint32_t *__restrict__ irr = nullptr, const uint32_t irr_cap = 0u)
 {
     static_assert(!CURSOR || (!HAS_VALUES && !TAIL && !PIPE && !OFF64), "cursor mode: full tiles of keys-only three-launch passes");
+    static_assert(!NARROW || (CURSOR && TW == 0), "16-bit stores: cursor mode, keys in twiddled form");
 #ifdef GS_EXP_ALLWAVE_KEYS
     constexpr bool ALLWAVE = true;
 #else
@@ -326,7 +327,7 @@
             for (int q = 0; q < 4; ++q) {
                 const int d = q * WAVE + lane;
                 const uint32_t g = claim[q] - sm.gbase[d];
-                sm.gbase[d] = BIG ? g : g << 2;
+                sm.gbase[d] = BIG ? g : g << (NARROW ? 1 : 2);
             }
         }
     }
@@ -356,6 +357,18 @@
 #define GS_EXP_STORE_PRIO 3
 #endif
     if (!HAS_VALUES) __builtin_amdgcn_s_setprio(GS_EXP_STORE_PRIO);
+    if constexpr (NARROW) {
+        uint32_t nslot0 = ((uint32_t)w * (WAVE * LSB_KPT) + (uint32_t)lane) * 2u;
+        asm volatile("" : "+v"(nslot0));
+#pragma unroll
+        for (int i = 0; i < LSB_KPT; ++i) {
+            const uint32_t slot = (uint32_t)w * (WAVE * LSB_KPT) + i * WAVE + lane;
+            const uint32_t k = sm.stage[slot];
+            const uint32_t g = sm.gbase[digit(k)];
+            if (BIG) reinterpret_cast<uint16_t *>(keys_out)[(uint32_t)(g + slot)] = (uint16_t)k;
+            else *reinterpret_cast<uint16_t *>(reinterpret_cast<char *>(keys_out) + (uint32_t)(g + nslot0 + (uint32_t)(i * WAVE) * 2u)) = (uint16_t)k;
+        }
+    } else {
 #pragma unroll
     for (int i = 0; i < LSB_KPT; ++i) {
         const uint32_t slot = (uint32_t)w * (WAVE * LSB_KPT) + i * WAVE + lane;
@@ -383,6 +396,7 @@
             }
         }
     }
+    }
     GS_PHASE(7);
 #ifdef GS_EXP_DRAIN
     asm volatile("s_waitcnt vmcnt(0)" ::: "memory");
diff --git a/gpu-sort_amd/csrc/gs_lsb_plan.hip b/gpu-sort_amd/csrc/gs_lsb_plan.hip
--- a/gpu-sort_amd/csrc/gs_lsb_plan.hip
+++ b/gpu-sort_amd/csrc/gs_lsb_plan.hip
@@ -44,6 +44,7 @@
     uint32_t offsets[PLAN_GROUPS + 1];
     uint32_t cursor_mode;
 };
+constexpr uint32_t PLAN_MODE_CURSOR = 1u, PLAN_MODE_NARROW = 2u;
 static_assert(1 + PLAN_IRR_CAP <= PLAN_LOOK_MAX_GRID, "the list of straddling tiles fits the look's flags");
 static_assert(sizeof(MsbLevel) == 64 && offsetof(PlanBlock, level) == 64, "plan block layout");
 
@@ -274,7 +275,7 @@
             plan->ups_skip[q] = planned && q != 1 ? 1u : 0u;
         }
         plan->offsets[PLAN_GROUPS] = n;
-        plan->cursor_mode = planned && cursor_on ? 1u : 0u;
+        plan->cursor_mode = planned ? cursor_on : 0u;
     }
 }
 
@@ -308,7 +309,7 @@
     if (cls >= 0) {
         uint32_t idx = plan->blk_class_base[blockIdx.x][cls] + lower;
         for (int j = 0; j < w; ++j) idx += wcnt[j][cls];
-        if (idx < lists.cap[cls]) lists.tasks[cls][idx] = MsbTask{off, size, (uint32_t)PLAN_SORT_BITS, 0u};
+        if (idx < lists.cap[cls]) lists.tasks[cls][idx] = MsbTask{off, size, (uint32_t)PLAN_SORT_BITS, g};
     }
 }
 
@@ -345,13 +346,13 @@
 __global__ __launch_bounds__(LSB_THREADS, GS_EXP_UPS_WPE) void lsb_plan_upsweep2_kernel(const uint32_t *__restrict__ keys,
                                                                         uint32_t *__restrict__ spine, uint16_t *__restrict__ prefix16,
                                                                         PlanBlock *__restrict__ plan, uint32_t *__restrict__ cursor,
-                                                                        PassParams p)
+                                                                        PassParams p, uint32_t narrow)
 {
     __shared__ UpsweepSmem<false, false> sm;
     if (plan->cursor_mode) {
         if (blockIdx.x == 0 && threadIdx.x == 0) plan->irr[0] = 0;
         for (uint32_t i = blockIdx.x * (uint32_t)LSB_THREADS + threadIdx.x; i < PLAN_GROUPS; i += gridDim.x * (uint32_t)LSB_THREADS)
-            cursor[i] = plan->offsets[((i & (uint32_t)(RADIX - 1)) << RADIX_BITS) | (i >> RADIX_BITS)];
+            cursor[i] = plan->offsets[((i & (uint32_t)(RADIX - 1)) << RADIX_BITS) | (i >> RADIX_BITS)] << narrow;
         return;
     }
     const uint32_t sh = plan->shift[1];
@@ -360,7 +361,7 @@
     upsweep_chunk<false, false, PLAIN>(sm, keys, chunk_of_block(blockIdx.x, p.grid), spine, prefix16, nullptr, nullptr, p, PipeParams{});
 }
 
-template <bool TAIL, bool BIG>
+template <bool TAIL, bool BIG, bool NARROW = false>
 __global__ __launch_bounds__(LSB_THREADS, 6) void lsb_plan_scatter2_kernel(const uint32_t *__restrict__ keys_in, uint32_t *__restrict__ keys_out,
                                                                            const uint32_t *__restrict__ totals, const uint32_t *__restrict__ spine,
                                                                            const uint16_t *__restrict__ prefix16, PlanBlock *__restrict__ plan,
@@ -380,7 +381,7 @@
         if (blockIdx.x >= full_tiles) return;
         const uint32_t t = tile_of_item_wide(blockIdx.x, full_tiles);
         if (mode)
-            downsweep_tile<false, false, 0, BIG, false, false, true>(sm, t, keys_in, keys_out, nullptr, nullptr, spine, prefix16, totals, p,
+            downsweep_tile<false, false, 0, BIG, false, false, true, NARROW>(sm, t, keys_in, keys_out, nullptr, nullptr, spine, prefix16, totals, p,
                                                                      nullptr, 0u, nullptr, threadIdx.x, nullptr, cursor, plan->irr, PLAN_IRR_CAP);
         else
             downsweep_tile<false, false, 0, BIG, false>(sm, t, keys_in, keys_out, nullptr, nullptr, spine, prefix16, totals, p, nullptr, 0u,
@@ -390,7 +391,7 @@
 
 __global__ __launch_bounds__(LSB_THREADS) void lsb_plan_irregular_kernel(const uint32_t *__restrict__ keys_in, uint32_t *__restrict__ keys_out,
                                                                          const PlanBlock *__restrict__ plan, uint32_t *__restrict__ cursor,
-                                                                         uint32_t n)
+                                                                         uint32_t n, uint32_t narrow)
 {
     if (!plan->cursor_mode) return;
     const uint32_t full_tiles = n / (uint32_t)LSB_TILE;
@@ -426,7 +427,11 @@
             rest &= ~m;
         }
         if ((rest >> lane) & 1ull) at = __hip_atomic_fetch_add(cursor + c, 1u, __ATOMIC_RELAXED, __HIP_MEMORY_SCOPE_AGENT);
-        if (have && at < n) keys_out[at] = k;
+        if (narrow) {
+            if (have && at < 2u * n) reinterpret_cast<uint16_t *>(keys_out)[at] = (uint16_t)k;
+        } else if (have && at < n) {
+            keys_out[at] = k;
+        }
     }
 }
 
@@ -441,6 +446,15 @@
 {
     static const bool v = [] { const char *e = getenv("GS_LSB_PLAN_SCATTER2"); return !(e && strcmp(e, "stable") == 0); }();
     return v;
+}
+static inline bool plan_narrow_enabled()
+{
+    static const bool wide = [] { const char *e = getenv("GS_LSB_PLAN_SCATTER2"); return e && strcmp(e, "cursor32") == 0; }();
+    return plan_cursor_enabled() && !wide;
+}
+static inline uint32_t plan_mode_bits()
+{
+    return !plan_cursor_enabled() ? 0u : plan_narrow_enabled() ? (PLAN_MODE_CURSOR | PLAN_MODE_NARROW) : PLAN_MODE_CURSOR;
 }
 constexpr uint64_t PLAN_N_MAX = (uint64_t)PLAN_GROUPS * 16620u;
 constexpr uint64_t PLAN_N_FLOOR = 65536;
@@ -518,6 +532,17 @@
     return (int)hipGetLastError();
 }
 
+static void launch_plan_scatter2(const uint32_t *kin, uint32_t *kout, const LsbWorkspace &ws, PlanBlock *plan, uint32_t *cursor,
+                                 const PassParams &p, hipStream_t s)
+{
+    const bool big = p.n > (1u << 30), narrow = plan_narrow_enabled();
+#define GS_PS2(BIG_, NARROW_) hipLaunchKernelGGL((lsb_plan_scatter2_kernel<false, BIG_, NARROW_>), dim3(p.ds_grid), dim3(LSB_THREADS), 0, s, kin, \
+                                                 kout, ws.totals, ws.spine, ws.prefix16, plan, cursor, p)
+    if (big) { if (narrow) GS_PS2(true, true); else GS_PS2(true, false); }
+    else { if (narrow) GS_PS2(false, true); else GS_PS2(false, false); }
+#undef GS_PS2
+}
+
 static int lsb_plan_slot2(const uint32_t *kin, uint32_t *kout, const LsbWorkspace &ws, PlanBlock *plan, uint32_t *cursor,
                           const PassParams &p, hipStream_t s)
 {
@@ -525,19 +550,13 @@
     if ((char *)cursor < (char *)ws.prefix16) return hipErrorInvalidValue;
     {
         KernelTimer kt(GS_K_OTHER, s);
-        hipLaunchKernelGGL(lsb_plan_upsweep2_kernel<true>, dim3(p.grid), dim3(LSB_THREADS), 0, s, kin, ws.spine, ws.prefix16, plan, cursor, p);
+        hipLaunchKernelGGL(lsb_plan_upsweep2_kernel<true>, dim3(p.grid), dim3(LSB_THREADS), 0, s, kin, ws.spine, ws.prefix16, plan, cursor, p,
+                           plan_narrow_enabled() ? 1u : 0u);
     }
     if (const int e = lsb_scan_as(ws.spine, ws.totals, p.grid, s, GS_K_LSB_SCAN)) return e;
     {
         KernelTimer kt(GS_K_LSB_DOWNSWEEP, s);
-        if (p.n >= (uint32_t)LSB_TILE) {
-            if (p.n > (1u << 30))
-                hipLaunchKernelGGL((lsb_plan_scatter2_kernel<false, true>), dim3(p.ds_grid), dim3(LSB_THREADS), 0, s, kin, kout, ws.totals,
-                                   ws.spine, ws.prefix16, plan, cursor, p);
-            else
-                hipLaunchKernelGGL((lsb_plan_scatter2_kernel<false, false>), dim3(p.ds_grid), dim3(LSB_THREADS), 0, s, kin, kout, ws.totals,
-                                   ws.spine, ws.prefix16, plan, cursor, p);
-        }
+        if (p.n >= (uint32_t)LSB_TILE) launch_plan_scatter2(kin, kout, ws, plan, cursor, p, s);
         if (p.n % (uint32_t)LSB_TILE)
             hipLaunchKernelGGL((lsb_plan_scatter2_kernel<true, true>), dim3(1), dim3(LSB_THREADS), 0, s, kin, kout, ws.totals,
                                (const uint32_t *)nullptr, (const uint16_t *)nullptr, plan, cursor, p);
@@ -545,7 +564,7 @@
     {
         KernelTimer kt(GS_K_OTHER, s);
         hipLaunchKernelGGL(lsb_plan_irregular_kernel, dim3(PLAN_IRR_CAP + (p.n % (uint32_t)LSB_TILE ? 1u : 0u)), dim3(LSB_THREADS), 0, s, kin,
-                           kout, plan, cursor, p.n);
+                           kout, plan, cursor, p.n, plan_narrow_enabled() ? 1u : 0u);
     }
     return (int)hipGetLastError();
 }
@@ -559,7 +578,7 @@
     hipLaunchKernelGGL(lsb_plan_look_kernel, dim3(parts), dim3(PLAN_LOOK_THREADS), 0, s, keys, alt, plan, ws.spine, ws.prefix16, (uint32_t)n,
                        chunks, tw.f32_in, tw.xor_in);
     hipLaunchKernelGGL(lsb_plan_reduce_kernel, dim3(PLAN_BLOCKS), dim3(RADIX), 0, s, alt, plan, parts);
-    hipLaunchKernelGGL(lsb_plan_decide_kernel, dim3(PLAN_BLOCKS), dim3(RADIX), 0, s, plan, (uint32_t)n, parts, plan_cursor_enabled() ? 1u : 0u);
+    hipLaunchKernelGGL(lsb_plan_decide_kernel, dim3(PLAN_BLOCKS), dim3(RADIX), 0, s, plan, (uint32_t)n, parts, plan_mode_bits());
     return (int)hipGetLastError();
 }
 
@@ -570,21 +589,17 @@
     if ((char *)cursor < (char *)ws.prefix16) return hipErrorInvalidValue;
     {
         KernelTimer kt(GS_K_OTHER, s);
-        hipLaunchKernelGGL(lsb_plan_upsweep2_kernel<true>, dim3(p.grid), dim3(LSB_THREADS), 0, s, kin, ws.spine, ws.prefix16, plan, cursor, p);
+        hipLaunchKernelGGL(lsb_plan_upsweep2_kernel<true>, dim3(p.grid), dim3(LSB_THREADS), 0, s, kin, ws.spine, ws.prefix16, plan, cursor, p,
+                           plan_narrow_enabled() ? 1u : 0u);
     }
     if (p.n >= (uint32_t)LSB_TILE) {
         KernelTimer kt(GS_K_LSB_DOWNSWEEP, s);
-        if (p.n > (1u << 30))
-            hipLaunchKernelGGL((lsb_plan_scatter2_kernel<false, true>), dim3(p.ds_grid), dim3(LSB_THREADS), 0, s, kin, kout, ws.totals,
-                               ws.spine, ws.prefix16, plan, cursor, p);
-        else
-            hipLaunchKernelGGL((lsb_plan_scatter2_kernel<false, false>), dim3(p.ds_grid), dim3(LSB_THREADS), 0, s, kin, kout, ws.totals,
-                               ws.spine, ws.prefix16, plan, cursor, p);
+        launch_plan_scatter2(kin, kout, ws, plan, cursor, p, s);
     }
     {
         KernelTimer kt(GS_K_OTHER, s);
         hipLaunchKernelGGL(lsb_plan_irregular_kernel, dim3(PLAN_IRR_CAP + (p.n % (uint32_t)LSB_TILE ? 1u : 0u)), dim3(LSB_THREADS), 0, s, kin,
-                           kout, plan, cursor, p.n);
+                           kout, plan, cursor, p.n, plan_narrow_enabled() ? 1u : 0u);
     }
     return (int)hipGetLastError();
 }
@@ -657,7 +672,7 @@
     const uint32_t route = w[0], nonempty = w[2], total = w[7], mode = w[8];
     if (route != PLAN_PLANNED && route != PLAN_CLASSIC) return seen;
     if (route == PLAN_PLANNED ? (uint64_t)total != n : (uint64_t)total > n) return seen;
-    if (mode > 1u || (mode && route != PLAN_PLANNED)) return seen;
+    if (mode > (PLAN_MODE_CURSOR | PLAN_MODE_NARROW) || mode == PLAN_MODE_NARROW || (mode && route != PLAN_PLANNED)) return seen;
     uint64_t sum = 0;
     for (int c = 0; c < MSB_NCLASS; ++c) {
         if (w[3 + c] > plan_list_cap(n, c)) return seen;
@@ -666,7 +681,7 @@
     if (route == PLAN_PLANNED ? sum != nonempty : sum != 0) return seen;
     seen.ok = true;
     seen.route = route;
-    seen.cursor_mode = mode;
+    seen.cursor_mode = mode & PLAN_MODE_CURSOR;
     for (int c = 0; c < MSB_NCLASS; ++c) seen.tasks[c] = w[3 + c];
     return seen;
 }
@@ -728,7 +743,7 @@
     }
     if ((e = (int)hipGetLastError())) return e;
     if ((e = msb_local_sorts_in_place(plan->level, lists.tasks, PLAN_GROUPS, PLAN_GROUPS, d_keys[sel], PLAN_SORT_BITS, n, tw.f32_out,
-                                      tw.xor_out, s, seen.ok ? seen.tasks : nullptr)))
+                                      tw.xor_out, s, seen.ok ? seen.tasks : nullptr, plan_narrow_enabled())))
         return e;
     *selector = sel;
     return hipSuccess;
@@ -769,11 +784,26 @@
     if (e == hipSuccess) e = hipMemcpyAsync(&w[1], &plan->irr[0], sizeof(uint32_t), hipMemcpyDeviceToHost, (hipStream_t)stream);
     if (e == hipSuccess) e = hipStreamSynchronize((hipStream_t)stream);
     if (e != hipSuccess) return (int)e;
-    if (w[0] == 1u) {
+    if (w[0] & PLAN_MODE_CURSOR) {
         out[0] = 1;
         out[2] = w[1];
         out[1] = w[1] + (num_items % (uint64_t)LSB_TILE ? 1u : 0u);
     }
+    return hipSuccess;
+}
+
+int gs_lsb_plan_narrow_status(void *d_temp, uint64_t num_items, uint32_t out[4], void *stream)
+{
+    GS_CLEAR_STALE_ERROR();
+    if (!d_temp || !out || num_items >= (1ull << 32)) return hipErrorInvalidValue;
+    memset(out, 0, 4 * sizeof(uint32_t));
+    if (!plan_enabled() || !plan_size_ok(num_items)) return hipSuccess;
+    const PlanBlock *plan = (const PlanBlock *)(gs_ws_base(d_temp) + plan_block_offset(num_items));
+    uint32_t w = 0;
+    hipError_t e = hipMemcpyAsync(&w, &plan->cursor_mode, sizeof(uint32_t), hipMemcpyDeviceToHost, (hipStream_t)stream);
+    if (e == hipSuccess) e = hipStreamSynchronize((hipStream_t)stream);
+    if (e != hipSuccess) return (int)e;
+    out[0] = (w & PLAN_MODE_CURSOR) && (w & PLAN_MODE_NARROW) ? 1u : 0u;
     return hipSuccess;
 }
 
diff --git a/gpu-sort_amd/csrc/gs_msb.hip b/gpu-sort_amd/csrc/gs_msb.hip
--- a/gpu-sort_amd/csrc/gs_msb.hip
+++ b/gpu-sort_amd/csrc/gs_msb.hip
@@ -945,6 +945,7 @@
 __host__ __device__ constexpr bool ls_is_dedupe(int mode) { return mode == LS_DEDUPE || mode == LS_DEDUPE_ALL; }
 constexpr uint32_t LS_DD = 0x20000000u;
 
+template <bool NARROW_IN = false>
 __global__ __launch_bounds__(256) void msb_task_sample_kernel(MsbWs ws, int L, const uint32_t *__restrict__ src_k, int has_values)
 {
     if (!(L < 3 && (ws.level[L + 1].packed >> 32) != 0ull)) return;
@@ -957,7 +958,9 @@
         for (uint32_t t = wv; t < ntasks; t += nwv) {
             const MsbTask c = ws.tasks[cls][t];
             if (c.sort_bits <= (uint32_t)b1 || c.sort_bits > 16u || c.size < 64u) continue;
-            const uint32_t smp = src_k[c.offset + (uint32_t)(((unsigned long long)(c.size - 8u) * (2u * (lane >> 3) + 1u)) >> 4) + (lane & 7u)];
+            const uint32_t cluster = (uint32_t)(((unsigned long long)(c.size - 8u) * (2u * (lane >> 3) + 1u)) >> 4);
+            const uint32_t smp = NARROW_IN ? (uint32_t)reinterpret_cast<const uint16_t *>(src_k + c.offset)[cluster + (lane & 7u)]
+                                           : src_k[c.offset + cluster + (lane & 7u)];
             unsigned long long same = ~0ull;
             for (uint32_t b = 0; b < c.sort_bits; ++b) {
                 const bool bit = (smp >> b) & 1u;
@@ -988,7 +991,7 @@
 #define LSP(k) do { } while (0)
 #define LSP_WAIT(what) do { } while (0)
 #endif
-template <int THREADS, int KPT, bool HAS_VALUES, bool STABLE = false, int MODE = LS_ALL, bool PLAIN = false>
+template <int THREADS, int KPT, bool HAS_VALUES, bool STABLE = false, int MODE = LS_ALL, bool PLAIN = false, bool NARROW_IN = false>
 #ifndef GS_LS_WPE_512x18
 #define GS_LS_WPE_512x18 4
 #endif
@@ -1009,6 +1012,7 @@
     const uint32_t wbase0 = (uint32_t)w * (WAVE * KPT) + lane;
     auto fresh = [](uint32_t x) { asm volatile("" : "+v"(x)); return x; };
     static_assert(!(STABLE && MODE != LS_ALL), "the stable sort has one plan");
+    static_assert(!NARROW_IN || (!STABLE && !HAS_VALUES), "16-bit input: unstable keys-only tasks (`pad` carries the top half)");
     auto advance = [&](uint32_t from, MsbTask &out) {
         uint32_t t = from;
         for (; t < ntasks; t += gridDim.x) {
@@ -1039,8 +1043,9 @@
 #pragma unroll
         for (int i = 0; i < KPT; ++i) {
             const uint32_t idx = wbase + i * WAVE;
-            const uint32_t off = (idx < last ? idx : last) * 4u;
-            key[i] = *reinterpret_cast<const uint32_t *>(reinterpret_cast<const char *>(pk) + off);
+            const uint32_t off = (idx < last ? idx : last) * (NARROW_IN ? 2u : 4u);
+            if constexpr (NARROW_IN) key[i] = *reinterpret_cast<const uint16_t *>(reinterpret_cast<const char *>(pk) + off);
+            else key[i] = *reinterpret_cast<const uint32_t *>(reinterpret_cast<const char *>(pk) + off);
             if (HAS_VALUES) val[i] = *reinterpret_cast<const uint32_t *>(reinterpret_cast<const char *>(pv) + off);
         }
     };
@@ -1062,7 +1067,8 @@
 #pragma unroll
             for (int i = 0; i < KPT; ++i) {
                 const uint32_t idx = wbase + i * WAVE;
-                const uint32_t k = PLAIN ? key[i] : twiddle_in(key[i], f32_in, xor_in);
+                const uint32_t k32 = NARROW_IN ? key[i] | (T.pad << 16) : key[i];
+                const uint32_t k = PLAIN ? k32 : twiddle_in(k32, f32_in, xor_in);
                 key[i] = (idx < T.size) ? k : 0xffffffffu;
             }
         }
@@ -1606,7 +1612,7 @@
 {
     return (min_bits > b1 && min_bits <= onepass_bits) || (min_bits + 8 > b1 && min_bits + 8 <= onepass_bits);
 }
-template <bool HAS_VALUES, bool STABLE = false>
+template <bool HAS_VALUES, bool STABLE = false, bool NARROW_IN = false>
 static void launch_local_sorts(const MsbWs &ws, int L, uint32_t bound, const uint32_t *sk, uint32_t *dk, const uint32_t *sv,
                                uint32_t *dv, int f32_in, uint32_t xor_in, int f32_out, uint32_t xor_out, hipStream_t s,
                                int min_bits = 0, uint64_t num_items = 0, const uint32_t *known_tasks = nullptr, bool maybe_skew = true)
@@ -1624,10 +1630,10 @@
 #endif
         return (uint32_t)(b < MSB_LS_MAX_GRID ? (b ? b : 1) : MSB_LS_MAX_GRID);
     };
-#define GS_LS1P(C, HV, M, P) hipLaunchKernelGGL((msb_local_sort_kernel<msb_class_threads(C), msb_class_kpt(C), HV, STABLE, M, P>), dim3(grid_of(C)), \
+#define GS_LS1P(C, HV, M, P) hipLaunchKernelGGL((msb_local_sort_kernel<msb_class_threads(C), msb_class_kpt(C), HV, STABLE, M, P, NARROW_IN>), dim3(grid_of(C)), \
                                                dim3(msb_class_threads(C)), 0, s, ws, L, C, sk, dk, sv, dv, f32_in, xor_in, f32_out, xor_out)
 #define GS_LS1(C, HV, M) GS_LS1P(C, HV, M, false)
-#define GS_LSDD(C, HV, M) hipLaunchKernelGGL((msb_local_sort_kernel<msb_class_threads(C), msb_class_kpt(C), HV, STABLE, M, false>),                \
+#define GS_LSDD(C, HV, M) hipLaunchKernelGGL((msb_local_sort_kernel<msb_class_threads(C), msb_class_kpt(C), HV, STABLE, M, false, NARROW_IN>),     \
                                              dim3(grid_of(C)), dim3(msb_class_threads(C)), 0, s, ws, L, C, sk, dk, sv, dv,                             \
                                              f32_in, xor_in, f32_out, xor_out)
     const bool plain = !f32_in && !xor_in && !f32_out && !xor_out;
@@ -1648,7 +1654,7 @@
         if (known_tasks) waves = (uint64_t)known_tasks[0] + known_tasks[1] + known_tasks[2] + known_tasks[3];
         if (L < 3 && waves && maybe_skew) {
             const uint32_t blocks = (uint32_t)(waves / 4 + 1 < 2048 ? waves / 4 + 1 : 2048);
-            hipLaunchKernelGGL(msb_task_sample_kernel, dim3(blocks), dim3(256), 0, s, ws, L, sk, HAS_VALUES ? 1 : 0);
+            hipLaunchKernelGGL(msb_task_sample_kernel<NARROW_IN>, dim3(blocks), dim3(256), 0, s, ws, L, sk, HAS_VALUES ? 1 : 0);
         }
     }
     if (wanted(0)) GS_LS(0, HAS_VALUES);
@@ -1662,7 +1668,8 @@
 }
 
 int msb_local_sorts_in_place(MsbLevel *level, MsbTask *const tasks[MSB_NCLASS], uint32_t max_tasks, uint32_t bound, uint32_t *keys,
-                             int sort_bits, uint64_t num_items, int f32_out, uint32_t xor_out, hipStream_t s, const uint32_t *known_tasks)
+                             int sort_bits, uint64_t num_items, int f32_out, uint32_t xor_out, hipStream_t s, const uint32_t *known_tasks,
+                             bool narrow_in)
 {
     MsbWs ws{};
     ws.level = level;
@@ -1670,7 +1677,12 @@
     ws.max_tasks = max_tasks;
     ws.tile_shift = 13u;
     ws.key_bits = 32u;
-    launch_local_sorts<false>(ws, 0, bound, keys, keys, nullptr, nullptr, 0, 0u, f32_out, xor_out, s, sort_bits, num_items, known_tasks);
+    if (narrow_in && sort_bits != 16) return hipErrorInvalidValue;
+    if (narrow_in)
+        launch_local_sorts<false, false, true>(ws, 0, bound, keys, keys, nullptr, nullptr, 0, 0u, f32_out, xor_out, s, sort_bits, num_items,
+                                               known_tasks);
+    else
+        launch_local_sorts<false>(ws, 0, bound, keys, keys, nullptr, nullptr, 0, 0u, f32_out, xor_out, s, sort_bits, num_items, known_tasks);
     return (int)hipGetLastError();
 }
 
diff --git a/gpu-sort_amd/csrc/gs_msb_tasks.hpp b/gpu-sort_amd/csrc/gs_msb_tasks.hpp
--- a/gpu-sort_amd/csrc/gs_msb_tasks.hpp
+++ b/gpu-sort_amd/csrc/gs_msb_tasks.hpp
@@ -38,6 +38,6 @@
 
 int msb_local_sorts_in_place(MsbLevel *level, MsbTask *const tasks[MSB_NCLASS], uint32_t max_tasks, uint32_t bound, uint32_t *keys,
                              int sort_bits, uint64_t num_items, int f32_out, uint32_t xor_out, hipStream_t s,
-                             const uint32_t *known_tasks = nullptr);
+                             const uint32_t *known_tasks = nullptr, bool narrow_in = false);
 
 }
diff --git a/include/gpusort.h b/include/gpusort.h
--- a/include/gpusort.h
+++ b/include/gpusort.h
@@ -56,6 +56,7 @@
 int  gs_lsb_pipe_status(void *d_temp, uint64_t num_items, uint32_t *h_status, void *stream);
 int  gs_lsb_plan_status(void *d_temp, uint64_t num_items, uint32_t out[8], void *stream);
 int  gs_lsb_plan_cursor_status(void *d_temp, uint64_t num_items, uint32_t out[4], void *stream);
+int  gs_lsb_plan_narrow_status(void *d_temp, uint64_t num_items, uint32_t out[4], void *stream);
 int  gs_lsb_plan_peek_status(uint32_t out[4]);
 int  gs_lsb_plan_look_only(void *d_temp, const void *d_keys, void *d_alt, uint64_t num_items,
                            int key_type, int descending, void *stream);
```

Result: no change. 163.2 Gkeys/s, median of 4 (+1.3%).
